# ricklisz/AnatoMask

Hardware: AMD Instinct MI355X
Metric: pretrain volumes/sec @128^3 patch mask=0.6 (higher is better)
Workload: dtype bf16; 1 GPU; STUNet-B AnatoMask step, 128^3 patch, mask_ratio 0.6, bf16 storage/MFMA + fp32 master; per_gpu_batch=16, global_batch=16, parallelism=dp1, step=teacher fwd + sampler + student fwd + loss + bwd + clip + AdamW + EMA

## Files before the change

anatomask_amd/csrc/stream_ops.hip:

```cpp
#include <mutex>
#include <type_traits>
#include "common.h"
#include "../../include/anatomask_hip.h"

namespace {

constexpr int NREP = 8;

struct Geo {
  int B, D, H, W, C;
  int vpw;
  unsigned mW, mH, mD;
  MaskView mask;
  __device__ __forceinline__ bool active(long v) const {
    if (!mask.m) return true;
    const unsigned u = (unsigned)v;
    const unsigned t1 = __umulhi(u, mW); const int w = u - t1 * W;
    const unsigned t2 = __umulhi(t1, mH); const int h = t1 - t2 * H;
    const unsigned b = __umulhi(t2, mD); const int d = t2 - b * D;
    return mask.active((int)b, d, h, w);
  }
  __device__ __forceinline__ void decode(long v, int& b, int& d, int& h, int& w) const {
    const unsigned u = (unsigned)v;
    const unsigned t1 = __umulhi(u, mW); w = u - t1 * W;
// ... 6 lines not shown
template <typename T> struct Walk {
  int cpv, vpp, cl, vl; bool live;
  __device__ __forceinline__ Walk(int C, int nthr = 256) {
    cpv = C / TT<T>::EPC; vpp = nthr / cpv; cl = threadIdx.x % cpv; vl = threadIdx.x / cpv; live = vl < vpp;
  }
};

template <typename T, int NT = 256>
__global__ __launch_bounds__(NT) void chan_stats_kernel(const T* __restrict__ x, Geo g, double* __restrict__ sums) {
  constexpr int EPC = TT<T>::EPC;
  __shared__ float red[NT * 2 * 8];
  Walk<T> wk(g.C, NT);
  float s1[EPC], s2[EPC];
#pragma unroll
  for (int i = 0; i < EPC; ++i) s1[i] = s2[i] = 0.f;
  const long v0 = (long)blockIdx.x * g.vpw, v1 = min(v0 + (long)g.vpw, g.nvox());
  if (wk.live)
    for (long v = v0 + wk.vl; v < v1; v += wk.vpp) {
      if (!g.active(v)) continue;
      float f[EPC];
      chunk_to_f<T>(*(const u32x4*)(x + v * g.C + wk.cl * EPC), f);
#pragma unroll
      for (int i = 0; i < EPC; ++i) { s1[i] += f[i]; s2[i] += f[i] * f[i]; }
    }
#pragma unroll
  for (int i = 0; i < EPC; ++i) { red[(threadIdx.x * 2) * 8 + i] = s1[i]; red[(threadIdx.x * 2 + 1) * 8 + i] = s2[i]; }
  __syncthreads();
  if (threadIdx.x < wk.cpv) {
    double a1[EPC], a2[EPC];
#pragma unroll
    for (int i = 0; i < EPC; ++i) a1[i] = a2[i] = 0.0;
    for (int vl = 0; vl < wk.vpp; ++vl) {
      const int t = vl * wk.cpv + threadIdx.x;
#pragma unroll
      for (int i = 0; i < EPC; ++i) { a1[i] += red[(t * 2) * 8 + i]; a2[i] += red[(t * 2 + 1) * 8 + i]; }
    }
#pragma unroll
    for (int i = 0; i < EPC; ++i) {
      const int c = threadIdx.x * EPC + i;
      double* sr = sums + (size_t)(blockIdx.x % NREP) * g.C * 2;
      atomicAdd(&sr[c * 2], a1[i]); atomicAdd(&sr[c * 2 + 1], a2[i]);
    }
  }
}

__global__ void mask_count_kernel(const uint8_t* mask, int n, int voxels_per_patch, double* out) {
  __shared__ double part[4];
  double c = 0;
  for (int i = threadIdx.x; i < n; i += 256) c += mask[i] ? 1.0 : 0.0;
  c = warp_sum_d(c);
  if ((threadIdx.x & 63) == 0) part[threadIdx.x >> 6] = c;
  __syncthreads();
  if (threadIdx.x == 0) out[0] = (part[0] + part[1] + part[2] + part[3]) * voxels_per_patch;
}

__global__ void norm_finalize_kernel(const double* sums, int nrep, const double* count_ptr, double count_host, int C,
                                     const float* gamma, const float* beta, float eps, float* mean, float* rstd,
                                     float* scale, float* shift, float* run_mean, float* run_var, float momentum) {
  const int c = blockIdx.x * 256 + threadIdx.x;
  if (c >= C) return;
  const double n = count_ptr ? count_ptr[0] : count_host;
  double q1 = 0.0, q2 = 0.0;
  for (int r = 0; r < nrep; ++r) { q1 += sums[((size_t)r * C + c) * 2]; q2 += sums[((size_t)r * C + c) * 2 + 1]; }
  const double m = q1 / n;
  double var = q2 / n - m * m;
  if (var < 0) var = 0;
  const float rs = (float)(1.0 / sqrt(var + (double)eps));
  mean[c] = (float)m; rstd[c] = rs;
  const float sc = gamma[c] * rs;
  scale[c] = sc; shift[c] = beta[c] - (float)m * sc;
  if (run_mean) {
    run_mean[c] = (1.f - momentum) * run_mean[c] + momentum * (float)m;
    run_var[c] = (1.f - momentum) * run_var[c] + momentum * (float)(var * (n / (n - 1.0)));
  }
}

__global__ void norm_fold_running_kernel(int C, const float* gamma, const float* beta, const float* run_mean,
                                         const float* run_var, float eps, float* scale, float* shift) {
  const int c = blockIdx.x * 256 + threadIdx.x;
  if (c >= C) return;
  const float sc = gamma[c] / sqrtf(run_var[c] + eps);
  scale[c] = sc; shift[c] = beta[c] - run_mean[c] * sc;
}

__device__ __forceinline__ float act_fwd(float v, int act) {
  if (act == AM_ACT_LRELU) return v > 0.f ? v : 0.01f * v;
  if (act == AM_ACT_RELU6) return fminf(fmaxf(v, 0.f), 6.f);
  return v;
}
__device__ __forceinline__ float act_grad(float out, int act) {
  if (act == AM_ACT_LRELU) return out > 0.f ? 1.f : 0.01f;
  if (act == AM_ACT_RELU6) return (out > 0.f && out < 6.f) ? 1.f : 0.f;
  return 1.f;
}

__device__ __forceinline__ float act_grad_pre(float pre, int act) {
  if (act == AM_ACT_LRELU) return pre > 0.f ? 1.f : 0.01f;
  if (act == AM_ACT_RELU6) return (pre > 0.f && pre < 6.f) ? 1.f : 0.f;
  return 1.f;
}

template <typename T, int NT = 256, int ACT_ = -1>
__global__ __launch_bounds__(NT) void norm_apply_kernel(const T* __restrict__ x, Geo g, const float* __restrict__ scale,
                                                         const float* __restrict__ shift, int act, const T* __restrict__ res,
                                                         const float* __restrict__ stem_x, const float* __restrict__ stem_w,
                                                         const float* __restrict__ stem_b, const float* __restrict__ fill,
                                                         T* __restrict__ y) {
  constexpr int EPC = TT<T>::EPC;
  Walk<T> wk(g.C, NT);
  if (!wk.live) return;
  float sc[EPC], sh[EPC];
#pragma unroll
  for (int i = 0; i < EPC; ++i) { sc[i] = scale[wk.cl * EPC + i]; sh[i] = shift[wk.cl * EPC + i]; }
  const long v0 = (long)blockIdx.x * g.vpw, v1 = min(v0 + (long)g.vpw, g.nvox());
  for (long v = v0 + wk.vl; v < v1; v += wk.vpp) {
    const size_t off = (size_t)v * g.C + wk.cl * EPC;
    float o[EPC];
    if (g.active(v)) {
      float f[EPC];
      chunk_to_f<T>(*(const u32x4*)(x + off), f);
#pragma unroll
      for (int i = 0; i < EPC; ++i) o[i] = f[i] * sc[i] + sh[i];
      if (res) {
        float r[EPC];
        chunk_to_f<T>(*(const u32x4*)(res + off), r);
#pragma unroll
        for (int i = 0; i < EPC; ++i) o[i] += r[i];
      }
      if (stem_x) {
        const float xv = stem_x[v];
#pragma unroll
        for (int i = 0; i < EPC; ++i) o[i] += stem_w[wk.cl * EPC + i] * xv + stem_b[wk.cl * EPC + i];
      }
#pragma unroll
      for (int i = 0; i < EPC; ++i) o[i] = act_fwd(o[i], ACT_ >= 0 ? ACT_ : act);
    } else if (fill) {
#pragma unroll
      for (int i = 0; i < EPC; ++i) o[i] = fill[wk.cl * EPC + i];
    } else {
      continue;
    }
    *(u32x4*)(y + off) = f_to_chunk<T>(o);
  }
}


struct BwdFin {
  unsigned* ticket;
  const double* count_ptr; double count_host;
  const float* gamma; const float* rstd;
  float *k0, *k1, *k2, *dgamma, *dbeta, *dtoken, *dbeta2;
};

__device__ __forceinline__ bool last_workgroup(unsigned* ticket) {
  __shared__ unsigned tk;
  asm volatile("s_waitcnt vmcnt(0)" ::: "memory");
  __syncthreads();
  if (threadIdx.x == 0) tk = atomicAdd(ticket, 1u);
  __syncthreads();
  return tk == gridDim.x - 1;
}

__device__ __forceinline__ void bwd_reduce_tail(double* bsum, int C, const BwdFin& f) {
  if (!f.ticket) return;
  if (!last_workgroup(f.ticket)) return;
  const double n = f.count_ptr ? f.count_ptr[0] : f.count_host;
  for (int c = threadIdx.x; c < C; c += blockDim.x) {
    double b1 = 0.0, b2 = 0.0, b3 = 0.0;
    for (int r = 0; r < NREP; ++r) {
      double* q = bsum + ((size_t)r * C + c) * 3;
      b1 += __longlong_as_double(atomicExch((unsigned long long*)&q[0], 0ull));
      b2 += __longlong_as_double(atomicExch((unsigned long long*)&q[1], 0ull));
      b3 += __longlong_as_double(atomicExch((unsigned long long*)&q[2], 0ull));
    }
    const float gr = f.gamma[c] * f.rstd[c];
    f.k0[c] = gr; f.k1[c] = gr * (float)(b1 / n); f.k2[c] = gr * (float)(b2 / n);
    if (f.dgamma) f.dgamma[c] += (float)b2;
    if (f.dbeta) f.dbeta[c] += (float)b1;
    if (f.dbeta2) f.dbeta2[c] += (float)b1;
    if (f.dtoken) f.dtoken[c] += (float)b3;
  }
  if (threadIdx.x == 0) atomicExch(f.ticket, 0u);
}

constexpr double AM_DX_FIX = 68719476736.0;
__device__ __forceinline__ void dxsum_tail(double* rep, int nrep, int C, float* accum, unsigned* ticket) {
  if (!ticket) return;
  if (!last_workgroup(ticket)) return;
  for (int c = threadIdx.x; c < C; c += blockDim.x) {
    long long s_ = 0;
    for (int r = 0; r < nrep; ++r) s_ += (long long)atomicExch((unsigned long long*)&rep[(size_t)r * C + c], 0ull);
    accum[c] += (float)((double)s_ / AM_DX_FIX);
  }
  if (threadIdx.x == 0) atomicExch(ticket, 0u);
}

template <typename T, int NT = 256, int ACT_ = -1, int OUT_ = 0>
__global__ __launch_bounds__(NT) void norm_bwd_reduce_kernel(const T* __restrict__ dout, const T* __restrict__ out,
                                                              const T* __restrict__ x, Geo g, const float* __restrict__ mean,
                                                              const float* __restrict__ rstd, int act, int fill,
                                                              double* __restrict__ bsum, const float* __restrict__ psc,
                                                              const float* __restrict__ psh, BwdFin fin) {
  constexpr int EPC = TT<T>::EPC;
  const int actv = ACT_ >= 0 ? ACT_ : act;
  const bool has_out = ACT_ >= 0 ? OUT_ != 0 : out != nullptr;
  __shared__ float red[NT * 3 * 8];
  Walk<T> wk(g.C, NT);
  float s1[EPC], s2[EPC], s3[EPC], mu[EPC], rs[EPC], qs[EPC], qh[EPC];
#pragma unroll
  for (int i = 0; i < EPC; ++i) { s1[i] = s2[i] = s3[i] = 0.f; mu[i] = rs[i] = qs[i] = qh[i] = 0.f; }
  if (wk.live) {
#pragma unroll
    for (int i = 0; i < EPC; ++i) {
      mu[i] = mean[wk.cl * EPC + i]; rs[i] = rstd[wk.cl * EPC + i];
      if (!has_out && actv != AM_ACT_NONE) { qs[i] = psc[wk.cl * EPC + i]; qh[i] = psh[wk.cl * EPC + i]; }
    }
    const long v0 = (long)blockIdx.x * g.vpw, v1 = min(v0 + (long)g.vpw, g.nvox());
    for (long v = v0 + wk.vl; v < v1; v += wk.vpp) {
      const size_t off = (size_t)v * g.C + wk.cl * EPC;
      const bool a = g.active(v);
      if (!a && !fill) continue;
      float d[EPC];
      chunk_to_f<T>(*(const u32x4*)(dout + off), d);
      if (!a) {
#pragma unroll
        for (int i = 0; i < EPC; ++i) s3[i] += d[i];
        continue;
      }
      float f[EPC];
      chunk_to_f<T>(*(const u32x4*)(x + off), f);
      if (actv != AM_ACT_NONE) {
        if (has_out) {
          float o[EPC];
          chunk_to_f<T>(*(const u32x4*)(out + off), o);
#pragma unroll
          for (int i = 0; i < EPC; ++i) d[i] *= act_grad(o[i], actv);
        } else {
#pragma unroll
          for (int i = 0; i < EPC; ++i) d[i] *= act_grad_pre(f[i] * qs[i] + qh[i], actv);
        }
      }
#pragma unroll
      for (int i = 0; i < EPC; ++i) { s1[i] += d[i]; s2[i] += d[i] * (f[i] - mu[i]) * rs[i]; }
    }
  }
#pragma unroll
  for (int i = 0; i < EPC; ++i) {
    red[(threadIdx.x * 3) * 8 + i] = s1[i]; red[(threadIdx.x * 3 + 1) * 8 + i] = s2[i]; red[(threadIdx.x * 3 + 2) * 8 + i] = s3[i];
  }
  __syncthreads();
  if (threadIdx.x < wk.cpv) {
    double a1[EPC], a2[EPC], a3[EPC];
#pragma unroll
    for (int i = 0; i < EPC; ++i) a1[i] = a2[i] = a3[i] = 0.0;
    for (int vl = 0; vl < wk.vpp; ++vl) {
      const int t = vl * wk.cpv + threadIdx.x;
#pragma unroll
      for (int i = 0; i < EPC; ++i) { a1[i] += red[(t * 3) * 8 + i]; a2[i] += red[(t * 3 + 1) * 8 + i]; a3[i] += red[(t * 3 + 2) * 8 + i]; }
    }
#pragma unroll
    for (int i = 0; i < EPC; ++i) {
      const int c = threadIdx.x * EPC + i;
      double* br = bsum + (size_t)(blockIdx.x % NREP) * g.C * 3;
      atomicAdd(&br[c * 3], a1[i]); atomicAdd(&br[c * 3 + 1], a2[i]);
      if (fill) atomicAdd(&br[c * 3 + 2], a3[i]);
    }
  }
  bwd_reduce_tail(bsum, g.C, fin);
}

__global__ void norm_bwd_finalize_kernel(const double* bsum, const double* count_ptr, double count_host, int C,
                                         const float* gamma, const float* rstd, float* k0, float* k1, float* k2,
                                         float* dgamma, float* dbeta, float* dtoken, float* dbeta2) {
  const int c = blockIdx.x * 256 + threadIdx.x;
  if (c >= C) return;
  const double n = count_ptr ? count_ptr[0] : count_host;
  double b1 = 0.0, b2 = 0.0, b3 = 0.0;
  for (int r = 0; r < NREP; ++r) { const double* q = bsum + ((size_t)r * C + c) * 3; b1 += q[0]; b2 += q[1]; b3 += q[2]; }
  const float gr = gamma[c] * rstd[c];
  k0[c] = gr;
  k1[c] = gr * (float)(b1 / n);
  k2[c] = gr * (float)(b2 / n);
  if (dgamma) dgamma[c] += (float)b2;
  if (dbeta) dbeta[c] += (float)b1;
  if (dbeta2) dbeta2[c] += (float)b1;
  if (dtoken) dtoken[c] += (float)b3;
}

template <typename T, int NT = 256, int ACT_ = -1, int OUT_ = 0>
__global__ __launch_bounds__(NT) void norm_bwd_apply_kernel(const T* __restrict__ dout, const T* __restrict__ out,
                                                             const T* __restrict__ x, Geo g, const float* __restrict__ mean,
                                                             const float* __restrict__ rstd, const float* __restrict__ k0,
                                                             const float* __restrict__ k1, const float* __restrict__ k2, int act,
                                                             T* __restrict__ dx, T* __restrict__ dres, double* __restrict__ dxsum,
                                                             int dxrep, const float* __restrict__ psc, const float* __restrict__ psh,
                                                             float* __restrict__ dx_accum, unsigned* dx_ticket) {
  constexpr int EPC = TT<T>::EPC;
  const int actv = ACT_ >= 0 ? ACT_ : act;
  const bool has_out = ACT_ >= 0 ? OUT_ != 0 : out != nullptr;
  __shared__ float red[NT * 8];
  Walk<T> wk(g.C, NT);
  float mu[EPC], rs[EPC], c0[EPC], c1[EPC], c2[EPC], sx[EPC], qs[EPC], qh[EPC];
#pragma unroll
  for (int i = 0; i < EPC; ++i) {
    const int c = wk.cl * EPC + i;
    sx[i] = 0.f; qs[i] = qh[i] = 0.f;
    if (wk.live) {
      mu[i] = mean[c]; rs[i] = rstd[c]; c0[i] = k0[c]; c1[i] = k1[c]; c2[i] = k2[c];
      if (!has_out && actv != AM_ACT_NONE) { qs[i] = psc[c]; qh[i] = psh[c]; }
    }
  }
  const long v0 = (long)blockIdx.x * g.vpw, v1 = min(v0 + (long)g.vpw, g.nvox());
  if (wk.live)
    for (long v = v0 + wk.vl; v < v1; v += wk.vpp) {
      if (!g.active(v)) continue;
      const size_t off = (size_t)v * g.C + wk.cl * EPC;
      float d[EPC], f[EPC];
      chunk_to_f<T>(*(const u32x4*)(dout + off), d);
      chunk_to_f<T>(*(const u32x4*)(x + off), f);
      if (actv != AM_ACT_NONE) {
        if (has_out) {
          float o[EPC];
          chunk_to_f<T>(*(const u32x4*)(out + off), o);
#pragma unroll
          for (int i = 0; i < EPC; ++i) d[i] *= act_grad(o[i], actv);
        } else {
#pragma unroll
          for (int i = 0; i < EPC; ++i) d[i] *= act_grad_pre(f[i] * qs[i] + qh[i], actv);
        }
      }
      if (dres) *(u32x4*)(dres + off) = f_to_chunk<T>(d);
      float r[EPC];
#pragma unroll
      for (int i = 0; i < EPC; ++i) r[i] = c0[i] * d[i] - c1[i] - c2[i] * (f[i] - mu[i]) * rs[i];
      const u32x4 pk = f_to_chunk<T>(r);
      *(u32x4*)(dx + off) = pk;
      if (dxsum) {
        float q[EPC];
        chunk_to_f<T>(pk, q);
#pragma unroll
        for (int i = 0; i < EPC; ++i) sx[i] += q[i];
      }
    }
  if (dxsum) {
#pragma unroll
    for (int i = 0; i < EPC; ++i) red[threadIdx.x * 8 + i] = sx[i];
    __syncthreads();
    if (threadIdx.x < wk.cpv) {
      float a1[EPC];
#pragma unroll
      for (int i = 0; i < EPC; ++i) a1[i] = 0.f;
      for (int vl = 0; vl < wk.vpp; ++vl)
#pragma unroll
        for (int i = 0; i < EPC; ++i) a1[i] += red[(vl * wk.cpv + threadIdx.x) * 8 + i];
#pragma unroll
      for (int i = 0; i < EPC; ++i)
        atomicAdd((unsigned long long*)&dxsum[(size_t)(blockIdx.x % dxrep) * g.C + threadIdx.x * EPC + i], (unsigned long long)__double2ll_rn((double)a1[i] * AM_DX_FIX));
    }
    dxsum_tail(dxsum, dxrep, g.C, dx_accum, dx_ticket);
  }
}


struct RowGeo {
  int B, D, H, W, C, bs;
  int rowchunks;
  int rpp;
  int rpw;
  long total_rows;
  const int* plist;
};
constexpr int UNR = 4;

template <typename T> struct RowWalk {
  int cl, vx, r0, cpv; bool live;
  long row, row_end; int rpp;
  __device__ __forceinline__ RowWalk(const RowGeo& g) {
    cpv = g.C / TT<T>::EPC;
    const int c = threadIdx.x % g.rowchunks;
    r0 = threadIdx.x / g.rowchunks; cl = c % cpv; vx = c / cpv; rpp = g.rpp; live = r0 < g.rpp;
    row = (long)blockIdx.x * g.rpw + r0;
    row_end = min((long)(blockIdx.x + 1) * g.rpw, g.total_rows);
  }
  __device__ __forceinline__ long voxel(const RowGeo& g, long rw) const {
    const int P = 1 << g.bs;
    const int a = (int)(rw >> (2 * g.bs)), r = (int)(rw & (P * P - 1));
    const int pk = g.plist[a];
    const int b = (pk >> 24) & 255, pd = (pk >> 16) & 255, ph = (pk >> 8) & 255, pw = pk & 255;
    return (((long)b * g.D + pd * P + (r >> g.bs)) * g.H + ph * P + (r & (P - 1))) * g.W + pw * P + vx;
  }
};

template <typename T, int ACT, int MODE>
__global__ __launch_bounds__(256) void norm_apply_rows_kernel(const T* __restrict__ x, RowGeo g, const float* __restrict__ scale,
                                                              const float* __restrict__ shift, const T* __restrict__ res,
                                                              const float* __restrict__ stem_x, const float* __restrict__ stem_w,
                                                              const float* __restrict__ stem_b, T* __restrict__ y) {
  constexpr int EPC = TT<T>::EPC;
  RowWalk<T> wk(g);
  float sc[EPC], sh[EPC], sw[EPC];
#pragma unroll
  for (int i = 0; i < EPC; ++i) {
    sc[i] = scale[wk.cl * EPC + i]; sh[i] = shift[wk.cl * EPC + i]; sw[i] = 0.f;
    if (MODE == 2) { sw[i] = stem_w[wk.cl * EPC + i]; sh[i] += stem_b[wk.cl * EPC + i]; }
  }
  const int P = 1 << g.bs, pm = P * P - 1, sh2 = 2 * g.bs;
  const long last = wk.row_end - 1;
  if (wk.row > last) return;
  int pk[UNR];
#pragma unroll
  for (int u = 0; u < UNR; ++u) { const long r = min(wk.row + (long)u * wk.rpp, last); pk[u] = g.plist[r >> sh2]; }
  for (long rw = wk.row; rw <= last; rw += (long)UNR * wk.rpp) {
    size_t off[UNR]; long vox[UNR]; u32x4 xv[UNR], rv[UNR]; float sx[UNR];
#pragma unroll
    for (int u = 0; u < UNR; ++u) {
      const long r = min(rw + (long)u * wk.rpp, last);
      const int q = (int)(r & pm);
      const int b = (pk[u] >> 24) & 255, pd = (pk[u] >> 16) & 255, ph = (pk[u] >> 8) & 255, pw = pk[u] & 255;
      vox[u] = (((long)b * g.D + pd * P + (q >> g.bs)) * g.H + ph * P + (q & (P - 1))) * g.W + pw * P + wk.vx;
      off[u] = (size_t)vox[u] * g.C + wk.cl * EPC;
    }
#pragma unroll
    for (int u = 0; u < UNR; ++u) {
      xv[u] = *(const u32x4*)(x + off[u]);
      if (MODE == 1) rv[u] = *(const u32x4*)(res + off[u]);
      if (MODE == 2) sx[u] = stem_x[vox[u]];
    }
#pragma unroll
    for (int u = 0; u < UNR; ++u) {
      const long r = min(rw + (long)(UNR + u) * wk.rpp, last);
      pk[u] = g.plist[r >> sh2];
    }
#pragma unroll
    for (int u = 0; u < UNR; ++u) {
      float f[EPC], o[EPC];
      chunk_to_f<T>(xv[u], f);
#pragma unroll
      for (int i = 0; i < EPC; ++i) o[i] = f[i] * sc[i] + sh[i];
      if (MODE == 1) {
        float r[EPC];
        chunk_to_f<T>(rv[u], r);
#pragma unroll
        for (int i = 0; i < EPC; ++i) o[i] += r[i];
      }
      if (MODE == 2) {
#pragma unroll
        for (int i = 0; i < EPC; ++i) o[i] += sw[i] * sx[u];
      }
#pragma unroll
      for (int i = 0; i < EPC; ++i) o[i] = act_fwd(o[i], ACT);
      *(u32x4*)(y + off[u]) = f_to_chunk<T>(o);
    }
  }
}

template <typename T>
__global__ __launch_bounds__(256) void chan_stats_rows_kernel(const T* __restrict__ x, RowGeo g, double* __restrict__ sums) {
  constexpr int EPC = TT<T>::EPC;
  __shared__ float red[256 * 2 * 8];
  RowWalk<T> wk(g);
  float s1[EPC], s2[EPC];
#pragma unroll
  for (int i = 0; i < EPC; ++i) s1[i] = s2[i] = 0.f;
  if (wk.live)
    for (long rw = wk.row; rw < wk.row_end; rw += (long)UNR * wk.rpp) {
      long v[UNR]; u32x4 xv[UNR];
#pragma unroll
      for (int u = 0; u < UNR; ++u) { const long r = rw + (long)u * wk.rpp; v[u] = r < wk.row_end ? wk.voxel(g, r) : -1; }
#pragma unroll
      for (int u = 0; u < UNR; ++u) if (v[u] >= 0) xv[u] = *(const u32x4*)(x + (size_t)v[u] * g.C + wk.cl * EPC);
#pragma unroll
      for (int u = 0; u < UNR; ++u) {
        if (v[u] < 0) continue;
        float f[EPC];
        chunk_to_f<T>(xv[u], f);
#pragma unroll
        for (int i = 0; i < EPC; ++i) { s1[i] += f[i]; s2[i] += f[i] * f[i]; }
      }
    }
#pragma unroll
  for (int i = 0; i < EPC; ++i) { red[(threadIdx.x * 2) * 8 + i] = s1[i]; red[(threadIdx.x * 2 + 1) * 8 + i] = s2[i]; }
  __syncthreads();
  const int nlane = blockDim.x / wk.cpv;
  if (threadIdx.x < wk.cpv) {
    double a1[EPC], a2[EPC];
#pragma unroll
    for (int i = 0; i < EPC; ++i) a1[i] = a2[i] = 0.0;
    for (int vl = 0; vl < nlane; ++vl) {
      const int t = vl * wk.cpv + threadIdx.x;
#pragma unroll
      for (int i = 0; i < EPC; ++i) { a1[i] += red[(t * 2) * 8 + i]; a2[i] += red[(t * 2 + 1) * 8 + i]; }
    }
#pragma unroll
    for (int i = 0; i < EPC; ++i) {
      const int c = threadIdx.x * EPC + i;
      double* sr = sums + (size_t)(blockIdx.x % NREP) * g.C * 2;
      atomicAdd(&sr[c * 2], a1[i]); atomicAdd(&sr[c * 2 + 1], a2[i]);
    }
  }
}

template <typename T, int ACT_ = -1, int OUT_ = 0>
__global__ __launch_bounds__(256) void norm_bwd_reduce_rows_kernel(const T* __restrict__ dout, const T* __restrict__ out,
                                                                   const T* __restrict__ x, RowGeo g, const float* __restrict__ mean,
                                                                   const float* __restrict__ rstd, int act, double* __restrict__ bsum,
                                                                   const float* __restrict__ psc, const float* __restrict__ psh, BwdFin fin) {
  constexpr int EPC = TT<T>::EPC;
  const int actv = ACT_ >= 0 ? ACT_ : act;
  const bool has_out = ACT_ >= 0 ? OUT_ != 0 : out != nullptr;
  __shared__ float red[256 * 2 * 8];
  RowWalk<T> wk(g);
  float s1[EPC], s2[EPC], mu[EPC], rs[EPC], qs[EPC], qh[EPC];
#pragma unroll
  for (int i = 0; i < EPC; ++i) { s1[i] = s2[i] = 0.f; mu[i] = rs[i] = qs[i] = qh[i] = 0.f; }
  if (wk.live) {
#pragma unroll
    for (int i = 0; i < EPC; ++i) {
      mu[i] = mean[wk.cl * EPC + i]; rs[i] = rstd[wk.cl * EPC + i];
      if (!has_out && actv != AM_ACT_NONE) { qs[i] = psc[wk.cl * EPC + i]; qh[i] = psh[wk.cl * EPC + i]; }
    }
    for (long rw = wk.row; rw < wk.row_end; rw += (long)UNR * wk.rpp) {
      long v[UNR]; u32x4 dv[UNR], xv[UNR], ov[UNR];
#pragma unroll
      for (int u = 0; u < UNR; ++u) { const long r = rw + (long)u * wk.rpp; v[u] = r < wk.row_end ? wk.voxel(g, r) : -1; }
#pragma unroll
      for (int u = 0; u < UNR; ++u) {
        if (v[u] < 0) continue;
        const size_t off = (size_t)v[u] * g.C + wk.cl * EPC;
        dv[u] = *(const u32x4*)(dout + off); xv[u] = *(const u32x4*)(x + off);
        if (has_out && actv != AM_ACT_NONE) ov[u] = *(const u32x4*)(out + off);
      }
#pragma unroll
      for (int u = 0; u < UNR; ++u) {
        if (v[u] < 0) continue;
        float d[EPC], f[EPC];
        chunk_to_f<T>(dv[u], d); chunk_to_f<T>(xv[u], f);
        if (actv != AM_ACT_NONE) {
          if (has_out) {
            float o[EPC];
            chunk_to_f<T>(ov[u], o);
#pragma unroll
            for (int i = 0; i < EPC; ++i) d[i] *= act_grad(o[i], actv);
          } else {
#pragma unroll
            for (int i = 0; i < EPC; ++i) d[i] *= act_grad_pre(f[i] * qs[i] + qh[i], actv);
          }
        }
#pragma unroll
        for (int i = 0; i < EPC; ++i) { s1[i] += d[i]; s2[i] += d[i] * (f[i] - mu[i]) * rs[i]; }
      }
    }
  }
#pragma unroll
  for (int i = 0; i < EPC; ++i) { red[(threadIdx.x * 2) * 8 + i] = s1[i]; red[(threadIdx.x * 2 + 1) * 8 + i] = s2[i]; }
  __syncthreads();
  const int nlane = blockDim.x / wk.cpv;
  if (threadIdx.x < wk.cpv) {
    double a1[EPC], a2[EPC];
#pragma unroll
    for (int i = 0; i < EPC; ++i) a1[i] = a2[i] = 0.0;
    for (int vl = 0; vl < nlane; ++vl) {
      const int t = vl * wk.cpv + threadIdx.x;
#pragma unroll
      for (int i = 0; i < EPC; ++i) { a1[i] += red[(t * 2) * 8 + i]; a2[i] += red[(t * 2 + 1) * 8 + i]; }
    }
#pragma unroll
    for (int i = 0; i < EPC; ++i) {
      const int c = threadIdx.x * EPC + i;
      double* br = bsum + (size_t)(blockIdx.x % NREP) * g.C * 3;
      atomicAdd(&br[c * 3], a1[i]); atomicAdd(&br[c * 3 + 1], a2[i]);
    }
  }
  bwd_reduce_tail(bsum, g.C, fin);
}

template <typename T, int ACT_ = -1, int OUT_ = 0>
__global__ __launch_bounds__(256) void norm_bwd_apply_rows_kernel(const T* __restrict__ dout, const T* __restrict__ out,
                                                                  const T* __restrict__ x, RowGeo g, const float* __restrict__ mean,
                                                                  const float* __restrict__ rstd, const float* __restrict__ k0,
                                                                  const float* __restrict__ k1, const float* __restrict__ k2, int act,
                                                                  T* __restrict__ dx, T* __restrict__ dres, double* __restrict__ dxsum,
                                                                  int dxrep, const float* __restrict__ psc, const float* __restrict__ psh,
                                                                  float* __restrict__ dx_accum, unsigned* dx_ticket) {
  constexpr int EPC = TT<T>::EPC;
  const int actv = ACT_ >= 0 ? ACT_ : act;
  const bool has_out = ACT_ >= 0 ? OUT_ != 0 : out != nullptr;
  __shared__ float red[256 * 8];
  RowWalk<T> wk(g);
  float mu[EPC], rs[EPC], c0[EPC], c1[EPC], c2[EPC], sx[EPC], qs[EPC], qh[EPC];
#pragma unroll
  for (int i = 0; i < EPC; ++i) {
    const int c = wk.cl * EPC + i;
    sx[i] = 0.f; qs[i] = qh[i] = 0.f;
    if (wk.live) {
      mu[i] = mean[c]; rs[i] = rstd[c]; c0[i] = k0[c]; c1[i] = k1[c]; c2[i] = k2[c];
      if (!has_out && actv != AM_ACT_NONE) { qs[i] = psc[c]; qh[i] = psh[c]; }
    }
  }
  if (wk.live)
    for (long rw = wk.row; rw < wk.row_end; rw += (long)UNR * wk.rpp) {
      long v[UNR]; u32x4 dv[UNR], xv[UNR], ov[UNR];
#pragma unroll
      for (int u = 0; u < UNR; ++u) { const long r = rw + (long)u * wk.rpp; v[u] = r < wk.row_end ? wk.voxel(g, r) : -1; }
#pragma unroll
      for (int u = 0; u < UNR; ++u) {
        if (v[u] < 0) continue;
        const size_t off = (size_t)v[u] * g.C + wk.cl * EPC;
        dv[u] = *(const u32x4*)(dout + off); xv[u] = *(const u32x4*)(x + off);
        if (has_out && actv != AM_ACT_NONE) ov[u] = *(const u32x4*)(out + off);
      }
#pragma unroll
      for (int u = 0; u < UNR; ++u) {
        if (v[u] < 0) continue;
        const size_t off = (size_t)v[u] * g.C + wk.cl * EPC;
        float d[EPC], f[EPC];
        chunk_to_f<T>(dv[u], d); chunk_to_f<T>(xv[u], f);
        if (actv != AM_ACT_NONE) {
          if (has_out) {
            float o[EPC];
            chunk_to_f<T>(ov[u], o);
#pragma unroll
            for (int i = 0; i < EPC; ++i) d[i] *= act_grad(o[i], actv);
          } else {
#pragma unroll
            for (int i = 0; i < EPC; ++i) d[i] *= act_grad_pre(f[i] * qs[i] + qh[i], actv);
          }
        }
        if (dres) *(u32x4*)(dres + off) = f_to_chunk<T>(d);
        float r[EPC];
#pragma unroll
        for (int i = 0; i < EPC; ++i) r[i] = c0[i] * d[i] - c1[i] - c2[i] * (f[i] - mu[i]) * rs[i];
        const u32x4 pk = f_to_chunk<T>(r);
        *(u32x4*)(dx + off) = pk;
        if (dxsum) {
          float q[EPC];
          chunk_to_f<T>(pk, q);
#pragma unroll
          for (int i = 0; i < EPC; ++i) sx[i] += q[i];
        }
      }
    }
  if (dxsum) {
#pragma unroll
    for (int i = 0; i < EPC; ++i) red[threadIdx.x * 8 + i] = sx[i];
    __syncthreads();
    const int nlane = blockDim.x / wk.cpv;
    if (threadIdx.x < wk.cpv) {
      float a1[EPC];
#pragma unroll
      for (int i = 0; i < EPC; ++i) a1[i] = 0.f;
      for (int vl = 0; vl < nlane; ++vl)
#pragma unroll
        for (int i = 0; i < EPC; ++i) a1[i] += red[(vl * wk.cpv + threadIdx.x) * 8 + i];
#pragma unroll
      for (int i = 0; i < EPC; ++i)
        atomicAdd((unsigned long long*)&dxsum[(size_t)(blockIdx.x % dxrep) * g.C + threadIdx.x * EPC + i], (unsigned long long)__double2ll_rn((double)a1[i] * AM_DX_FIX));
    }
    dxsum_tail(dxsum, dxrep, g.C, dx_accum, dx_ticket);
  }
}

__global__ __launch_bounds__(256) void mask_compact_kernel(const uint8_t* __restrict__ mask, int B, int fd, int fh, int fw,
                                                           int* __restrict__ list, int* __restrict__ count) {
  __shared__ int wsum[4];
  __shared__ int base;
  const int n = B * fd * fh * fw;
  if (threadIdx.x == 0) base = 0;
  __syncthreads();
  for (int i0 = 0; i0 < n; i0 += 256) {
    const int i = i0 + threadIdx.x;
    const int a = (i < n && mask[i]) ? 1 : 0;
    const unsigned long long bal = __ballot(a);
    const int lane = threadIdx.x & 63, wv = threadIdx.x >> 6;
    const int pre = __popcll(bal & ((1ull << lane) - 1ull));
    if (lane == 0) wsum[wv] = __popcll(bal);
    __syncthreads();
    int off = base;
    for (int w = 0; w < wv; ++w) off += wsum[w];
    if (a) {
      int q = i;
      const int pw = q % fw; q /= fw;
      const int ph = q % fh; q /= fh;
      const int pd = q % fd; const int b = q / fd;
      list[off + pre] = (b << 24) | (pd << 16) | (ph << 8) | pw;
    }
    __syncthreads();
    if (threadIdx.x == 0) base += wsum[0] + wsum[1] + wsum[2] + wsum[3];
    __syncthreads();
  }
  if (threadIdx.x == 0) count[0] = base;
}

template <typename T, int NT = 256>
__global__ __launch_bounds__(NT) void chan_sum_kernel(const T* __restrict__ x, Geo g, float* __restrict__ out) {
  constexpr int EPC = TT<T>::EPC;
  __shared__ float red[NT * 8];
  Walk<T> wk(g.C, NT);
  float s1[EPC];
#pragma unroll
  for (int i = 0; i < EPC; ++i) s1[i] = 0.f;
  const long v0 = (long)blockIdx.x * g.vpw, v1 = min(v0 + (long)g.vpw, g.nvox());
  if (wk.live)
    for (long v = v0 + wk.vl; v < v1; v += wk.vpp) {
      if (!g.active(v)) continue;
      float f[EPC];
      chunk_to_f<T>(*(const u32x4*)(x + v * g.C + wk.cl * EPC), f);
#pragma unroll
      for (int i = 0; i < EPC; ++i) s1[i] += f[i];
    }
#pragma unroll
  for (int i = 0; i < EPC; ++i) red[threadIdx.x * 8 + i] = s1[i];
  __syncthreads();
  if (threadIdx.x < wk.cpv) {
    float a1[EPC];
#pragma unroll
    for (int i = 0; i < EPC; ++i) a1[i] = 0.f;
    for (int vl = 0; vl < wk.vpp; ++vl)
#pragma unroll
      for (int i = 0; i < EPC; ++i) a1[i] += red[(vl * wk.cpv + threadIdx.x) * 8 + i];
#pragma unroll
    for (int i = 0; i < EPC; ++i) atomicAdd(&out[threadIdx.x * EPC + i], a1[i]);
  }
}

template <typename T>
__global__ void add_kernel(const T* a, const T* b, T* y, size_t nchunk) {
  constexpr int EPC = TT<T>::EPC;
  for (size_t i = (size_t)blockIdx.x * 256 + threadIdx.x; i < nchunk; i += (size_t)gridDim.x * 256) {
    float fa[EPC], fb[EPC];
    chunk_to_f<T>(((const u32x4*)a)[i], fa); chunk_to_f<T>(((const u32x4*)b)[i], fb);
#pragma unroll
    for (int k = 0; k < EPC; ++k) fa[k] += fb[k];
    ((u32x4*)y)[i] = f_to_chunk<T>(fa);
  }
}

constexpr int SBD = 4, SBH = 8, SBW = 16;

template <typename T, int K>
__global__ __launch_bounds__(256) void stem_conv_fwd_kernel(const float* __restrict__ x, Geo g,
                                                            const float* __restrict__ w, const float* __restrict__ bias,
                                                            T* __restrict__ y, float* __restrict__ part) {
  constexpr int EPC = TT<T>::EPC;
  constexpr int NTP = K * K * K, PAD = K / 2;
  constexpr int ED = SBD + 2 * PAD, EH = SBH + 2 * PAD, EW = SBW + 2 * PAD;
  constexpr int MV = SBD * SBH * SBW;
  extern __shared__ float sm[];
  float* wl = sm;
  float* xb = sm + g.C * NTP;
  int bid = blockIdx.x;
  const int nbw = g.W / SBW, nbh = g.H / SBH, nbd = g.D / SBD;
  const int bw_ = bid % nbw; bid /= nbw;
  const int bh_ = bid % nbh; bid /= nbh;
  const int bd_ = bid % nbd; const int b = bid / nbd;
  const int d0 = bd_ * SBD, h0 = bh_ * SBH, w0 = bw_ * SBW;
  float* prow = part ? part + (size_t)blockIdx.x * g.C * 2 : nullptr;
  if (!g.mask.active(b, d0, h0, w0)) {
    if (prow) for (int i = threadIdx.x; i < g.C * 2; i += 256) prow[i] = 0.f;
    return;
  }
  for (int i = threadIdx.x; i < g.C * NTP; i += 256) wl[(i % NTP) * g.C + i / NTP] = w[i];
  for (int e = threadIdx.x; e < ED * EH * EW; e += 256) {
    const int ex = e % EW, ey = (e / EW) % EH, ez = e / (EW * EH);
    const int id = d0 + ez - PAD, ih = h0 + ey - PAD, iw = w0 + ex - PAD;
    float v = 0.f;
    if (id >= 0 && id < g.D && ih >= 0 && ih < g.H && iw >= 0 && iw < g.W && g.mask.active(b, id, ih, iw))
      v = x[((size_t)(b * g.D + id) * g.H + ih) * g.W + iw];
    xb[e] = v;
  }
  __syncthreads();
  Walk<T> wk(g.C);
  float s1[EPC], s2[EPC];
#pragma unroll
  for (int i = 0; i < EPC; ++i) s1[i] = s2[i] = 0.f;
  if (wk.live) {
    float bs[EPC];
#pragma unroll
    for (int i = 0; i < EPC; ++i) bs[i] = bias ? bias[wk.cl * EPC + i] : 0.f;
    constexpr int VPT = 8;
    for (int vb = wk.vl; vb < MV; vb += wk.vpp * VPT) {
      float o[VPT][EPC];
      int xo[VPT];
#pragma unroll
      for (int q = 0; q < VPT; ++q) {
        const int v = vb + q * wk.vpp;
        const int vv = v < MV ? v : 0;
        xo[q] = ((vv / (SBW * SBH)) * EH + (vv / SBW) % SBH) * EW + vv % SBW;
#pragma unroll
        for (int i = 0; i < EPC; ++i) o[q][i] = bs[i];
      }
#pragma unroll 1
      for (int td = 0; td < K; ++td)
#pragma unroll 1
        for (int th = 0; th < K; ++th)
#pragma unroll
          for (int tw = 0; tw < K; ++tw) {
            const int ti = (td * K + th) * K + tw;
            const f32x4 wa = *(const f32x4*)(wl + ti * g.C + wk.cl * EPC);
            f32x4 wb = wa;
            if constexpr (EPC == 8) wb = *(const f32x4*)(wl + ti * g.C + wk.cl * EPC + 4);
#pragma unroll
            for (int q = 0; q < VPT; ++q) {
              const float xv = xb[xo[q] + (td * EH + th) * EW + tw];
#pragma unroll
              for (int i = 0; i < 4; ++i) o[q][i] += wa[i] * xv;
              if constexpr (EPC == 8) {
#pragma unroll
                for (int i = 0; i < 4; ++i) o[q][4 + i] += wb[i] * xv;
              }
            }
          }
#pragma unroll
      for (int q = 0; q < VPT; ++q) {
        const int v = vb + q * wk.vpp;
        if (v >= MV) continue;
        const int lw = v % SBW, lh = (v / SBW) % SBH, ld = v / (SBW * SBH);
        const size_t vox = ((size_t)(b * g.D + d0 + ld) * g.H + h0 + lh) * g.W + w0 + lw;
        const u32x4 pk = f_to_chunk<T>(o[q]);
        *(u32x4*)(y + vox * g.C + wk.cl * EPC) = pk;
        if (prow) {
          float r[EPC];
          chunk_to_f<T>(pk, r);
#pragma unroll
          for (int i = 0; i < EPC; ++i) { s1[i] += r[i]; s2[i] += r[i] * r[i]; }
        }
      }
    }
  }
  if (prow) {
    __syncthreads();
    float* red = sm;
    if (wk.live) {
#pragma unroll
      for (int i = 0; i < EPC; ++i) { red[(threadIdx.x * EPC + i) * 2] = s1[i]; red[(threadIdx.x * EPC + i) * 2 + 1] = s2[i]; }
    }
    __syncthreads();
    for (int c2 = threadIdx.x; c2 < g.C * 2; c2 += 256) {
      const int c = c2 >> 1, cl = c / EPC, i = c % EPC;
      float a = 0.f;
      for (int vl = 0; vl < wk.vpp; ++vl) a += red[((vl * wk.cpv + cl) * EPC + i) * 2 + (c2 & 1)];
      prow[c2] = a;
    }
  }
}


template <int NS>
__global__ __launch_bounds__(256) void stem_conv_mfma_kernel(const float* __restrict__ x, int D, int H, int W, int C, MaskView mask,
                                                             const int* __restrict__ plist, const float* __restrict__ w,
                                                             const float* __restrict__ bias, bf16_t* __restrict__ y,
                                                             float* __restrict__ part) {
  constexpr int E = 18;
  __shared__ float xl[E * E * E + 8];
  __shared__ float red[4 * 16 * NS * 2];
  const int tid = threadIdx.x, lane = tid & 63, wave = tid >> 6, g = lane >> 4, r16 = lane & 15;
  const int pk = plist[blockIdx.x];
  const int b = (pk >> 24) & 255, pd = (pk >> 16) & 255, ph = (pk >> 8) & 255, pw = pk & 255;
  const int d0 = pd * 16, h0 = ph * 16, w0 = pw * 16;
  for (int e = tid; e < E * E * E; e += 256) {
    const int ex = e % E, ey = (e / E) % E, ez = e / (E * E);
    const int id = d0 + ez - 1, ih = h0 + ey - 1, iw = w0 + ex - 1;
    float v = 0.f;
    if ((unsigned)id < (unsigned)D && (unsigned)ih < (unsigned)H && (unsigned)iw < (unsigned)W && mask.active(b, id, ih, iw))
      v = x[((size_t)(b * D + id) * H + ih) * W + iw];
    xl[e] = v;
  }
  typedef __attribute__((ext_vector_type(8))) __bf16 bfx8;
  bfx8 af[NS], afl[NS];
  int toff[8];
#pragma unroll
  for (int j = 0; j < 8; ++j) {
    const int t = 8 * g + j;
    toff[j] = t < 27 ? ((t / 9) * E + (t / 3) % 3) * E + t % 3 : 0;
  }
#pragma unroll
  for (int i = 0; i < NS; ++i) {
    const int ch = crow(i * 16 + r16);
    float wv[8];
#pragma unroll
    for (int j = 0; j < 8; ++j) { const int t = 8 * g + j; wv[j] = t < 27 ? w[ch * 27 + t] : 0.f; }
    u32x4 h, l;
    split8_bf16(wv, h, l);
    af[i] = __builtin_bit_cast(bfx8, h); afl[i] = __builtin_bit_cast(bfx8, l);
  }
  f32x4 bia[NS];
#pragma unroll
  for (int i = 0; i < NS; ++i) bia[i] = bias ? *(const f32x4*)(bias + (i >> 1) * 32 + g * 8 + (i & 1) * 4) : f32x4{0.f, 0.f, 0.f, 0.f};
  float s1[NS][4], s2[NS][4];
#pragma unroll
  for (int i = 0; i < NS; ++i)
#pragma unroll
    for (int q = 0; q < 4; ++q) s1[i][q] = s2[i][q] = 0.f;
  __syncthreads();
  for (int row = wave; row < 256; row += 4) {
    const int dz = row >> 4, dy = row & 15;
    const int base = (dz * E + dy) * E + r16;
    float xv[8];
#pragma unroll
    for (int j = 0; j < 8; ++j) xv[j] = xl[base + toff[j]];
    u32x4 xh, xo;
    split8_bf16(xv, xh, xo);
    const bfx8 bf = __builtin_bit_cast(bfx8, xh), bfl = __builtin_bit_cast(bfx8, xo);
    f32x4 o[NS];
#pragma unroll
    for (int i = 0; i < NS; ++i) {
      o[i] = __builtin_amdgcn_mfma_f32_16x16x32_bf16(afl[i], bf, bia[i], 0, 0, 0);
      o[i] = __builtin_amdgcn_mfma_f32_16x16x32_bf16(af[i], bfl, o[i], 0, 0, 0);
      o[i] = __builtin_amdgcn_mfma_f32_16x16x32_bf16(af[i], bf, o[i], 0, 0, 0);
    }
    const size_t vox = ((size_t)(b * D + d0 + dz) * H + h0 + dy) * W + w0 + r16;
    bf16_t* dst = y + vox * C + g * 8;
#pragma unroll
    for (int h = 0; h < NS / 2; ++h) {
      typedef __attribute__((ext_vector_type(4))) __bf16 bfx4;
      const bfx4 p0 = __builtin_convertvector(o[2 * h], bfx4), p1 = __builtin_convertvector(o[2 * h + 1], bfx4);
      *(bfx8*)(dst + h * 32) = __builtin_shufflevector(p0, p1, 0, 1, 2, 3, 4, 5, 6, 7);
      const f32x4 q0 = __builtin_convertvector(p0, f32x4), q1 = __builtin_convertvector(p1, f32x4);
#pragma unroll
      for (int c = 0; c < 4; ++c) {
        s1[2 * h][c] += q0[c]; s2[2 * h][c] += q0[c] * q0[c];
        s1[2 * h + 1][c] += q1[c]; s2[2 * h + 1][c] += q1[c] * q1[c];
      }
    }
  }
  if (part) {
#pragma unroll
    for (int i = 0; i < NS; ++i)
#pragma unroll
      for (int c = 0; c < 4; ++c) {
        float a1 = s1[i][c], a2 = s2[i][c];
        a1 = row16_sum(a1); a2 = row16_sum(a2);
        if (r16 == 0) {
          const int ch = (i >> 1) * 32 + g * 8 + (i & 1) * 4 + c;
          red[(wave * 16 * NS + ch) * 2] = a1; red[(wave * 16 * NS + ch) * 2 + 1] = a2;
        }
      }
    __syncthreads();
    if (tid < 16 * NS) {
      float a1 = 0.f, a2 = 0.f;
#pragma unroll
      for (int wv = 0; wv < 4; ++wv) { a1 += red[(wv * 16 * NS + tid) * 2]; a2 += red[(wv * 16 * NS + tid) * 2 + 1]; }
      float* pr = part + ((size_t)blockIdx.x * C + tid) * 2;
      pr[0] = a1; pr[1] = a2;
    }
  }
}

__device__ __forceinline__ s16x4 tr_read16(const unsigned char* p) {
  return __builtin_amdgcn_ds_read_tr16_b64_v4i16((__attribute__((address_space(3))) s16x4*)(p));
}

template <int NS, int K>
__global__ __launch_bounds__(256) void stem_wgrad_mfma_kernel(const float* __restrict__ x, const bf16_t* __restrict__ dy, int D, int H, int W,
                                                              MaskView mask, const int* __restrict__ plist, int n_active,
                                                              float* __restrict__ dw, float* __restrict__ db, float* __restrict__ det_ws) {
  constexpr int E = 18, C = 16 * NS, RS = 2 * C + 32;
  constexpr int NTT = K == 3 ? 2 : 1, NTAP = K * K * K;
  constexpr int XB = (E * E * E + 8) * 4;
  constexpr int CPV = C / 8, NLD = CPV;
  extern __shared__ __attribute__((aligned(16))) unsigned char lds[];
  float* xl = (float*)lds;
  unsigned char* yl = lds + XB;
  const int tid = threadIdx.x, lane = tid & 63, wave = tid >> 6, g = lane >> 4, r16 = lane & 15;
  const int q = (lane >> 2) & 3, p = lane & 3;
  typedef __attribute__((ext_vector_type(8))) __bf16 bfx8;
  f32x4 acc[NS][NTT];
#pragma unroll
  for (int i = 0; i < NS; ++i)
#pragma unroll
    for (int n = 0; n < NTT; ++n) acc[i][n] = f32x4{0.f, 0.f, 0.f, 0.f};
  int toff[NTT], kind[NTT];
#pragma unroll
  for (int n = 0; n < NTT; ++n) {
    const int t = 16 * n + r16;
    kind[n] = t < NTAP ? 0 : (t == NTAP ? 1 : 2);
    toff[n] = t < NTAP ? (K == 3 ? ((t / 9) * E + (t / 3) % 3) * E + t % 3 : (E + 1) * E + 1) : 0;
  }
  for (int pi = blockIdx.x; pi < n_active; pi += gridDim.x) {
    const int pk = plist[pi];
    const int b = (pk >> 24) & 255, d0 = ((pk >> 16) & 255) * 16, h0 = ((pk >> 8) & 255) * 16, w0 = (pk & 255) * 16;
    __syncthreads();
    for (int e = tid; e < E * E * E; e += 256) {
      const int ex = e % E, ey = (e / E) % E, ez = e / (E * E);
      const int id = d0 + ez - 1, ih = h0 + ey - 1, iw = w0 + ex - 1;
      float v = 0.f;
      if ((unsigned)id < (unsigned)D && (unsigned)ih < (unsigned)H && (unsigned)iw < (unsigned)W && mask.active(b, id, ih, iw))
        v = x[((size_t)(b * D + id) * H + ih) * W + iw];
      xl[e] = v;
    }
    u32x4 ld[NLD];
    auto load_plane = [&](int dz) {
#pragma unroll
      for (int it = 0; it < NLD; ++it) {
        const int idx = tid + it * 256, vox = idx / CPV, ch = idx % CPV;
        const size_t gv = ((size_t)(b * D + d0 + dz) * H + h0 + (vox >> 4)) * W + w0 + (vox & 15);
        ld[it] = *(const u32x4*)(dy + gv * C + ch * 8);
      }
    };
    load_plane(0);
    for (int dz = 0; dz < 16; ++dz) {
      __syncthreads();
#pragma unroll
      for (int it = 0; it < NLD; ++it) {
        const int idx = tid + it * 256, vox = idx / CPV, ch = idx % CPV;
        *(u32x4*)(yl + vox * RS + ch * 16) = ld[it];
      }
      load_plane(dz < 15 ? dz + 1 : 15);
      __syncthreads();
#pragma unroll
      for (int s2 = 0; s2 < 2; ++s2) {
        const int s = wave + 4 * s2;
        const int v1 = s * 32 + g * 4 + q, v2 = v1 + 16;
        bfx8 af[NS];
#pragma unroll
        for (int i = 0; i < NS; ++i) {
          const s16x4 lo = tr_read16(yl + v1 * RS + (16 * i + 4 * p) * 2), hi = tr_read16(yl + v2 * RS + (16 * i + 4 * p) * 2);
          af[i] = __builtin_bit_cast(bfx8, s16x8{lo[0], lo[1], lo[2], lo[3], hi[0], hi[1], hi[2], hi[3]});
        }
        const int xbase = (dz * E + 2 * s) * E + 4 * g;
#pragma unroll
        for (int n = 0; n < NTT; ++n) {
          float qv[8];
#pragma unroll
          for (int j = 0; j < 4; ++j) { qv[j] = xl[xbase + toff[n] + j]; qv[4 + j] = xl[xbase + toff[n] + E + j]; }
          if (kind[n]) {
#pragma unroll
            for (int j = 0; j < 8; ++j) qv[j] = kind[n] == 1 ? 1.f : 0.f;
          }
          u32x4 xh, xo;
          split8_bf16(qv, xh, xo);
          const bfx8 bf = __builtin_bit_cast(bfx8, xh), bfl = __builtin_bit_cast(bfx8, xo);
#pragma unroll
          for (int i = 0; i < NS; ++i) {
            acc[i][n] = __builtin_amdgcn_mfma_f32_16x16x32_bf16(af[i], bfl, acc[i][n], 0, 0, 0);
            acc[i][n] = __builtin_amdgcn_mfma_f32_16x16x32_bf16(af[i], bf, acc[i][n], 0, 0, 0);
          }
        }
      }
    }
  }
  __syncthreads();
  float* red = (float*)lds;
#pragma unroll
  for (int i = 0; i < NS; ++i)
#pragma unroll
    for (int n = 0; n < NTT; ++n)
#pragma unroll
      for (int r = 0; r < 4; ++r) red[(wave * C + 16 * i + 4 * g + r) * (16 * NTT) + 16 * n + r16] = acc[i][n][r];
  __syncthreads();
  for (int i = tid; i < C * (NTAP + 1); i += 256) {
    const int c = i / (NTAP + 1), t = i % (NTAP + 1);
    float v = 0.f;
#pragma unroll
    for (int wv = 0; wv < 4; ++wv) v += red[(wv * C + c) * (16 * NTT) + t];
    if (det_ws) det_ws[(size_t)blockIdx.x * (C * (NTAP + 1)) + i] = v;
    else if (t < NTAP) atomicAdd(&dw[c * NTAP + t], v);
    else if (db) atomicAdd(&db[c], v);
  }
}

__global__ __launch_bounds__(256) void stem_wgrad_fold_kernel(const float* __restrict__ ws, int nwg, int C, int ntap, float* __restrict__ dw,
                                                              float* __restrict__ db) {
  const int i = blockIdx.x * 256 + threadIdx.x;
  if (i >= C * (ntap + 1)) return;
  float s = 0.f;
  for (int r = 0; r < nwg; ++r) s += ws[(size_t)r * C * (ntap + 1) + i];
  const int c = i / (ntap + 1), t = i % (ntap + 1);
  if (t < ntap) dw[c * ntap + t] += s;
  else if (db) db[c] += s;
}

template <typename T>
__global__ __launch_bounds__(256) void stem_conv_wgrad_kernel(const float* __restrict__ x, const T* __restrict__ dy, Geo g, int k,
                                                              float* __restrict__ dw, float* __restrict__ db) {
  constexpr int EPC = TT<T>::EPC;
  extern __shared__ float sm[];
  const int nt = k * k * k, pad = k / 2;
  const int ED = SBD + 2 * pad, EH = SBH + 2 * pad, EW = SBW + 2 * pad;
  float* acc_l = sm;
  float* xb = sm + g.C * (nt + 1);
  const int nbw = g.W / SBW, nbh = g.H / SBH, nbd = g.D / SBD;
  const int nbrick = g.B * nbd * nbh * nbw;
  for (int i = threadIdx.x; i < g.C * (nt + 1); i += 256) acc_l[i] = 0.f;
  Walk<T> wk(g.C);
  for (int tg = 0; tg < nt; tg += 9) {
    float a[9][EPC], sb[EPC];
#pragma unroll
    for (int q = 0; q < 9; ++q)
#pragma unroll
      for (int i = 0; i < EPC; ++i) a[q][i] = 0.f;
#pragma unroll
    for (int i = 0; i < EPC; ++i) sb[i] = 0.f;
    for (int brick = blockIdx.x; brick < nbrick; brick += gridDim.x) {
      int bid = brick;
      const int bw_ = bid % nbw; bid /= nbw;
      const int bh_ = bid % nbh; bid /= nbh;
      const int bd_ = bid % nbd; const int b = bid / nbd;
      const int d0 = bd_ * SBD, h0 = bh_ * SBH, w0 = bw_ * SBW;
      if (!g.mask.active(b, d0, h0, w0)) continue;
      __syncthreads();
      for (int e = threadIdx.x; e < ED * EH * EW; e += 256) {
        const int ex = e % EW, ey = (e / EW) % EH, ez = e / (EW * EH);
        const int id = d0 + ez - pad, ih = h0 + ey - pad, iw = w0 + ex - pad;
        float v = 0.f;
        if (id >= 0 && id < g.D && ih >= 0 && ih < g.H && iw >= 0 && iw < g.W && g.mask.active(b, id, ih, iw))
          v = x[((size_t)(b * g.D + id) * g.H + ih) * g.W + iw];
        xb[e] = v;
      }
      __syncthreads();
      if (!wk.live) continue;
      for (int v = wk.vl; v < SBD * SBH * SBW; v += wk.vpp) {
        const int lw = v % SBW, lh = (v / SBW) % SBH, ld = v / (SBW * SBH);
        const size_t vox = ((size_t)(b * g.D + d0 + ld) * g.H + h0 + lh) * g.W + w0 + lw;
        float d[EPC];
        chunk_to_f<T>(*(const u32x4*)(dy + vox * g.C + wk.cl * EPC), d);
        if (tg == 0) {
#pragma unroll
          for (int i = 0; i < EPC; ++i) sb[i] += d[i];
        }
#pragma unroll
        for (int q = 0; q < 9; ++q) {
          const int ti = tg + q;
          if (ti < nt) {
            const int td = ti / (k * k), th = (ti / k) % k, tw = ti % k;
            const float xv = xb[((ld + td) * EH + lh + th) * EW + lw + tw];
#pragma unroll
            for (int i = 0; i < EPC; ++i) a[q][i] += d[i] * xv;
          }
        }
      }
    }
    if (wk.live) {
#pragma unroll
      for (int q = 0; q < 9; ++q)
        if (tg + q < nt)
#pragma unroll
          for (int i = 0; i < EPC; ++i) atomicAdd(&acc_l[(wk.cl * EPC + i) * (nt + 1) + tg + q], a[q][i]);
      if (tg == 0)
#pragma unroll
        for (int i = 0; i < EPC; ++i) atomicAdd(&acc_l[(wk.cl * EPC + i) * (nt + 1) + nt], sb[i]);
    }
  }
  __syncthreads();
  for (int i = threadIdx.x; i < g.C * (nt + 1); i += 256) {
    const int c = i / (nt + 1), t = i % (nt + 1);
    const float v = acc_l[i];
    if (v == 0.f) continue;
    if (t < nt) atomicAdd(&dw[c * nt + t], v);
    else if (db) atomicAdd(&db[c], v);
  }
}

template <typename T>
__global__ __launch_bounds__(256) void proj_fwd_kernel(const T* __restrict__ x, long nvox, int C, const float* __restrict__ w,
                                                       const float* __restrict__ b, const float* __restrict__ psc,
                                                       const float* __restrict__ psh, float* __restrict__ rec) {
  constexpr int EPC = TT<T>::EPC;
  const long v = (long)blockIdx.x * 256 + threadIdx.x;
  if (v >= nvox) return;
  float s = b[0];
  if (psc) {
    for (int c = 0; c < C; c += EPC) {
      float f[EPC];
      chunk_to_f<T>(*(const u32x4*)(x + (size_t)v * C + c), f);
#pragma unroll
      for (int i = 0; i < EPC; ++i) s += (f[i] * psc[c + i] + psh[c + i]) * w[c + i];
    }
  } else {
    for (int c = 0; c < C; c += EPC) {
      float f[EPC];
      chunk_to_f<T>(*(const u32x4*)(x + (size_t)v * C + c), f);
#pragma unroll
      for (int i = 0; i < EPC; ++i) s += f[i] * w[c + i];
    }
  }
  rec[v] = s;
}

struct ProjNormFin {
  unsigned* ticket; double n;
  const float *gamma, *beta, *rstd, *scale, *w;
  float *k0w, *k1, *k2, *dgamma, *dbeta, *dw, *db;
};

template <typename T>
__global__ __launch_bounds__(256) void proj_norm_bwd_reduce_kernel(const T* __restrict__ x, const float* __restrict__ drec, long nvox, int C,
                                                                   int vpw, const float* __restrict__ mean, double* __restrict__ acc,
                                                                   ProjNormFin fin) {
  constexpr int EPC = TT<T>::EPC;
  __shared__ float red[256 * 8];
  __shared__ float redb[4];
  __shared__ double s0sh;
  Walk<T> wk(C);
  float s1[EPC], mu[EPC], sb = 0.f;
#pragma unroll
  for (int i = 0; i < EPC; ++i) { s1[i] = 0.f; mu[i] = wk.live ? mean[wk.cl * EPC + i] : 0.f; }
  const long v0 = (long)blockIdx.x * vpw, v1 = min(v0 + (long)vpw, nvox);
  if (wk.live)
    for (long v = v0 + wk.vl; v < v1; v += wk.vpp) {
      const float d = drec[v];
      float f[EPC];
      chunk_to_f<T>(*(const u32x4*)(x + (size_t)v * C + wk.cl * EPC), f);
#pragma unroll
      for (int i = 0; i < EPC; ++i) s1[i] += d * (f[i] - mu[i]);
      if (wk.cl == 0) sb += d;
    }
#pragma unroll
  for (int i = 0; i < EPC; ++i) red[threadIdx.x * 8 + i] = s1[i];
  sb = warp_sum(sb);
  if ((threadIdx.x & 63) == 0) redb[threadIdx.x >> 6] = sb;
// ... 358 lines not shown
  g.vpw = pick_vpw((long)B * D * H * W, C, dtype, reduction);
  g.mW = (unsigned)(0x100000000ull / (unsigned)W) + 1; g.mH = (unsigned)(0x100000000ull / (unsigned)H) + 1;
  g.mD = (unsigned)(0x100000000ull / (unsigned)D) + 1;
  return g;
}
inline bool geo_ok(int B, int D, int H, int W) {
  const unsigned long long n = (unsigned long long)B * D * H * W;
  int m = W > H ? W : H; if (D > m) m = D;
  return n * (unsigned long long)m < 0xffffffffull;
}


inline bool mkrows(RowGeo& r, int dtype, bool reduction, int B, int D, int H, int W, int C, int bs, const int* plist, int n_active) {
  if (!plist || n_active <= 0 || bs < 0 || bs > 6) return false;
  const int epc = dtype == AM_DT_BF16 ? 8 : 4;
  const int P = 1 << bs;
  const long rc = (long)P * C / epc;
  if (rc > 256 || rc < 1 || (D >> bs) > 255 || (H >> bs) > 255 || (W >> bs) > 255 || B > 255) return false;
  if (D % P || H % P || W % P) return false;
  r.B = B; r.D = D; r.H = H; r.W = W; r.C = C; r.bs = bs; r.plist = plist;
  r.rowchunks = (int)rc; r.rpp = 256 / r.rowchunks;
  r.total_rows = (long)n_active * P * P;
  const long target = reduction ? 1024 : 2048;
  long rpw = (r.total_rows + target - 1) / target;
  const long unit = (long)UNR * r.rpp;
  rpw = (rpw + unit - 1) / unit * unit;
  if (rpw < unit) rpw = unit;
  if (rpw > 64 * unit) rpw = 64 * unit;
  r.rpw = (int)rpw;
  return true;
}
inline int rows_blocks(const RowGeo& r) { return (int)((r.total_rows + r.rpw - 1) / r.rpw); }
inline int rows_threads(const RowGeo& r) { return r.rpp * r.rowchunks; }

}

constexpr int F32_MAX_C_512 = 2048, F32_MAX_C_256 = 1024;
template <typename F> inline void by_pack_dtype(int dtype, F&& f) { if (dtype == AM_DT_F32S) f(am_type<f32s_t>{}); else am_by_dtype(dtype, f); }

extern "C" {

int am_chan_stats(int dtype, const void* x, int B, int D, int H, int W, int C, const uint8_t* mask, int bshift, int fd, int fh,
                  int fw, double* sums, const int32_t* active_list, int n_active, void* stream) {
  if (!am_row_ok(dtype, C, F32_MAX_C_512)) return -1;
  Geo g = mkgeo(dtype, true, B, D, H, W, C, mask, bshift, fd, fh, fw);
  const bool geo_bad = mask && !geo_ok(B, D, H, W);
  hipStream_t st = (hipStream_t)stream;
  AM_HIP(hipMemsetAsync(sums, 0, sizeof(double) * 2 * C * NREP, st));
  RowGeo rg;
  if (mask && mkrows(rg, dtype, true, B, D, H, W, C, bshift, active_list, n_active)) {
    am_by_dtype(dtype, [&](auto t) {
      using T = typename decltype(t)::type;
      AM_LAUNCH(chan_stats_rows_kernel<T>, dim3(rows_blocks(rg)), dim3(rows_threads(rg)), 0, st, (const T*)x, rg, sums);
    });
    AM_CHECK_LAUNCH();
    return 0;
  }
  if (geo_bad) return -4;
  const int nb = nblk((long)B * D * H * W, g.vpw);
  am_by_walk(dtype, C, [&](auto t, auto nt) {
    using T = typename decltype(t)::type;
    AM_LAUNCH((chan_stats_kernel<T, nt>), dim3(nb), dim3(nt), 0, st, (const T*)x, g, sums);
  });
  AM_CHECK_LAUNCH();
  return 0;
}

int am_mask_count(const uint8_t* mask, int n, int voxels_per_patch, double* out, void* stream) {
  AM_LAUNCH(mask_count_kernel, dim3(1), dim3(256), 0, (hipStream_t)stream, mask, n, voxels_per_patch, out);
  AM_CHECK_LAUNCH();
  return 0;
}

int am_mask_compact(const uint8_t* mask, int B, int fd, int fh, int fw, int32_t* list, int32_t* count, void* stream) {
  if (B > 255 || fd > 255 || fh > 255 || fw > 255) return -1;
  AM_LAUNCH(mask_compact_kernel, dim3(1), dim3(256), 0, (hipStream_t)stream, mask, B, fd, fh, fw, list, count);
  AM_CHECK_LAUNCH();
  return 0;
}

int am_norm_finalize(const double* sums, int nrep, const double* count_ptr, double count_host, int C, const float* gamma,
                     const float* beta, float eps, float* mean, float* rstd, float* scale, float* shift, float* run_mean,
                     float* run_var, float momentum, void* stream) {
  AM_LAUNCH(norm_finalize_kernel, dim3((C + 255) / 256), dim3(256), 0, (hipStream_t)stream, sums, nrep, count_ptr, count_host,
                     C, gamma, beta, eps, mean, rstd, scale, shift, run_mean, run_var, momentum);
  AM_CHECK_LAUNCH();
  return 0;
}

int am_norm_fold_running(int C, const float* gamma, const float* beta, const float* run_mean, const float* run_var, float eps,
                         float* scale, float* shift, void* stream) {
  AM_LAUNCH(norm_fold_running_kernel, dim3((C + 255) / 256), dim3(256), 0, (hipStream_t)stream, C, gamma, beta, run_mean,
                     run_var, eps, scale, shift);
  AM_CHECK_LAUNCH();
  return 0;
}

int am_norm_apply(int dtype, const void* x, int B, int D, int H, int W, int C, const uint8_t* mask, int bshift, int fd, int fh,
                  int fw, const float* scale, const float* shift, int act, const void* res, const float* stem_x,
                  const float* stem_w, const float* stem_b, const float* fill, void* y, const int32_t* active_list, int n_active,
                  void* stream) {
  if (!am_row_ok(dtype, C, F32_MAX_C_512)) return -1;
  Geo g = mkgeo(dtype, false, B, D, H, W, C, mask, bshift, fd, fh, fw);
  const bool geo_bad = mask && !geo_ok(B, D, H, W);
  hipStream_t st = (hipStream_t)stream;
  RowGeo rg;
  if (mask && !fill && !(res && stem_x) && mkrows(rg, dtype, false, B, D, H, W, C, bshift, active_list, n_active)) {
    const dim3 gr(rows_blocks(rg)), bl(rows_threads(rg));
    const int racts = act == AM_ACT_LRELU || act == AM_ACT_RELU6 ? act : AM_ACT_NONE;
    am_by_dtype_int<AM_ACT_NONE, AM_ACT_LRELU, AM_ACT_RELU6>(dtype, racts, [&](auto t, auto a) {
      using T = typename decltype(t)::type;
      am_by_int<0, 1, 2>(res ? 1 : (stem_x ? 2 : 0), [&](auto m) {
        AM_LAUNCH((norm_apply_rows_kernel<T, a, m>), gr, bl, 0, st, (const T*)x, rg, scale, shift, (const T*)res, stem_x, stem_w, stem_b, (T*)y);
      });
    });
    AM_CHECK_LAUNCH();
    return 0;
  }
  if (geo_bad) return -4;
  const int nb = nblk((long)B * D * H * W, g.vpw);
  am_by_walk_act(dtype, C, act, false, [&](auto t, auto nt, auto a, auto) {
    using T = typename decltype(t)::type;
    AM_LAUNCH((norm_apply_kernel<T, nt, a>), dim3(nb), dim3(nt), 0, st, (const T*)x, g, scale, shift, act, (const T*)res, stem_x, stem_w, stem_b, fill, (T*)y);
  });
  AM_CHECK_LAUNCH();
  return 0;
}

int am_norm_bwd_reduce(int dtype, const void* dout, const void* out, const void* x, int B, int D, int H, int W, int C,
                       const uint8_t* mask, int bshift, int fd, int fh, int fw, const float* mean, const float* rstd, int act,
                       int fill, double* bsum, const float* pre_scale, const float* pre_shift, const int32_t* active_list,
                       int n_active, const double* count_ptr, double count_host, const float* gamma, float* k0, float* k1, float* k2,
                       float* dgamma, float* dbeta, float* dtoken, float* dbeta2, void* stream) {
  if (!am_row_ok(dtype, C, F32_MAX_C_512)) return -1;
  if (!out && act != AM_ACT_NONE && (!pre_scale || !pre_shift)) return -1;
  Geo g = mkgeo(dtype, true, B, D, H, W, C, mask, bshift, fd, fh, fw);
  const bool geo_bad = mask && !geo_ok(B, D, H, W);
  hipStream_t st = (hipStream_t)stream;
  BwdFin fin{};
  if (k0) {
    if (!gamma || !k1 || !k2) return -1;
    fin.ticket = (unsigned*)(bsum + (size_t)3 * C * NREP);
    fin.count_ptr = count_ptr; fin.count_host = count_host; fin.gamma = gamma; fin.rstd = rstd;
    fin.k0 = k0; fin.k1 = k1; fin.k2 = k2; fin.dgamma = dgamma; fin.dbeta = dbeta; fin.dtoken = dtoken; fin.dbeta2 = dbeta2;
  } else {
    AM_HIP(hipMemsetAsync(bsum, 0, sizeof(double) * 3 * C * NREP, st));
  }
  RowGeo rg;
  if (mask && !fill && mkrows(rg, dtype, true, B, D, H, W, C, bshift, active_list, n_active)) {
    am_by_dtype(dtype, [&](auto t) {
      using T = typename decltype(t)::type;
      am_by_act(act, out != nullptr, [&](auto a, auto o) {
        AM_LAUNCH((norm_bwd_reduce_rows_kernel<T, a, o>), dim3(rows_blocks(rg)), dim3(rows_threads(rg)), 0, st, (const T*)dout, (const T*)out, (const T*)x, rg,
                  mean, rstd, act, bsum, pre_scale, pre_shift, fin);
      });
    });
    AM_CHECK_LAUNCH();
    return 0;
  }
  if (geo_bad) return -4;
  const int nb = nblk((long)B * D * H * W, g.vpw);
  am_by_walk_act(dtype, C, act, out != nullptr, [&](auto t, auto nt, auto a, auto o) {
    using T = typename decltype(t)::type;
    AM_LAUNCH((norm_bwd_reduce_kernel<T, nt, a, o>), dim3(nb), dim3(nt), 0, st, (const T*)dout, (const T*)out, (const T*)x, g, mean, rstd, act, fill, bsum,
              pre_scale, pre_shift, fin);
  });
  AM_CHECK_LAUNCH();
  return 0;
}

int am_norm_bwd_finalize(const double* bsum, const double* count_ptr, double count_host, int C, const float* gamma,
                         const float* rstd, float* k0, float* k1, float* k2, float* dgamma, float* dbeta, float* dtoken,
                         float* dbeta2, void* stream) {
  AM_LAUNCH(norm_bwd_finalize_kernel, dim3((C + 255) / 256), dim3(256), 0, (hipStream_t)stream, bsum, count_ptr,
                     count_host, C, gamma, rstd, k0, k1, k2, dgamma, dbeta, dtoken, dbeta2);
  AM_CHECK_LAUNCH();
  return 0;
}

int am_norm_bwd_apply(int dtype, const void* dout, const void* out, const void* x, int B, int D, int H, int W, int C,
                      const uint8_t* mask, int bshift, int fd, int fh, int fw, const float* mean, const float* rstd,
                      const float* k0, const float* k1, const float* k2, int act, void* dx, void* dres, float* dxsum_accum,
                      double* dxsum_scratch, const float* pre_scale, const float* pre_shift, const int32_t* active_list, int n_active,
                      int scratch_is_zero_workspace, void* stream) {
  if (!am_row_ok(dtype, C, F32_MAX_C_512)) return -1;
  if (!out && act != AM_ACT_NONE && (!pre_scale || !pre_shift)) return -1;
  Geo g = mkgeo(dtype, false, B, D, H, W, C, mask, bshift, fd, fh, fw);
  const bool geo_bad = mask && !geo_ok(B, D, H, W);
  hipStream_t st = (hipStream_t)stream;
  RowGeo rg;
  const bool rows = mask && mkrows(rg, dtype, false, B, D, H, W, C, bshift, active_list, n_active);
  if (!rows && geo_bad) return -4;
  const int nb = rows ? rows_blocks(rg) : nblk((long)B * D * H * W, g.vpw);
  if (dxsum_accum && !dxsum_scratch) return -1;
  const bool rep = dxsum_accum != nullptr;
  double* dxs = rep ? dxsum_scratch : nullptr;
  const int nrep = AM_DXREP;
  const bool fused = rep && scratch_is_zero_workspace;
  float* dx_accum = fused ? dxsum_accum : nullptr;
  unsigned* dx_ticket = fused ? (unsigned*)(dxsum_scratch + (size_t)AM_DXREP * C) : nullptr;
  if (rep && !fused) AM_HIP(hipMemsetAsync(dxsum_scratch, 0, sizeof(double) * AM_DXREP * C, st));
  if (rows) {
    am_by_dtype(dtype, [&](auto t) {
      using T = typename decltype(t)::type;
      am_by_act(act, out != nullptr, [&](auto a, auto o) {
        AM_LAUNCH((norm_bwd_apply_rows_kernel<T, a, o>), dim3(nb), dim3(rows_threads(rg)), 0, st, (const T*)dout, (const T*)out, (const T*)x, rg, mean, rstd,
                  k0, k1, k2, act, (T*)dx, (T*)dres, dxs, nrep, pre_scale, pre_shift, dx_accum, dx_ticket);
      });
    });
  } else {
    am_by_walk_act(dtype, C, act, out != nullptr, [&](auto t, auto nt, auto a, auto o) {
      using T = typename decltype(t)::type;
      AM_LAUNCH((norm_bwd_apply_kernel<T, nt, a, o>), dim3(nb), dim3(nt), 0, st, (const T*)dout, (const T*)out, (const T*)x, g, mean, rstd,
                k0, k1, k2, act, (T*)dx, (T*)dres, dxs, nrep, pre_scale, pre_shift, dx_accum, dx_ticket);
    });
  }
  AM_CHECK_LAUNCH();
  if (rep && !fused) { AM_LAUNCH(rep_reduce_kernel, dim3((C + 255) / 256), dim3(256), 0, st, dxsum_scratch, AM_DXREP, C, dxsum_accum); AM_CHECK_LAUNCH(); }
  return 0;
}

int am_chan_sum(int dtype, const void* x, int B, int D, int H, int W, int C, const uint8_t* mask, int bshift, int fd, int fh,
                int fw, float* out_accum, void* stream) {
  if (!am_row_ok(dtype, C, F32_MAX_C_512)) return -1;
  Geo g = mkgeo(dtype, true, B, D, H, W, C, mask, bshift, fd, fh, fw);
  if (mask && !geo_ok(B, D, H, W)) return -4;
  hipStream_t st = (hipStream_t)stream;
  if ((long)B * D * H * W * C <= (4L << 20)) { g.vpw = (int)((long)B * D * H * W); const int vpp = walk_threads(C, dtype) / (C / (dtype == AM_DT_BF16 ? 8 : 4)) > 0 ? walk_threads(C, dtype) / (C / (dtype == AM_DT_BF16 ? 8 : 4)) : 1; g.vpw = (g.vpw + vpp - 1) / vpp * vpp; }
  const int nb = nblk((long)B * D * H * W, g.vpw);
  am_by_walk(dtype, C, [&](auto t, auto nt) {
    using T = typename decltype(t)::type;
    AM_LAUNCH((chan_sum_kernel<T, nt>), dim3(nb), dim3(nt), 0, st, (const T*)x, g, out_accum);
  });
  AM_CHECK_LAUNCH();
  return 0;
}

int am_add(int dtype, const void* a, const void* b, void* y, long n_elems, void* stream) {
  hipStream_t st = (hipStream_t)stream;
  const size_t nchunk = (size_t)n_elems / (dtype == AM_DT_BF16 ? 8 : 4);
  int nb = (int)((nchunk + 255) / 256); if (nb > 4096) nb = 4096; if (nb < 1) nb = 1;
  am_by_dtype(dtype, [&](auto t) {
    using T = typename decltype(t)::type;
    AM_LAUNCH(add_kernel<T>, dim3(nb), dim3(256), 0, st, (const T*)a, (const T*)b, (T*)y, nchunk);
  });
  AM_CHECK_LAUNCH();
  return 0;
}

int am_stem_conv_fwd(int dtype, const float* x, int B, int D, int H, int W, int C, int ksize, const uint8_t* mask, int bshift,
                     int fd, int fh, int fw, const float* w, const float* bias, void* y, float* partials,
                     const int32_t* active_list, int n_active, int* partial_rows_written, void* stream) {
  if (!am_row_ok(dtype, C, F32_MAX_C_256)) return -1;
  if (ksize != 1 && ksize != 3) return -2;
  Geo g = mkgeo(dtype, false, B, D, H, W, C, mask, bshift, fd, fh, fw);
  hipStream_t st = (hipStream_t)stream;
  if (!mask || bshift != 4 || D % 16 || H % 16 || W % 16) return -2;
  if ((long)B * (D / SBD) * (H / SBH) * (W / SBW) > 0x7fffffffL) return -4;
  if (partial_rows_written) *partial_rows_written = B * (D / SBD) * (H / SBH) * (W / SBW);
  if (dtype == AM_DT_BF16 && ksize == 3 && active_list && n_active > 0 && (C == 32 || C == 64 || C == 96) && B <= 255 && fd <= 255 && fh <= 255 && fw <= 255) {
    const MaskView mv{mask, fd, fh, fw, bshift};
    am_by_int<2, 4, 6>(C / 16, [&](auto ns) {
      AM_LAUNCH(stem_conv_mfma_kernel<ns>, dim3(n_active), dim3(256), 0, st, x, D, H, W, C, mv, active_list, w, bias, (bf16_t*)y, partials);
    });
    AM_CHECK_LAUNCH();
    if (partial_rows_written) *partial_rows_written = n_active;
    return 0;
  }
  const int nb = B * (D / SBD) * (H / SBH) * (W / SBW);
  const int pad_ = ksize / 2;
  size_t fl = (size_t)C * ksize * ksize * ksize;
  if (partials && fl < (size_t)256 * 8 * 2) fl = (size_t)256 * 8 * 2;
  const size_t sm = sizeof(float) * (fl + (size_t)(SBD + 2 * pad_) * (SBH + 2 * pad_) * (SBW + 2 * pad_));
  am_by_dtype_int<1, 3>(dtype, ksize, [&](auto t, auto k) {
    using T = typename decltype(t)::type;
    AM_LAUNCH((stem_conv_fwd_kernel<T, k>), dim3(nb), dim3(256), sm, st, x, g, w, bias, (T*)y, partials);
  });
  AM_CHECK_LAUNCH();
  return 0;
}

int am_stem_conv_wgrad(int dtype, const float* x, const void* dy, int B, int D, int H, int W, int C, int ksize,
                       const uint8_t* mask, int bshift, int fd, int fh, int fw, float* dw_accum, float* db_accum,
                       const int32_t* active_list, int n_active, float* det_workspace, long det_workspace_floats, void* stream) {
  if (!am_row_ok(dtype, C, F32_MAX_C_256)) return -1;
  if (ksize != 1 && ksize != 3) return -2;
  Geo g = mkgeo(dtype, true, B, D, H, W, C, mask, bshift, fd, fh, fw);
  hipStream_t st = (hipStream_t)stream;
  if (!mask || bshift != 4 || D % 16 || H % 16 || W % 16) return -2;
  if (dtype == AM_DT_BF16 && active_list && n_active > 0 && (C == 32 || C == 64 || C == 96) && B <= 255 && fd <= 255 && fh <= 255 && fw <= 255) {
    const MaskView mv{mask, fd, fh, fw, bshift};
    int nwg = n_active < 1024 ? n_active : 1024;
    const long det_row = (long)C * (ksize * ksize * ksize + 1);
    if (det_workspace) {
        if (det_workspace_floats < det_row) return -6;
        if (nwg > det_workspace_floats / det_row) nwg = (int)(det_workspace_floats / det_row);
    }
    const size_t sm = (size_t)(18 * 18 * 18 + 8) * 4 + (size_t)256 * (2 * C + 32);
    hipError_t optin = hipSuccess;
    am_by_int<2, 4, 6>(C / 16, [&](auto ns) {
      am_by_int<1, 3>(ksize, [&](auto k) {
        constexpr auto kern = stem_wgrad_mfma_kernel<ns, k>;
        if ((optin = am_lds_optin<kern>()) != hipSuccess) return;
        AM_LAUNCH(kern, dim3(nwg), dim3(256), sm, st, x, (const bf16_t*)dy, D, H, W, mv, active_list, n_active, dw_accum, db_accum, det_workspace);
      });
    });
    AM_HIP(optin);
    AM_CHECK_LAUNCH();
    if (det_workspace) {
      AM_LAUNCH(stem_wgrad_fold_kernel, dim3((unsigned)((det_row + 255) / 256)), dim3(256), 0, st, det_workspace, nwg, C, ksize * ksize * ksize, dw_accum, db_accum);
      AM_CHECK_LAUNCH();
    }
    return 0;
  }
  if ((long)B * (D / SBD) * (H / SBH) * (W / SBW) > 0x7fffffffL) return -4;
  int nb = B * (D / SBD) * (H / SBH) * (W / SBW);
  if (nb > 1024) nb = 1024;
  const int pad_ = ksize / 2;
  const size_t sm = sizeof(float) * ((size_t)C * (ksize * ksize * ksize + 1) + (size_t)(SBD + 2 * pad_) * (SBH + 2 * pad_) * (SBW + 2 * pad_));
  am_by_dtype(dtype, [&](auto t) {
    using T = typename decltype(t)::type;
    AM_LAUNCH(stem_conv_wgrad_kernel<T>, dim3(nb), dim3(256), sm, st, x, (const T*)dy, g, ksize, dw_accum, db_accum);
  });
  AM_CHECK_LAUNCH();
  return 0;
}

int am_proj_fwd(int dtype, const void* x, long nvox, int C, const float* w, const float* b, const float* pre_scale, const float* pre_shift,
                float* rec, void* stream) {
  if (!am_row_ok(dtype, C, F32_MAX_C_256)) return -1;
  if ((pre_scale == nullptr) != (pre_shift == nullptr)) return -1;
  hipStream_t st = (hipStream_t)stream;
  const int nb = (int)((nvox + 255) / 256);
  am_by_dtype(dtype, [&](auto t) {
    using T = typename decltype(t)::type;
    AM_LAUNCH(proj_fwd_kernel<T>, dim3(nb), dim3(256), 0, st, (const T*)x, nvox, C, w, b, pre_scale, pre_shift, rec);
  });
  AM_CHECK_LAUNCH();
  return 0;
}

int am_proj_norm_bwd(int dtype, const void* x, const float* drec, long nvox, int C, const float* w, const float* gamma, const float* beta,
                     const float* mean, const float* rstd, const float* scale, double* workspace, float* coef, void* dx,
                     float* dgamma_accum, float* dbeta_accum, float* dw_accum, float* db_accum, void* stream) {
  if (!am_row_ok(dtype, C, F32_MAX_C_256)) return -1;
  if (!x || !drec || !w || !gamma || !beta || !mean || !rstd || !scale || !workspace || !coef || !dx || !dgamma_accum || !dbeta_accum ||
      !dw_accum || !db_accum || nvox <= 0) return -1;
  hipStream_t st = (hipStream_t)stream;
  ProjNormFin fin{(unsigned*)(workspace + (size_t)NREP * (C + 1)), (double)nvox, gamma, beta, rstd, scale, w,
                  coef, coef + C, coef + 2 * C, dgamma_accum, dbeta_accum, dw_accum, db_accum};
  const int vr = pick_vpw(nvox, C, dtype, true), va = pick_vpw(nvox, C, dtype, false);
  am_by_dtype(dtype, [&](auto t) {
    using T = typename decltype(t)::type;
    AM_LAUNCH(proj_norm_bwd_reduce_kernel<T>, dim3(nblk(nvox, vr)), dim3(256), 0, st, (const T*)x, drec, nvox, C, vr, mean, workspace, fin);
  });
  AM_CHECK_LAUNCH();
  am_by_dtype(dtype, [&](auto t) {
    using T = typename decltype(t)::type;
    AM_LAUNCH(proj_norm_bwd_apply_kernel<T>, dim3(nblk(nvox, va)), dim3(256), 0, st, (const T*)x, drec, nvox, C, va, mean, rstd, coef, coef + C, coef + 2 * C, (T*)dx);
  });
  AM_CHECK_LAUNCH();
  return 0;
}

int am_proj_bwd(int dtype, const void* x, const float* drec, long nvox, int C, const float* w, void* dx, float* dw_accum,
                float* db_accum, float* det_workspace, long det_workspace_floats, void* stream) {
  if (!am_row_ok(dtype, C, F32_MAX_C_256)) return -1;
  hipStream_t st = (hipStream_t)stream;
  const int vpw = pick_vpw(nvox, C, dtype, true);
  const int nb = nblk(nvox, vpw);
  if (det_workspace && det_workspace_floats < (long)nb * (C + 1)) return -6;
  am_by_dtype(dtype, [&](auto t) {
    using T = typename decltype(t)::type;
    AM_LAUNCH(proj_bwd_kernel<T>, dim3(nb), dim3(256), 0, st, (const T*)x, drec, nvox, C, vpw, w, (T*)dx, dw_accum, db_accum, det_workspace);
  });
  AM_CHECK_LAUNCH();
  if (det_workspace) {
    AM_LAUNCH(rows_fold_kernel, dim3((C + 1 + 255) / 256), dim3(256), 0, st, det_workspace, nb, C + 1, C, dw_accum, db_accum);
    AM_CHECK_LAUNCH();
  }
  return 0;
}

int am_partials_reduce(const float* partials, int rows, int C, double* sums, float* sum_accum, void* stream) {
  hipStream_t st = (hipStream_t)stream;
  if ((256 % C == 0 || C % 256 == 0) && rows >= 64) {
    const int rstep = C <= 256 ? 256 / C : 1;
    int nb = rows / (rstep * 16); nb = nb < 1 ? 1 : (nb > 256 ? 256 : nb);
    const int rpb = ((rows + nb - 1) / nb + rstep - 1) / rstep * rstep;
    nb = (rows + rpb - 1) / rpb;
    if (sums) AM_HIP(hipMemsetAsync(sums, 0, sizeof(double) * 2 * C, st));
    AM_LAUNCH(partials_reduce2_kernel, dim3(nb), dim3(256), 0, st, partials, rows, C, rpb, sums, sum_accum);
    AM_CHECK_LAUNCH();
    return 0;
  }
  AM_LAUNCH(partials_reduce_kernel, dim3(C), dim3(256), 0, st, partials, rows, C, sums, sum_accum);
  AM_CHECK_LAUNCH();
  return 0;
}


int am_partials_finalize(const float* partials, int rows, int C, double* workspace, const double* count_ptr, double count_host,
                         const float* gamma, const float* beta, float eps, float* mean, float* rstd, float* scale, float* shift,
                         float* run_mean, float* run_var, float momentum, long* num_batches_tracked, float* sum_accum, void* stream) {
  if (C <= 0 || C > 4096 || rows <= 0 || !workspace) return -1;
  if (gamma && (!beta || !mean || !rstd || !scale || !shift)) return -1;
  if (C % 2) return -1;
  const int cp = C / 2, rstep = cp <= 256 ? 256 / cp : 1;
  int nb = rows / (rstep * 8); nb = nb < 1 ? 1 : (nb > 2048 ? 2048 : nb);
  const int rpb = ((rows + nb - 1) / nb + rstep - 1) / rstep * rstep;
  nb = (rows + rpb - 1) / rpb;
  AM_LAUNCH(partials_finalize_kernel, dim3(nb), dim3(256), 0, (hipStream_t)stream, partials, rows, C, rpb, workspace, count_ptr, count_host,
            gamma, beta, eps, mean, rstd, scale, shift, run_mean, run_var, momentum, num_batches_tracked, sum_accum,
            (const float*)nullptr, (const float*)nullptr, (float*)nullptr, (float*)nullptr, (float*)nullptr, (float*)nullptr, (float*)nullptr, (float*)nullptr);
  AM_CHECK_LAUNCH();
  return 0;
}

int am_norm_bwd_from_partials(const float* partials, int rows, int C, double* workspace, const double* count_ptr, double count_host,
                              const float* gamma, const float* mean, const float* rstd, float* k0, float* k1, float* k2,
                              float* dgamma, float* dbeta, float* dbeta2, void* stream) {
  if (C <= 0 || C > 4096 || C % 2 || rows <= 0 || !workspace || !gamma || !mean || !rstd || !k0 || !k1 || !k2) return -1;
  const int cp = C / 2, rstep = cp <= 256 ? 256 / cp : 1;
  int nb = rows / (rstep * 8); nb = nb < 1 ? 1 : (nb > 2048 ? 2048 : nb);
  const int rpb = ((rows + nb - 1) / nb + rstep - 1) / rstep * rstep;
  nb = (rows + rpb - 1) / rpb;
  AM_LAUNCH(partials_finalize_kernel, dim3(nb), dim3(256), 0, (hipStream_t)stream, partials, rows, C, rpb, workspace, count_ptr, count_host,
            gamma, (const float*)nullptr, 0.f, (float*)nullptr, (float*)nullptr, (float*)nullptr, (float*)nullptr, (float*)nullptr, (float*)nullptr,
            0.f, (long*)nullptr, (float*)nullptr, mean, rstd, k0, k1, k2, dgamma, dbeta, dbeta2);
  AM_CHECK_LAUNCH();
  return 0;
}

int am_pack_weight(int dtype, const float* src, void* dst, int R, int K, int taps, long stride_r, long stride_k, int Rp, int Kp,
                   void* stream) {
  hipStream_t st = (hipStream_t)stream;
  if (Rp < R || Kp < K) return -1;
  dim3 grid(Rp, (Kp + 63) / 64);
  const size_t sm = sizeof(float) * 64 * taps;
  if (dtype == AM_DT_F32S && Kp % 16) return -1;
  by_pack_dtype(dtype, [&](auto t) {
    using T = typename decltype(t)::type;
    AM_LAUNCH(pack_weight_kernel<T>, grid, dim3(256), sm, st, src, (T*)dst, R, K, taps, stride_r, stride_k, Rp, Kp);
  });
  AM_CHECK_LAUNCH();
  return 0;
}

int am_pack_weights_batched(int dtype, const am_pack_desc* descs, int ndesc, int total_blocks, void* stream) {
  hipStream_t st = (hipStream_t)stream;
  if (ndesc <= 0 || total_blocks <= 0) return 0;
  by_pack_dtype(dtype, [&](auto t) { AM_LAUNCH(pack_weights_batched_kernel<typename decltype(t)::type>, dim3(total_blocks), dim3(256), 0, st, descs, ndesc); });
  AM_CHECK_LAUNCH();
  return 0;
}

int am_split_bf16(const float* x, void* hi, void* lo, long n, void* stream) {
  if (n % 4) return -1;
  long nb = (n / 4 + 255) / 256; if (nb > 16384) nb = 16384;
  AM_LAUNCH(split_bf16_kernel, dim3((unsigned)nb), dim3(256), 0, (hipStream_t)stream, x, (bf16_t*)hi, (bf16_t*)lo, n / 4);
  AM_CHECK_LAUNCH();
  return 0;
}

int am_unpack_grad(const float* src_packed, float* dst, int R, int K, int taps, long stride_r, long stride_k, int accumulate,
                   void* stream) {
  const long n = (long)taps * R * K;
  int nb = (int)((n + 255) / 256); if (nb > 8192) nb = 8192;
  AM_LAUNCH(unpack_grad_kernel, dim3(nb), dim3(256), 0, (hipStream_t)stream, src_packed, dst, R, K, taps, stride_r, stride_k, accumulate);
  AM_CHECK_LAUNCH();
  return 0;
}

}
```

anatomask_amd/engine.py:

```python
from __future__ import annotations

from dataclasses import dataclass, field
from typing import Dict, List, Optional, Sequence, Tuple

import torch

from . import ops
from .ops import ACT_LRELU, ACT_NONE, ACT_RELU6, CONV_DGRAD, CONV_FWD, CONVT_DGRAD, CONVT_FWD, MaskInfo, NormStats

ENC = "sparse_encoder.sp_cnn.conv_blocks_context"
DEC = "dense_decoder.dec"


@dataclass
class Spec:
    dims: Sequence[int]
    depth: Sequence[int]
    width: int
    input_size: Tuple[int, int, int]
    in_ch: int = 1
    out_ch: int = 1
    downsample: int = 16
    n_stage: int = 5
    sync_bn: bool = False
# ... 201 lines not shown
    else:
        a1 = ops.norm_apply(y1, st1, ACT_LRELU, mask, bs)
        y2, pt2 = ops.conv3d(CONV_FWD, a1, w2, W[f"{p}.conv2.bias"], sp, 3, 1,
                             in_mask=mask, in_bshift=bs, out_mask=mask, out_bshift=bs, want_partials=True)
    st2 = _sparse_norm(y2, mask, bs, counts, W[f"{p}.norm2.weight"], W[f"{p}.norm2.bias"], 1e-5, pt2)
    if s == 0 and first and prefix is None:
        out = ops.norm_apply(y2, st2, ACT_LRELU, mask, bs, stem=(inp, W[f"{p}.conv3.weight"].view(-1), W[f"{p}.conv3.bias"]))
    elif first:
        sc = ops.conv3d(CONV_FWD, x, pk.get(W, f"{p}.conv3.weight", False, False), W[f"{p}.conv3.bias"], sp, 1, stride,
                        in_mask=mask, in_bshift=bs + (1 if stride == 2 else 0), out_mask=mask, out_bshift=bs)
        out = ops.norm_apply(y2, st2, ACT_LRELU, mask, bs, res=sc)
    else:
        out = ops.norm_apply(y2, st2, ACT_LRELU, mask, bs, res=x)
    rec_.update(y1=y1, st1=st1, a1=a1, y2=y2, st2=st2, out=out)
    return out, rec_


def _dec_block(W, pk, i: int, x, nxt, train: bool, update_running: bool = True, fuse_eval: bool = False, out_skip=None, sync: bool = False,
               head: bool = False, inorm: bool = False, stencil_tail: bool = False):
    q = f"{DEC}.{i}"
    so = tuple(2 * v for v in x.shape[1:4])
    u = ops.conv3d(CONVT_FWD, x, pk.get(W, f"{q}.up_sample.weight", True, False), W[f"{q}.up_sample.bias"], so, 4, 2)
    if inorm:
        assert not head
        c1 = ops.conv3d(CONV_FWD, u, pk.get(W, f"{q}.conv.0.weight", False, False), None, so, 3, 1)
        r, st1 = _instance_norm(c1, ACT_RELU6)
        c2 = ops.conv3d(CONV_FWD, r, pk.get(W, f"{q}.conv.3.weight", False, False), None, so, 3, 1)
        o, st2 = _instance_norm(c2, ACT_NONE, res=nxt)
        return o, {"q": q, "xin": x, "u": u, "c1": c1, "st1": st1, "r": r, "c2": c2, "st2": st2, "inorm": True}
    if not train and fuse_eval:
        C1, C2 = W[f"{q}.conv.0.weight"].shape[0], W[f"{q}.conv.3.weight"].shape[0]
        st1, st2 = NormStats(C1, x.device), NormStats(C2, x.device)
        ops.norm_fold_running(st1, W[f"{q}.conv.1.weight"], W[f"{q}.conv.1.bias"], W[f"{q}.conv.1.running_mean"], W[f"{q}.conv.1.running_var"], 1e-5)
        ops.norm_fold_running(st2, W[f"{q}.conv.4.weight"], W[f"{q}.conv.4.bias"], W[f"{q}.conv.4.running_mean"], W[f"{q}.conv.4.running_var"], 1e-5)
        r = ops.conv3d(CONV_FWD, u, pk.get(W, f"{q}.conv.0.weight", False, False), None, so, 3, 1,
                       ep_scale=st1.scale, ep_shift=st1.shift, ep_act=ACT_RELU6)
        if stencil_tail and nxt is None and ops.head_stencil_supported(r):
            return r, {"stencil": True, "st2": st2}
        o = ops.conv3d(CONV_FWD, r, pk.get(W, f"{q}.conv.3.weight", False, False), None, so, 3, 1,
                       ep_scale=st2.scale, ep_shift=st2.shift, ep_res=nxt, out_mask=out_skip, out_bshift=4 if out_skip is not None else 0)
        return o, None
    c1, pt1 = ops.conv3d(CONV_FWD, u, pk.get(W, f"{q}.conv.0.weight", False, False), None, so, 3, 1, want_partials=train), None
    if train:
        c1, pt1 = c1
    st1 = _batch_norm(c1, W, f"{q}.conv.1", train, pt1, update_running, sync)
    r = ops.norm_apply(c1, st1, ACT_RELU6)
    c2, pt2 = ops.conv3d(CONV_FWD, r, pk.get(W, f"{q}.conv.3.weight", False, False), None, so, 3, 1, want_partials=train), None
    if train:
        c2, pt2 = c2
    st2 = _batch_norm(c2, W, f"{q}.conv.4", train, pt2, update_running, sync)
    if head:
        assert train and nxt is None and st2.sync_world <= 1
        return c2, {"q": q, "xin": x, "u": u, "c1": c1, "st1": st1, "r": r, "c2": c2, "st2": st2, "head": True}
    o = ops.norm_apply(c2, st2, ACT_NONE, res=nxt)
    return o, {"q": q, "xin": x, "u": u, "c1": c1, "st1": st1, "r": r, "c2": c2, "st2": st2}


def encoder_forward(spec: Spec, W, pk: PackCache, inp: torch.Tensor, mask: MaskInfo, counts, tape: Optional[Tape] = None,
                    recompute: bool = False) -> List[torch.Tensor]:
    feats = []
    x = None
    for s in range(spec.n_stage):
        sp = spec.stage_spatial(s)
        if tape is not None and recompute:
            tape.enc_in.append(x)
        for b in range(spec.depth[s]):
            x, rec_ = _enc_block(W, pk, inp, mask, counts, sp, s, b, x, keep=tape is not None)
            if tape is not None and not recompute:
                tape.enc.append(rec_)
        feats.append(x)
    return feats


def densify_forward(spec: Spec, W, pk: PackCache, feats, mask: MaskInfo, counts, tape: Optional[Tape] = None) -> List[torch.Tensor]:
    n_dec = len(spec.dec_chs) - 1
    to_dec = []
    for i in range(n_dec):
        f = feats[4 - i]
        st = _sparse_norm(f, mask, i, counts, W[f"densify_norms.{i}.weight"], W[f"densify_norms.{i}.bias"], 1e-6)
        d = ops.norm_apply(f, st, ACT_NONE, mask, i, fill=W[f"mask_tokens.{i}"].view(-1))
        pw = f"densify_projs.{i}.weight"
        if pw in W:
            k = W[pw].shape[-1]
            pr = ops.conv3d(CONV_FWD, d, pk.get(W, pw, False, False), W[f"densify_projs.{i}.bias"], tuple(d.shape[1:4]), k, 1)
        else:
            pr = d
        to_dec.append(pr)
        if tape is not None:
            tape.dens.append({"i": i, "f": f, "st": st, "d": d, "k": W[pw].shape[-1] if pw in W else 0})
    return to_dec


HEAD_STENCIL = True


def decoder_forward(spec: Spec, W, pk: PackCache, to_dec, train: bool, tape: Optional[Tape] = None, recompute: bool = False,
                    needed_patches: Optional[MaskInfo] = None, fuse_eval: Optional[bool] = None, l2_of: Optional[tuple] = None) -> torch.Tensor:
    n_dec = len(spec.dec_chs) - 1
    if fuse_eval is None:
        fuse_eval = tape is None
    x = to_dec[0]
    head = bool(train and FUSED_HEAD and _sync_world(spec.sync_bn) <= 1 and not spec.dec_inorm)
    st_head = None
    for i in range(n_dec):
        nxt = to_dec[i + 1] if i + 1 < n_dec else None
        last = i == n_dec - 1
        o, rec_ = _dec_block(W, pk, i, x, nxt, train, fuse_eval=fuse_eval,
                             out_skip=needed_patches if (last and tape is None and not train) else None, sync=spec.sync_bn,
                             head=head and last, inorm=spec.dec_inorm,
                             stencil_tail=bool(HEAD_STENCIL and last and tape is None and not train and fuse_eval and not spec.dec_inorm))
        if rec_ is not None and rec_.get("stencil"):
            q = f"{DEC}.{i}"
            weff, beff = ops.head_fold(W[f"{q}.conv.3.weight"], rec_["st2"].scale, rec_["st2"].shift, W["dense_decoder.proj.weight"].view(-1),
                                       W["dense_decoder.proj.bias"])
            B_, D_, H_, W_ = o.shape[:4]
            patches = needed_patches
            if patches is None:
                patches = MaskInfo(torch.ones(B_, D_ // 16, H_ // 16, W_ // 16, device=o.device, dtype=torch.uint8), n_active=B_ * (D_ // 16) * (H_ // 16) * (W_ // 16))
            if l2_of is not None:
                ops.head_stencil(o, weff, beff, patches, inp=l2_of[0], l2=l2_of[1])
                return None
            rec = torch.empty(B_, D_, H_, W_, device=o.device, dtype=torch.float32)
            ops.head_stencil(o, weff, beff, patches, rec=rec)
            return rec
        if head and last:
            st_head = rec_["st2"]
        if tape is not None:
            tape.dec.append({"q": rec_["q"], "xin": x, "nxt": nxt, "head": head and last} if recompute else rec_)
        x = o
    rec = ops.proj_fwd(x, W["dense_decoder.proj.weight"].view(-1), W["dense_decoder.proj.bias"], pre=st_head)
    if tape is not None:
        tape.last = x
    return rec


def forward(spec: Spec, W: Dict[str, torch.Tensor], pk: PackCache, inp: torch.Tensor, mask: MaskInfo, train: bool,
            tape: Optional[Tape] = None, want_feats: bool = False, encoder_only: bool = False, recompute: bool = False,
            want_to_dec0: bool = False, needed_patches: Optional[MaskInfo] = None, l2_out: Optional[torch.Tensor] = None):
    counts = _counts(mask, range(5))
    if tape is not None:
        tape.counts = counts
        tape.recompute = recompute
    feats = encoder_forward(spec, W, pk, inp, mask, counts, tape, recompute)
    if encoder_only:
        return feats
    to_dec = densify_forward(spec, W, pk, feats, mask, counts, tape)
    rec = decoder_forward(spec, W, pk, to_dec, train, tape, recompute, needed_patches, l2_of=(inp, l2_out) if l2_out is not None else None)
    if want_to_dec0:
        return rec, to_dec[0]
    return (rec, feats) if want_feats else rec


FUSED_HEAD = True
_SIDE: Dict[int, "torch.cuda.Stream"] = {}
_SIDE_KEEP: Dict[int, List[torch.Tensor]] = {}
_USE_SIDE = True


def _dev_index(dev) -> int:
    return dev.index if dev.index is not None else torch.cuda.current_device()


def _side_stream(dev) -> "torch.cuda.Stream":
    i = _dev_index(dev)
    if i not in _SIDE:
        _SIDE[i] = torch.cuda.Stream(device=dev)
    return _SIDE[i]


def _on_side(dev, tensors, fn):
    if not _USE_SIDE:
        return fn()
    s2 = _side_stream(dev)
    ev = torch.cuda.Event()
    ev.record()
    s2.wait_event(ev)
    _SIDE_KEEP.setdefault(_dev_index(dev), []).extend(tensors)
    with torch.cuda.stream(s2):
        fn()


def _join_side(dev):
    i = _dev_index(dev)
    if _USE_SIDE and i in _SIDE:
        ev = torch.cuda.Event()
        ev.record(_SIDE[i])
        torch.cuda.current_stream(dev).wait_event(ev)
    _SIDE_KEEP.pop(i, None)


def _wgrad_into(pk: PackCache, G, name, mode, x, dy, k, stride, transposed=False, **masks):
    def run():
        dwp = ops.conv3d_wgrad(mode, x, dy, k, stride, f32_split=pk.f32_split, deterministic=pk.deterministic, **masks)
        ops.unpack_grad(dwp, G[name], transposed, accumulate=True)
    _on_side(x.device, (x, dy), run)


def _dec_block_backward(W, G, pk: PackCache, t: dict, g: Optional[torch.Tensor], drec: Optional[torch.Tensor], bias_sum_into: Optional[torch.Tensor]):
    q = t["q"]
    if t.get("inorm"):
        so = tuple(t["r"].shape[1:4])
        dc2 = _instance_norm_backward(g, t["c2"], t["st2"], ACT_NONE)
        dr = ops.conv3d(CONV_DGRAD, dc2, pk.get(W, f"{q}.conv.3.weight", False, True), None, so, 3, 1)
        _wgrad_into(pk, G, f"{q}.conv.3.weight", CONV_FWD, t["r"], dc2, 3, 1)
        dc1 = _instance_norm_backward(dr, t["c1"], t["st1"], ACT_RELU6)
    elif t.get("head"):
        dc2 = ops.proj_norm_bwd(t["c2"], t["st2"], drec, W["dense_decoder.proj.weight"].view(-1), W[f"{q}.conv.4.weight"],
                                W[f"{q}.conv.4.bias"], G[f"{q}.conv.4.weight"], G[f"{q}.conv.4.bias"],
                                G["dense_decoder.proj.weight"].view(-1), G["dense_decoder.proj.bias"])
    else:
        dc2 = ops.norm_backward(g, None, t["c2"], t["st2"], W[f"{q}.conv.4.weight"], ACT_NONE, None, 0,
                                G[f"{q}.conv.4.weight"], G[f"{q}.conv.4.bias"])
    if not t.get("inorm"):
        so = tuple(t["r"].shape[1:4])
        fuse = ops.FUSED_NORM_BWD_REDUCE and dc2.dtype == torch.bfloat16 and t["st1"].sync_world <= 1 and dc2.shape[-1] >= 128
        dr = ops.conv3d(CONV_DGRAD, dc2, pk.get(W, f"{q}.conv.3.weight", False, True), None, so, 3, 1,
                        norm_bwd=(t["c1"], t["st1"], ACT_RELU6) if fuse else None)
        dr, red1 = dr if fuse else (dr, None)
        _wgrad_into(pk, G, f"{q}.conv.3.weight", CONV_FWD, t["r"], dc2, 3, 1)
        dc1 = ops.norm_backward(dr, None, t["c1"], t["st1"], W[f"{q}.conv.1.weight"], ACT_RELU6, None, 0,
                                G[f"{q}.conv.1.weight"], G[f"{q}.conv.1.bias"], reduced=red1)
    du, ptu = ops.conv3d(CONV_DGRAD, dc1, pk.get(W, f"{q}.conv.0.weight", False, True), None, so, 3, 1, want_partials=True, partials_sum_only=True)
    ptu.finalize(None, sum_accum=G[f"{q}.up_sample.bias"])
    _wgrad_into(pk, G, f"{q}.conv.0.weight", CONV_FWD, t["u"], dc1, 3, 1)
    si = tuple(t["xin"].shape[1:4])
    gin = ops.conv3d(CONVT_DGRAD, du, pk.get(W, f"{q}.up_sample.weight", True, True), None, si, 4, 2, want_partials=bias_sum_into is not None)
    if bias_sum_into is not None:
        gin, ptg = gin
        ptg.finalize(None, sum_accum=bias_sum_into)
    _wgrad_into(pk, G, f"{q}.up_sample.weight", CONVT_FWD, t["xin"], du, 4, 2, transposed=True)
    return gin


def decoder_backward(spec: Spec, W, G, pk: PackCache, tape: Tape, drec: torch.Tensor, after_group=None) -> List[Optional[torch.Tensor]]:
    n_dec = len(spec.dec_chs) - 1
    fused_head = bool(tape.dec[n_dec - 1].get("head"))
    g = None
    if not fused_head:
        g = ops.proj_bwd(tape.last, drec, W["dense_decoder.proj.weight"].view(-1), G["dense_decoder.proj.weight"].view(-1),
                         G["dense_decoder.proj.bias"], deterministic=pk.deterministic)
        if after_group:
            after_group("proj")
    dproj: List[Optional[torch.Tensor]] = [None] * n_dec
    for i in reversed(range(n_dec)):
        t = tape.dec[i]
        if tape.recompute:
            _, t = _dec_block(W, pk, i, t["xin"], t["nxt"], True, update_running=False, sync=spec.sync_bn, head=bool(t.get("head")),
                              inorm=spec.dec_inorm)
            tape.dec[i] = None
        if i + 1 < n_dec:
            dproj[i + 1] = g
        need_sum = i > 0 and f"densify_projs.{i}.bias" in G
        g = _dec_block_backward(W, G, pk, t, g, drec, G[f"densify_projs.{i}.bias"] if need_sum else None)
        if t.get("head") and after_group:
            after_group("proj")
        if after_group:
            after_group(f"dec{i}")
    dproj[0] = g
    return dproj


def densify_backward(spec: Spec, W, G, pk: PackCache, mask: MaskInfo, tape: Tape, dproj) -> List[Optional[torch.Tensor]]:
    n_dec = len(spec.dec_chs) - 1
    dfeat: List[Optional[torch.Tensor]] = [None] * spec.n_stage
    for i in range(n_dec):
        t = tape.dens[i]
        dp = dproj[i]
        if t["k"]:
            pw = f"densify_projs.{i}.weight"
            dd = ops.conv3d(CONV_DGRAD, dp, pk.get(W, pw, False, True), None, tuple(dp.shape[1:4]), t["k"], 1)
            _wgrad_into(pk, G, pw, CONV_FWD, t["d"], dp, t["k"], 1)
            if i == 0:
                ops.chan_sum(dp, None, 0, G[f"densify_projs.{i}.bias"])
        else:
            dd = dp
        dfeat[4 - i] = ops.norm_backward(dd, None, t["f"], t["st"], W[f"densify_norms.{i}.weight"], ACT_NONE, mask, i,
                                         G[f"densify_norms.{i}.weight"], G[f"densify_norms.{i}.bias"],
                                         dtoken=G[f"mask_tokens.{i}"].view(-1), fill=True)
    return dfeat


def _enc_block_backward(W, G, pk: PackCache, inp: torch.Tensor, mask: MaskInfo, t: dict, gout: torch.Tensor, base: Optional[torch.Tensor],
                        free_saved: bool = False) -> Optional[torch.Tensor]:
    p, s = t["p"], t["s"]
    bs = 4 - s
    y2, a1, y1, out, x = t["y2"], t["a1"], t["y1"], t["out"], t["x"]
    dpre = torch.empty_like(y2)
    dy2 = ops.norm_backward(gout, out, y2, t["st2"], W[f"{p}.norm2.weight"], ACT_LRELU, mask, bs,
                            G[f"{p}.norm2.weight"], G[f"{p}.norm2.bias"], dres=dpre,
                            dbeta2=G.get(f"{p}.conv3.bias"), dxsum=G[f"{p}.conv2.bias"])
    sp = tuple(y2.shape[1:4])
    da1 = ops.conv3d(CONV_DGRAD, dy2, pk.get(W, f"{p}.conv2.weight", False, True), None, sp, 3, 1,
                     in_mask=mask, in_bshift=bs, out_mask=mask, out_bshift=bs)
    red1 = None
    _wgrad_into(pk, G, f"{p}.conv2.weight", CONV_FWD, a1, dy2, 3, 1, x_mask=mask, x_bshift=bs, y_mask=mask, y_bshift=bs)
    dy1 = ops.norm_backward(da1, None, y1, t["st1"], W[f"{p}.norm1.weight"], ACT_LRELU, mask, bs,
                            G[f"{p}.norm1.weight"], G[f"{p}.norm1.bias"], dxsum=G[f"{p}.conv1.bias"], reduced=red1)
    stride = t["stride"]
    if s == 0 and t["first"]:
        ops.stem_conv_wgrad(inp, dy1, 3, mask, bs, G[f"{p}.conv1.weight"].view(-1, 27), None, deterministic=pk.deterministic)
        ops.stem_conv_wgrad(inp, dpre, 1, mask, bs, G[f"{p}.conv3.weight"].view(-1, 1), None, deterministic=pk.deterministic)
        return None
    bsx = bs + (1 if stride == 2 else 0)
    spx = tuple(x.shape[1:4])
    _wgrad_into(pk, G, f"{p}.conv1.weight", CONV_FWD, x, dy1, 3, stride, x_mask=mask, x_bshift=bsx, y_mask=mask, y_bshift=bs)
    if free_saved:
        t["y1"] = t["a1"] = t["y2"] = t["out"] = None
    if t["first"]:
        gx = ops.conv3d(CONV_DGRAD, dy1, pk.get(W, f"{p}.conv1.weight", False, True), None, spx, 3, stride,
                        in_mask=mask, in_bshift=bs, out_mask=mask, out_bshift=bsx, out=base, accumulate=base is not None)
        _wgrad_into(pk, G, f"{p}.conv3.weight", CONV_FWD, x, dpre, 1, stride, x_mask=mask, x_bshift=bsx, y_mask=mask, y_bshift=bs)
        ops.conv3d(CONV_DGRAD, dpre, pk.get(W, f"{p}.conv3.weight", False, True), None, spx, 1, stride,
                   in_mask=mask, in_bshift=bs, out_mask=mask, out_bshift=bsx, out=gx, accumulate=True)
        return gx
    gx = ops.conv3d(CONV_DGRAD, dy1, pk.get(W, f"{p}.conv1.weight", False, True), None, spx, 3, 1,
                    in_mask=mask, in_bshift=bs, out_mask=mask, out_bshift=bs)
    return ops.add(gx, dpre, out=gx)


def encoder_backward(spec: Spec, W, G, pk: PackCache, inp: torch.Tensor, mask: MaskInfo, tape: Tape, dfeat, after_group=None):
    counts = tape.counts
    gstage: List[Optional[torch.Tensor]] = list(dfeat)
    by_stage: Dict[int, List[dict]] = {}
    for t in tape.enc:
        by_stage.setdefault(t["s"], []).append(t)
    for s in reversed(range(spec.n_stage)):
        if tape.recompute:
            xs, recs = tape.enc_in[s], []
            for b in range(spec.depth[s]):
                xs, r_ = _enc_block(W, pk, inp, mask, counts, spec.stage_spatial(s), s, b, xs)
                recs.append(r_)
            by_stage[s] = recs
        gout = gstage[s]
        if gout is None:
            gout = torch.zeros_like(by_stage[s][-1]["out"])
        for t in reversed(by_stage[s]):
            gx = _enc_block_backward(W, G, pk, inp, mask, t, gout, gstage[s - 1] if (t["first"] and s > 0) else None, tape.recompute)
            if t["first"] and s > 0:
                gstage[s - 1] = gx
            elif gx is not None:
                gout = gx
            if after_group:
                after_group(f"stage{s}.{t['b']}")
            if gx is None:
                break
    _join_side(inp.device)


def backward(spec: Spec, W: Dict[str, torch.Tensor], G: Dict[str, torch.Tensor], pk: PackCache, inp: torch.Tensor, mask: MaskInfo,
             tape: Tape, drec: torch.Tensor, after_group=None, join_before_hook: bool = True):
    if after_group is not None and join_before_hook:
        user_hook = after_group

        def after_group(tag, _h=user_hook, _dev=inp.device):
            _join_side(_dev)
            _h(tag)
    try:
        dproj = decoder_backward(spec, W, G, pk, tape, drec, after_group)
        dfeat = densify_backward(spec, W, G, pk, mask, tape, dproj)
        if after_group:
            after_group("densify")
        encoder_backward(spec, W, G, pk, inp, mask, tape, dfeat, after_group)
    finally:
        _join_side(inp.device)


NET = ENC.rsplit(".", 1)[0]


def _dense_mask(size: Tuple[int, int, int], device) -> MaskInfo:
    f = tuple(v // 16 for v in size)
    return MaskInfo(torch.ones(1, *f, dtype=torch.uint8, device=device), n_active=f[0] * f[1] * f[2])


def seg_encoder_forward(W, pk: PackCache, inp: torch.Tensor, depth: Sequence[int], mask: Optional[MaskInfo] = None, counts=None) -> List[torch.Tensor]:
    size = tuple(inp.shape[1:])
    if mask is None:
        mask = _dense_mask(size, inp.device)
        counts = _counts(mask, range(5))
    feats, x = [], None
    for s in range(6):
        sp = tuple(v >> min(s, 4) for v in size)
        for b in range(depth[s]):
            x, _ = _enc_block(W, pk, inp, mask, counts, sp, s, b, x, keep=False, stride=1 if s == 5 else None)
        feats.append(x)
    return feats


def seg_forward(W, pk: PackCache, inp: torch.Tensor, depth: Sequence[int], all_levels: bool = False) -> List[torch.Tensor]:
    B = inp.shape[0]
    outs: List[Optional[torch.Tensor]] = [None] * 5
    mask = _dense_mask(tuple(inp.shape[1:]), inp.device)
    counts = _counts(mask, range(5))
    for bi in range(B):
        feats = seg_encoder_forward(W, pk, inp[bi:bi + 1], depth, mask, counts)
        x = feats[5]
        for u in range(5):
            s = 4 - u
            skip = feats[s]
            sp = tuple(skip.shape[1:4])
            wn = f"{NET}.upsample_layers.{u}.conv.weight"
            xu = ops.conv3d(CONV_FWD, x, pk.get(W, wn, False, False), W[f"{NET}.upsample_layers.{u}.conv.bias"], tuple(x.shape[1:4]), 1, 1)
            x = ops.seg_upcat(xu, skip)
            for b in range(depth[s]):
                x, _ = _enc_block(W, pk, None, mask, counts, sp, s, b, x, keep=False, stride=1, prefix=f"{NET}.conv_blocks_localization.{u}")
            if (all_levels or u == 4) and B == 1:
                outs[u] = x
            elif all_levels or u == 4:
                if outs[u] is None:
                    outs[u] = torch.empty(B, *x.shape[1:], device=x.device, dtype=x.dtype)
                outs[u][bi:bi + 1].copy_(x)
    return outs if all_levels else [outs[4]]
```

anatomask_amd/hip.py:

```python
import ctypes as C
import os
import re

_HERE = os.path.dirname(os.path.abspath(__file__))
LIB_PATH = os.path.join(_HERE, "libanatomask_hip.so")
HEADER = os.path.join(os.path.dirname(_HERE), "include", "anatomask_hip.h")

DT_F32, DT_BF16, DT_F32S = 0, 1, 2
CONV_FWD, CONV_DGRAD, CONVT_FWD, CONVT_DGRAD = 0, 1, 2, 3
ACT_NONE, ACT_LRELU, ACT_RELU6 = 0, 1, 2

_CT = {"int": C.c_int, "long": C.c_long, "float": C.c_float, "double": C.c_double}


def declared_functions(header: str = HEADER):
    txt = open(header).read()
    txt = re.sub(r"/\*.*?\*/", " ", txt, flags=re.S)
    out = {}
    for m in re.finditer(r"\bint\s+(am_\w+)\s*\(([^;]*?)\)\s*;", txt, flags=re.S):
        name, args = m.group(1), m.group(2).strip()
        types = []
        if args and args != "void":
            for a in args.split(","):
                a = " ".join(a.split())
                if "*" in a:
                    types.append(C.c_void_p)
                else:
                    types.append(_CT[a.replace("const ", "").split(" ")[0]])
        out[name] = types
    return out


class HipLib:
    ANSWERS = ("am_head_stencil_supported", "am_conv3d_wgrad_uses_k3", "am_conv3d_uses_k3", "am_conv3d_prenorm_supported", "am_version")

    def __init__(self, path: str = LIB_PATH):
        import torch
        if not os.path.exists(path):
            raise RuntimeError(f"{path} not built: run `python -m anatomask_amd.build` (no fallback path exists)")
        if os.path.abspath(path) == LIB_PATH:
            from . import build as _b
            sp = _b.stamp_path(path)
            have = open(sp).read().strip() if os.path.exists(sp) else None
            if have != _b.source_digest():
                raise RuntimeError(f"{path} was not built from the csrc/ + include/ sources next to it (stamp {str(have)[:12]}.. != sources "
                                   f"{_b.source_digest()[:12]}..): run `python -m anatomask_amd.build`")
        self._lib = C.CDLL(path)
        self.functions = declared_functions()
        for name, argtypes in self.functions.items():
            fn = getattr(self._lib, name)
            fn.argtypes = argtypes
            fn.restype = C.c_int
            if name not in self.ANSWERS:
                setattr(self, name[3:], self._wrap(name, fn))

    @staticmethod
    def _wrap(name, fn):
        def call(*args):
            rc = fn(*args)
            if rc != 0:
                raise RuntimeError(f"{name} failed with code {rc}")
        call.__name__ = name
        return call


_LIB = None


def lib() -> HipLib:
    global _LIB
    if _LIB is None:
        _LIB = HipLib()
    return _LIB


def use_library(path: str) -> HipLib:
    global _LIB
    if _LIB is not None:
        raise RuntimeError("use_library() after the library was loaded")
    _LIB = HipLib(path)
    return _LIB
```

anatomask_amd/ops.py:

```python
from __future__ import annotations

from typing import Optional, Tuple

import torch

from . import hip
from .hip import ACT_LRELU, ACT_NONE, ACT_RELU6, CONV_DGRAD, CONV_FWD, CONVT_DGRAD, CONVT_FWD


def _dt(t: torch.Tensor) -> int:
    if t.dtype == torch.float32:
        return hip.DT_F32
    if t.dtype == torch.bfloat16:
        return hip.DT_BF16
    raise TypeError(f"unsupported dtype {t.dtype}")


DEFAULT_F32_SPLIT = False


def _dtc(t: torch.Tensor, f32_split: bool) -> int:
    return hip.DT_F32S if (t.dtype == torch.float32 and f32_split) else _dt(t)


# ... 297 lines not shown
    return hi, lo


def stem_conv_fwd(x_b1: torch.Tensor, w: torch.Tensor, bias: Optional[torch.Tensor], mask: Optional[MaskInfo], bshift: int,
                  dtype: torch.dtype, want_partials: bool = False, out: Optional[torch.Tensor] = None):
    B, D, H, W = x_b1.shape
    Cc, k = w.shape[0], w.shape[2]
    y = torch.empty(B, D, H, W, Cc, device=x_b1.device, dtype=dtype) if out is None else out
    mp, fd, fh, fw = _mk(mask)
    part = None
    if want_partials:
        part = ConvPartials.__new__(ConvPartials)
        part.rows, part.C = B * (D // 4) * (H // 8) * (W // 16), Cc
        part.t = torch.empty(part.rows, Cc, 2, device=x_b1.device, dtype=torch.float32)
    hip.lib().stem_conv_fwd(_dt(y), x_b1.data_ptr(), B, D, H, W, Cc, k, mp, bshift, fd, fh, fw, w.data_ptr(), _p(bias),
                            y.data_ptr(), part.t.data_ptr() if part else None, *_al(mask), _ROWS_ADDR if part else None, _stream())
    if part is not None:
        part.rows = _ROWS_OUT.value
    return (y, part) if want_partials else y


def stem_conv_wgrad(x_b1: torch.Tensor, dy: torch.Tensor, ksize: int, mask: Optional[MaskInfo], bshift: int,
                    dw_accum: torch.Tensor, db_accum: Optional[torch.Tensor], deterministic: Optional[bool] = None):
    B, D, H, W, Cc = dy.shape
    mp, fd, fh, fw = _mk(mask)
    ws = _det_workspace(dy.device, 1024 * Cc * (ksize ** 3 + 1) // 8) if (_det(deterministic) and dy.dtype == torch.bfloat16) else None
    hip.lib().stem_conv_wgrad(_dt(dy), x_b1.data_ptr(), dy.data_ptr(), B, D, H, W, Cc, ksize, mp, bshift, fd, fh, fw,
                              dw_accum.data_ptr(), _p(db_accum), *_al(mask), _p(ws), ws.numel() if ws is not None else 0, _stream())


NREP = 8
DXREP = 64


class NormStats:

    def __init__(self, C: int, device):
        self.sums = torch.empty(NREP, C, 2, device=device, dtype=torch.float64)
        self.nrep = NREP
        self.buf = torch.empty(4, C, device=device, dtype=torch.float32)
        self.mean, self.rstd, self.scale, self.shift = self.buf[0], self.buf[1], self.buf[2], self.buf[3]
        self.count_ptr: Optional[torch.Tensor] = None
        self.count_host: float = 0.0
        self.sync_world: int = 1


def chan_stats(x: torch.Tensor, mask: Optional[MaskInfo], bshift: int, st: NormStats):
    B, D, H, W, Cc = x.shape
    mp, fd, fh, fw = _mk(mask)
    hip.lib().chan_stats(_dt(x), x.data_ptr(), B, D, H, W, Cc, mp, bshift, fd, fh, fw, st.sums.data_ptr(), *_al(mask), _stream())
    st.nrep = NREP


def mask_count(mask: MaskInfo, voxels_per_patch: int, out: torch.Tensor):
    hip.lib().mask_count(mask.t.data_ptr(), mask.t.numel(), voxels_per_patch, out.data_ptr(), _stream())


def norm_finalize(st: NormStats, gamma: torch.Tensor, beta: torch.Tensor, eps: float,
                  run_mean: Optional[torch.Tensor] = None, run_var: Optional[torch.Tensor] = None, momentum: float = 0.1):
    Cc = gamma.numel()
    hip.lib().norm_finalize(st.sums.data_ptr(), st.nrep, _p(st.count_ptr), float(st.count_host), Cc, gamma.data_ptr(), beta.data_ptr(),
                            eps, st.mean.data_ptr(), st.rstd.data_ptr(), st.scale.data_ptr(), st.shift.data_ptr(),
                            _p(run_mean), _p(run_var), momentum, _stream())


def norm_fold_running(st: NormStats, gamma, beta, run_mean, run_var, eps: float):
    hip.lib().norm_fold_running(gamma.numel(), gamma.data_ptr(), beta.data_ptr(), run_mean.data_ptr(), run_var.data_ptr(), eps,
                                st.scale.data_ptr(), st.shift.data_ptr(), _stream())


def norm_apply(x: torch.Tensor, st: NormStats, act: int, mask: Optional[MaskInfo] = None, bshift: int = 0,
               res: Optional[torch.Tensor] = None, stem: Optional[Tuple[torch.Tensor, torch.Tensor, torch.Tensor]] = None,
               fill: Optional[torch.Tensor] = None, out: Optional[torch.Tensor] = None) -> torch.Tensor:
    B, D, H, W, Cc = x.shape
    if out is None:
        out = torch.empty_like(x)
    mp, fd, fh, fw = _mk(mask)
    sx, sw, sb = stem if stem is not None else (None, None, None)
    hip.lib().norm_apply(_dt(x), x.data_ptr(), B, D, H, W, Cc, mp, bshift, fd, fh, fw, st.scale.data_ptr(), st.shift.data_ptr(),
                         act, _p(res), _p(sx), _p(sw), _p(sb), _p(fill), out.data_ptr(), *_al(mask), _stream())
    return out


class NormBwdScratch:
    def __init__(self, C: int, device):
        self.k = torch.empty(3, C, device=device, dtype=torch.float32)


def norm_backward(dout: torch.Tensor, out: Optional[torch.Tensor], x: torch.Tensor, st: NormStats, gamma: torch.Tensor, act: int,
                  mask: Optional[MaskInfo], bshift: int, dgamma: Optional[torch.Tensor], dbeta: Optional[torch.Tensor],
                  dtoken: Optional[torch.Tensor] = None, fill: bool = False, dx: Optional[torch.Tensor] = None,
                  dres: Optional[torch.Tensor] = None, scratch: Optional[NormBwdScratch] = None,
                  dbeta2: Optional[torch.Tensor] = None, dxsum: Optional[torch.Tensor] = None,
                  reduced: Optional[ConvPartials] = None) -> torch.Tensor:
    B, D, H, W, Cc = x.shape
    sc = scratch or NormBwdScratch(Cc, x.device)
    mp, fd, fh, fw = _mk(mask)
    L = hip.lib()
    s = _stream()
    ws_b, ws_x = _bwd_workspaces(x.device, Cc)
    if reduced is not None:
        assert st.sync_world <= 1 and out is None and dtoken is None and not fill
        reduced.finalize_bwd(st, gamma, sc, dgamma, dbeta, dbeta2)
        if dx is None:
            dx = torch.empty_like(x)
        L.norm_bwd_apply(_dt(x), dout.data_ptr(), None, x.data_ptr(), B, D, H, W, Cc, mp, bshift, fd, fh, fw,
                         st.mean.data_ptr(), st.rstd.data_ptr(), sc.k[0].data_ptr(), sc.k[1].data_ptr(), sc.k[2].data_ptr(), act,
                         dx.data_ptr(), _p(dres), _p(dxsum), ws_x.data_ptr(), st.scale.data_ptr(), st.shift.data_ptr(), *_al(mask), 1, s)
        return dx
    if st.sync_world > 1:
        import torch.distributed as dist
        L.norm_bwd_reduce(_dt(x), dout.data_ptr(), _p(out), x.data_ptr(), B, D, H, W, Cc, mp, bshift, fd, fh, fw,
                          st.mean.data_ptr(), st.rstd.data_ptr(), act, int(fill), ws_b.data_ptr(), st.scale.data_ptr(), st.shift.data_ptr(),
                          *_al(mask), None, 0.0, None, None, None, None, None, None, None, None, s)
        L.norm_bwd_finalize(ws_b.data_ptr(), None, float(st.count_host), Cc, gamma.data_ptr(), st.rstd.data_ptr(),
                            sc.k[0].data_ptr(), sc.k[1].data_ptr(), sc.k[2].data_ptr(), _p(dgamma), _p(dbeta), _p(dtoken), _p(dbeta2), s)
        dist.all_reduce(ws_b[:NREP * Cc * 3])
        L.norm_bwd_finalize(ws_b.data_ptr(), None, float(st.count_host), Cc, gamma.data_ptr(), st.rstd.data_ptr(),
                            sc.k[0].data_ptr(), sc.k[1].data_ptr(), sc.k[2].data_ptr(), None, None, None, None, s)
        ws_b[:NREP * Cc * 3].zero_()
        if dx is None:
            dx = torch.empty_like(x)
        L.norm_bwd_apply(_dt(x), dout.data_ptr(), _p(out), x.data_ptr(), B, D, H, W, Cc, mp, bshift, fd, fh, fw,
                         st.mean.data_ptr(), st.rstd.data_ptr(), sc.k[0].data_ptr(), sc.k[1].data_ptr(), sc.k[2].data_ptr(), act,
                         dx.data_ptr(), _p(dres), _p(dxsum), ws_x.data_ptr(), st.scale.data_ptr(), st.shift.data_ptr(), *_al(mask), 1, s)
        return dx
    if not FUSED_BWD_TAILS:
        L.norm_bwd_reduce(_dt(x), dout.data_ptr(), _p(out), x.data_ptr(), B, D, H, W, Cc, mp, bshift, fd, fh, fw,
                          st.mean.data_ptr(), st.rstd.data_ptr(), act, int(fill), ws_b.data_ptr(), st.scale.data_ptr(), st.shift.data_ptr(),
                          *_al(mask), None, 0.0, None, None, None, None, None, None, None, None, s)
        L.norm_bwd_finalize(ws_b.data_ptr(), _p(st.count_ptr), float(st.count_host), Cc, gamma.data_ptr(), st.rstd.data_ptr(),
                            sc.k[0].data_ptr(), sc.k[1].data_ptr(), sc.k[2].data_ptr(), _p(dgamma), _p(dbeta), _p(dtoken), _p(dbeta2), s)
        ws_b[:NREP * Cc * 3].zero_()
        if dx is None:
            dx = torch.empty_like(x)
        L.norm_bwd_apply(_dt(x), dout.data_ptr(), _p(out), x.data_ptr(), B, D, H, W, Cc, mp, bshift, fd, fh, fw,
                         st.mean.data_ptr(), st.rstd.data_ptr(), sc.k[0].data_ptr(), sc.k[1].data_ptr(), sc.k[2].data_ptr(), act,
                         dx.data_ptr(), _p(dres), _p(dxsum), ws_x.data_ptr(), st.scale.data_ptr(), st.shift.data_ptr(), *_al(mask), 0, s)
        if dxsum is not None:
            ws_x[:DXREP * Cc].zero_()
        return dx
    L.norm_bwd_reduce(_dt(x), dout.data_ptr(), _p(out), x.data_ptr(), B, D, H, W, Cc, mp, bshift, fd, fh, fw,
                      st.mean.data_ptr(), st.rstd.data_ptr(), act, int(fill), ws_b.data_ptr(), st.scale.data_ptr(), st.shift.data_ptr(),
                      *_al(mask), _p(st.count_ptr), float(st.count_host), gamma.data_ptr(), sc.k[0].data_ptr(), sc.k[1].data_ptr(),
                      sc.k[2].data_ptr(), _p(dgamma), _p(dbeta), _p(dtoken), _p(dbeta2), s)
    if dx is None:
        dx = torch.empty_like(x)
    L.norm_bwd_apply(_dt(x), dout.data_ptr(), _p(out), x.data_ptr(), B, D, H, W, Cc, mp, bshift, fd, fh, fw,
                     st.mean.data_ptr(), st.rstd.data_ptr(), sc.k[0].data_ptr(), sc.k[1].data_ptr(), sc.k[2].data_ptr(), act,
                     dx.data_ptr(), _p(dres), _p(dxsum), ws_x.data_ptr(), st.scale.data_ptr(), st.shift.data_ptr(), *_al(mask), 1, s)
    return dx


_BWS = {}
FUSED_BWD_TAILS = True
FUSED_NORM_BWD_REDUCE = False


def _bwd_workspaces(device, C: int):
    key = (device, torch.cuda.current_stream(device).cuda_stream)
    ws = _BWS.get(key)
    if ws is None or ws[2] < C:
        cap = max(C, 2048)
        ws = _BWS[key] = (torch.zeros(NREP * cap * 3 + 2, device=device, dtype=torch.float64),
                          torch.zeros(DXREP * cap + 2, device=device, dtype=torch.float64), cap)
    return ws[0], ws[1]


def chan_sum(x: torch.Tensor, mask: Optional[MaskInfo], bshift: int, out_accum: torch.Tensor):
    B, D, H, W, Cc = x.shape
    mp, fd, fh, fw = _mk(mask)
    hip.lib().chan_sum(_dt(x), x.data_ptr(), B, D, H, W, Cc, mp, bshift, fd, fh, fw, out_accum.data_ptr(), _stream())


def add(a: torch.Tensor, b: torch.Tensor, out: Optional[torch.Tensor] = None) -> torch.Tensor:
    if out is None:
        out = torch.empty_like(a)
    hip.lib().add(_dt(a), a.data_ptr(), b.data_ptr(), out.data_ptr(), a.numel(), _stream())
    return out


def proj_fwd(x: torch.Tensor, w: torch.Tensor, b: torch.Tensor, pre: Optional["NormStats"] = None) -> torch.Tensor:
    B, D, H, W, Cc = x.shape
    rec = torch.empty(B, D, H, W, device=x.device, dtype=torch.float32)
    hip.lib().proj_fwd(_dt(x), x.data_ptr(), B * D * H * W, Cc, w.data_ptr(), b.data_ptr(), _p(pre.scale) if pre else None,
                       _p(pre.shift) if pre else None, rec.data_ptr(), _stream())
    return rec


def proj_norm_bwd(x: torch.Tensor, st: "NormStats", drec: torch.Tensor, w: torch.Tensor, gamma: torch.Tensor, beta: torch.Tensor,
                  dgamma: torch.Tensor, dbeta: torch.Tensor, dw_accum: torch.Tensor, db_accum: torch.Tensor) -> torch.Tensor:
    B, D, H, W, Cc = x.shape
    assert st.sync_world <= 1
    dx = torch.empty_like(x)
    ws_b, _ = _bwd_workspaces(x.device, Cc)
    coef = torch.empty(3, Cc, device=x.device, dtype=torch.float32)
    hip.lib().proj_norm_bwd(_dt(x), x.data_ptr(), drec.data_ptr(), B * D * H * W, Cc, w.data_ptr(), gamma.data_ptr(), beta.data_ptr(),
                            st.mean.data_ptr(), st.rstd.data_ptr(), st.scale.data_ptr(), ws_b.data_ptr(), coef.data_ptr(), dx.data_ptr(),
                            dgamma.data_ptr(), dbeta.data_ptr(), dw_accum.data_ptr(), db_accum.data_ptr(), _stream())
    return dx


def proj_bwd(x: torch.Tensor, drec: torch.Tensor, w: torch.Tensor, dw_accum: torch.Tensor, db_accum: torch.Tensor,
             deterministic: Optional[bool] = None) -> torch.Tensor:
    B, D, H, W, Cc = x.shape
    dx = torch.empty_like(x)
    ws = _det_workspace(x.device, 4096 * (Cc + 1) // 8) if _det(deterministic) else None
    hip.lib().proj_bwd(_dt(x), x.data_ptr(), drec.data_ptr(), B * D * H * W, Cc, w.data_ptr(), dx.data_ptr(), dw_accum.data_ptr(),
                       db_accum.data_ptr(), _p(ws), ws.numel() if ws is not None else 0, _stream())
    return dx


def head_stencil_supported(x: torch.Tensor) -> bool:
    B, D, H, W, C = x.shape
    ok = hip.lib()._lib.am_head_stencil_supported(_dt(x), C) == 1
    return bool(ok and D % 16 == 0 and H % 16 == 0 and W % 16 == 0 and max(B, D // 16, H // 16, W // 16) <= 255)


def head_fold(w2: torch.Tensor, scale: torch.Tensor, shift: torch.Tensor, wproj: torch.Tensor, bproj: torch.Tensor):
    cmid, cin = w2.shape[0], w2.shape[1]
    assert tuple(w2.shape[2:]) == (3, 3, 3) and w2.is_contiguous() and wproj.numel() == cmid
    weff = torch.empty(27, cin, device=w2.device, dtype=torch.float32)
    beff = torch.empty(1, device=w2.device, dtype=torch.float32)
    hip.lib().head_fold(w2.data_ptr(), cmid, cin, scale.data_ptr(), shift.data_ptr(), wproj.data_ptr(), bproj.data_ptr(), weff.data_ptr(),
                        beff.data_ptr(), _stream())
    return weff, beff


def head_stencil(r: torch.Tensor, weff: torch.Tensor, beff: torch.Tensor, patches: MaskInfo, rec: Optional[torch.Tensor] = None,
                 inp: Optional[torch.Tensor] = None, l2: Optional[torch.Tensor] = None):
    B, D, H, W, C = r.shape
    lst, n = patches.active_list()
    assert lst is not None and (patches.fd, patches.fh, patches.fw) == (D // 16, H // 16, W // 16) and r.is_contiguous()
    assert rec is None or (rec.dtype == torch.float32 and tuple(rec.shape) == (B, D, H, W) and rec.is_contiguous())
    assert l2 is None or (inp is not None and l2.dtype == torch.float32 and l2.numel() == B * patches.fd * patches.fh * patches.fw)
    hip.lib().head_stencil(_dt(r), r.data_ptr(), B, D, H, W, C, weff.data_ptr(), beff.data_ptr(), lst.data_ptr(), n, _p(rec), _p(inp), _p(l2), _stream())


def patch_loss_fwd(inp: torch.Tensor, rec: torch.Tensor, mask: MaskInfo, normalized: bool, want_loss: bool = True):
    B, D, H, W = inp.shape
    L = mask.fd * mask.fh * mask.fw
    l2m = torch.empty(B, L, device=inp.device, dtype=torch.float32)
    pm = torch.empty(B, L, device=inp.device, dtype=torch.float32) if want_loss else None
    pr = torch.empty(B, L, device=inp.device, dtype=torch.float32) if want_loss else None
    info = torch.empty(2, device=inp.device, dtype=torch.float32) if want_loss else None
    hip.lib().patch_loss_fwd(inp.data_ptr(), rec.data_ptr(), mask.t.data_ptr(), B, D, H, W, int(normalized), l2m.data_ptr(),
                             _p(pm), _p(pr), _p(info), _stream())
    return l2m, pm, pr, info


def patch_loss_bwd(inp, rec, mask: MaskInfo, pm, pr, info, gout: Optional[torch.Tensor]) -> torch.Tensor:
    B, D, H, W = inp.shape
    drec = torch.empty_like(rec)
    hip.lib().patch_loss_bwd(inp.data_ptr(), rec.data_ptr(), mask.t.data_ptr(), B, D, H, W, pm.data_ptr(), pr.data_ptr(),
                             info.data_ptr(), _p(gout), drec.data_ptr(), _stream())
    return drec


def mask_sampler(loss: torch.Tensor, keys: torch.Tensor, len_keep: int, len_loss: int) -> torch.Tensor:
    B, L = loss.shape
    out = torch.empty(B, L, device=loss.device, dtype=torch.uint8)
    hip.lib().mask_sampler(loss.data_ptr(), keys.data_ptr(), B, L, len_keep, len_loss, out.data_ptr(), _stream())
    return out


def sumsq(g: torch.Tensor, out: torch.Tensor):
    hip.lib().sumsq(g.data_ptr(), g.numel(), out.data_ptr(), _stream())


def adamw_ema(p, g, m, v, ema, n, lr, betas, eps, wd, step, sumsq_t, max_norm, ema_decay, gnorm_out, grad_scale: float = 1.0, dyn=None,
              guard: Optional[torch.Tensor] = None):
    assert guard is None or (guard.dtype == torch.int32 and guard.numel() >= 4)
    hip.lib().adamw_ema(p.data_ptr(), g.data_ptr(), m.data_ptr(), v.data_ptr(), _p(ema), n, lr, betas[0], betas[1], eps, wd, step,
                        _p(sumsq_t), max_norm, ema_decay, grad_scale, _p(gnorm_out), _p(dyn), _p(guard), _stream())


def adam_dyn_scalars(lr: float, betas, step: int, ema_decay: float):
    import math
    return [float(lr), 1.0 - betas[0] ** step, math.sqrt(1.0 - betas[1] ** step), float(ema_decay)]


def ema(ema_t: torch.Tensor, p: torch.Tensor, decay: float, guard: Optional[torch.Tensor] = None):
    hip.lib().ema(ema_t.data_ptr(), p.data_ptr(), p.numel(), decay, _p(guard), _stream())


def ema_i64(ema_t: torch.Tensor, p: torch.Tensor, decay: float, guard: Optional[torch.Tensor] = None):
    assert ema_t.dtype == p.dtype == torch.int64 and ema_t.numel() == p.numel() and ema_t.is_contiguous() and p.is_contiguous()
    hip.lib().ema_i64(ema_t.data_ptr(), p.data_ptr(), p.numel(), decay, _p(guard), _stream())


def guard_restore(dst: torch.Tensor, snapshot: torch.Tensor, guard: torch.Tensor):
    assert dst.dtype == snapshot.dtype and dst.numel() == snapshot.numel() and dst.is_contiguous() and snapshot.is_contiguous()
    hip.lib().guard_restore(dst.data_ptr(), snapshot.data_ptr(), dst.numel() * dst.element_size(), guard.data_ptr(), _stream())


def spline_prefilter(vol: torch.Tensor):
    assert vol.dtype == torch.float32 and vol.dim() == 3 and vol.is_contiguous()
    hip.lib().spline_prefilter(vol.data_ptr(), *vol.shape, _stream())
    return vol


def resample_affine(src: torch.Tensor, dst: torch.Tensor, affine_3x4, order: int, cval: float = 0.0):
    assert src.dtype == dst.dtype == torch.float32 and src.is_contiguous() and dst.is_contiguous()
    arr = (_ct.c_float * 12)(*[float(v) for v in affine_3x4])
    hip.lib().resample_affine(src.data_ptr(), *src.shape, dst.data_ptr(), *dst.shape, _ct.addressof(arr), int(order), float(cval), _stream())
    return dst
# ... 99 lines not shown
```

include/anatomask_hip.h:

```cpp
#ifndef ANATOMASK_HIP_H
#define ANATOMASK_HIP_H
#include <stdint.h>
#ifdef __cplusplus
extern "C" {
#endif

#define AM_DT_F32 0
#define AM_DT_BF16 1
#define AM_DT_F32S 2

#define AM_CONV_PARTIALS_SUM_ONLY 2
#define AM_CONV_FWD 0
#define AM_CONV_DGRAD 1
#define AM_CONVT_FWD 2
#define AM_CONVT_DGRAD 3

#define AM_DXREP 64
#define AM_NREP 8

#define AM_ACT_NONE 0
#define AM_ACT_LRELU 1
#define AM_ACT_RELU6 2

int am_version(void);

int am_conv3d(int mode, int dtype, int ksize, int stride, const void* x, const void* w_packed, const float* bias, void* y,
              int B, int Di, int Hi, int Wi, int Cin, int Do, int Ho, int Wo, int Cout,
              const uint8_t* in_mask, int in_bshift, const uint8_t* out_mask, int out_bshift, int fd, int fh, int fw,
              int accumulate, float* partials ,
              const float* ep_scale, const float* ep_shift ,
              const void* ep_res ,
              int ep_act ,
              const int32_t* active_list, int n_active ,
              int* partial_rows_written ,
              void* stream);
int am_conv3d_prenorm_supported(int mode, int dtype, int ksize, int stride, int B, int Do, int Ho, int Wo, int Cin, int Cout, int sparse,
                                int in_bshift, int out_bshift, int n_active);
int am_conv3d_prenorm(int mode, int dtype, int ksize, int stride, const void* x, const void* w_packed, const float* bias, void* y, int B, int Di,
                      int Hi, int Wi, int Cin, int Do, int Ho, int Wo, int Cout, const uint8_t* mask, int in_bshift, int out_bshift, int fd,
                      int fh, int fw, float* partials , const float* in_scale, const float* in_shift, int in_act,
                      const int32_t* active_list, int n_active, int* partial_rows_written , void* stream);

int am_conv3d_nbred(int mode, int dtype, int ksize, int stride, const void* x, const void* w_packed, void* y, int B, int Di,
                    int Hi, int Wi, int Cin, int Do, int Ho, int Wo, int Cout, const uint8_t* in_mask, int in_bshift,
                    const uint8_t* out_mask, int out_bshift, int fd, int fh, int fw, int accumulate, float* partials,
                    const void* nb_x, const float* nb_scale, const float* nb_shift, int nb_act,
                    int* partial_rows_written, void* stream);
int am_packed_dims(int dtype, int rows, int k, int* rows_padded, int* k_padded);
int am_conv3d_partials_rows(int mode, int dtype, int ksize, int stride, int B, int Do, int Ho, int Wo, int Cin, int Cout,
                            int out_sparse, int out_bshift ,
                            int n_active, int* rows );
int am_conv3d_uses_k3(int mode, int dtype, int ksize, int stride, int B, int Di, int Hi, int Wi, int Cin, int Do, int Ho, int Wo, int Cout,
                      int has_masks, int accumulate, int fused_epilogue, int want_partials);
int am_partials_reduce(const float* partials, int rows, int C, double* sums, float* sum_accum, void* stream);

int am_conv3d_wgrad(int mode, int dtype, int ksize, int stride, const void* x, const void* dy, float* dw_packed,
                    int B, int Dx, int Hx, int Wx, int Cx, int Dy, int Hy, int Wy, int Cy,
                    const uint8_t* x_mask, int x_bshift, const uint8_t* y_mask, int y_bshift, int fd, int fh, int fw,
                    float* det_workspace, long det_workspace_floats,
                    const int32_t* active_list, int n_active ,
                    void* gather_workspace, long gather_workspace_bytes ,
                    void* stream);
int am_conv3d_wgrad_uses_k3(int mode, int dtype, int ksize, int stride, int B, int D, int H, int W, int Cx, int Cy, int has_masks,
                            int deterministic);
int am_conv3d_wgrad_gather_bytes(int mode, int dtype, int ksize, int stride, int B, int Cx, int Cy, int y_bshift, int has_y_mask, int n_active,
                                 int fd, int fh, int fw, long* bytes );

int am_split_bf16(const float* x, void* hi, void* lo, long n, void* stream);

int am_pack_weight(int dtype, const float* src, void* dst, int R, int K, int taps, long stride_r, long stride_k, int Rp, int Kp,
                   void* stream);
typedef struct am_pack_desc {
  const float* src; void* dst; long stride_r, stride_k; int R, K, taps, Rp, Kp, first_block;
} am_pack_desc;
int am_pack_weights_batched(int dtype, const am_pack_desc* descs, int ndesc, int total_blocks, void* stream);
int am_unpack_grad(const float* src_packed, float* dst, int R, int K, int taps, long stride_r, long stride_k, int accumulate,
                   void* stream);

int am_stem_conv_fwd(int dtype, const float* x, int B, int D, int H, int W, int C, int ksize, const uint8_t* mask, int bshift,
                     int fd, int fh, int fw, const float* w, const float* bias, void* y,
                     float* partials ,
                     const int32_t* active_list, int n_active ,
                     int* partial_rows_written , void* stream);
int am_stem_conv_wgrad(int dtype, const float* x, const void* dy, int B, int D, int H, int W, int C, int ksize,
                       const uint8_t* mask, int bshift, int fd, int fh, int fw, float* dw_accum, float* db_accum,
                       const int32_t* active_list, int n_active ,
                       float* det_workspace, long det_workspace_floats ,
                       void* stream);

int am_chan_stats(int dtype, const void* x, int B, int D, int H, int W, int C, const uint8_t* mask, int bshift, int fd, int fh,
                  int fw, double* sums ,
                  const int32_t* active_list, int n_active ,
                  void* stream);
int am_mask_count(const uint8_t* mask, int n, int voxels_per_patch, double* out, void* stream);
int am_mask_compact(const uint8_t* mask, int B, int fd, int fh, int fw, int32_t* list, int32_t* count, void* stream);
int am_norm_finalize(const double* sums, int nrep , const double* count_ptr, double count_host, int C, const float* gamma,
                     const float* beta, float eps, float* mean, float* rstd, float* scale, float* shift,
                     float* run_mean , float* run_var, float momentum, void* stream);
#define AM_FIN_REP 16
int am_partials_finalize(const float* partials, int rows, int C, double* workspace, const double* count_ptr, double count_host,
                         const float* gamma, const float* beta, float eps, float* mean, float* rstd, float* scale, float* shift,
                         float* run_mean, float* run_var, float momentum, long* num_batches_tracked, float* sum_accum, void* stream);
int am_norm_bwd_from_partials(const float* partials, int rows, int C, double* workspace, const double* count_ptr, double count_host,
                              const float* gamma, const float* mean, const float* rstd, float* k0, float* k1, float* k2,
                              float* dgamma, float* dbeta, float* dbeta2, void* stream);
int am_norm_fold_running(int C, const float* gamma, const float* beta, const float* run_mean, const float* run_var, float eps,
                         float* scale, float* shift, void* stream);
int am_norm_apply(int dtype, const void* x, int B, int D, int H, int W, int C, const uint8_t* mask, int bshift, int fd, int fh,
                  int fw, const float* scale, const float* shift, int act, const void* res, const float* stem_x,
                  const float* stem_w, const float* stem_b, const float* fill, void* y,
                  const int32_t* active_list, int n_active, void* stream);
int am_norm_bwd_reduce(int dtype, const void* dout, const void* out, const void* x, int B, int D, int H, int W, int C,
                       const uint8_t* mask, int bshift, int fd, int fh, int fw, const float* mean, const float* rstd, int act,
                       int fill, double* bsum ,
                       const float* pre_scale, const float* pre_shift ,
                       const int32_t* active_list, int n_active,
                       const double* count_ptr, double count_host, const float* gamma, float* k0, float* k1, float* k2,
                       float* dgamma_accum, float* dbeta_accum, float* dtoken_accum, float* dbeta2_accum
                       ,
                       void* stream);
int am_norm_bwd_finalize(const double* bsum, const double* count_ptr, double count_host, int C, const float* gamma,
                         const float* rstd, float* k0, float* k1, float* k2, float* dgamma_accum, float* dbeta_accum,
                         float* dtoken_accum, float* dbeta2_accum , void* stream);
int am_norm_bwd_apply(int dtype, const void* dout, const void* out, const void* x, int B, int D, int H, int W, int C,
                      const uint8_t* mask, int bshift, int fd, int fh, int fw, const float* mean, const float* rstd,
                      const float* k0, const float* k1, const float* k2, int act, void* dx, void* dres,
                      float* dxsum_accum ,
                      double* dxsum_scratch ,
                      const float* pre_scale, const float* pre_shift ,
                      const int32_t* active_list, int n_active,
                      int scratch_is_zero_workspace , void* stream);
int am_chan_sum(int dtype, const void* x, int B, int D, int H, int W, int C, const uint8_t* mask, int bshift, int fd, int fh,
                int fw, float* out_accum, void* stream);
int am_add(int dtype, const void* a, const void* b, void* y, long n_elems, void* stream);

int am_head_fold(const float* w2, int cmid, int cin, const float* scale, const float* shift, const float* wproj, const float* bproj,
                 float* weff, float* beff, void* stream);
int am_head_stencil(int dtype, const void* r, int B, int D, int H, int W, int C, const float* weff, const float* beff,
                    const int32_t* patch_list, int n_patches, float* rec , const float* inp ,
                    float* l2 , void* stream);
int am_head_stencil_supported(int dtype, int C);

int am_proj_fwd(int dtype, const void* x, long nvox, int C, const float* w, const float* b,
                const float* pre_scale, const float* pre_shift , float* rec, void* stream);
int am_proj_norm_bwd(int dtype, const void* x, const float* drec, long nvox, int C, const float* w, const float* gamma, const float* beta,
                     const float* mean, const float* rstd, const float* scale, double* workspace, float* coef, void* dx,
                     float* dgamma_accum, float* dbeta_accum, float* dw_accum, float* db_accum, void* stream);
int am_proj_bwd(int dtype, const void* x, const float* drec, long nvox, int C, const float* w, void* dx, float* dw_accum,
                float* db_accum, float* det_workspace, long det_workspace_floats , void* stream);

int am_patch_loss_fwd(const float* inp, const float* rec, const uint8_t* active, int B, int D, int H, int W, int normalized,
                      float* l2m, float* pmean, float* prstd, float* lossinfo, void* stream);
int am_patch_loss_bwd(const float* inp, const float* rec, const uint8_t* active, int B, int D, int H, int W, const float* pmean,
                      const float* prstd, const float* lossinfo, const float* gout, float* drec, void* stream);

int am_mask_sampler(const float* loss, const float* keys, int B, int L, int len_keep, int len_loss, uint8_t* mask, void* stream);

int am_sumsq(const float* g, long n, double* out, void* stream);
int am_adamw_ema(float* p, const float* g, float* m, float* v, float* ema , long n, double lr, double beta1,
                 double beta2, double eps, double weight_decay, int step, const double* sumsq ,
                 double max_norm, double ema_decay, double grad_scale ,
                 float* gnorm_out,
                 const float* dyn_scalars ,
                 int* guard ,
                 void* stream);
int am_ema(float* ema, const float* p, long n, double decay, const int* guard , void* stream);
int am_ema_i64(long* ema, const long* p, int n, double decay, const int* guard, void* stream);
int am_guard_restore(void* dst, const void* snapshot, long nbytes, const int* guard, void* stream);

int am_spline_prefilter(float* vol, int D, int H, int W, void* stream);
int am_resample_affine(const float* src, int Ds, int Hs, int Ws, float* dst, int D, int H, int W, const float* affine_host12, int order,
                       float cval, void* stream);


#define AM_LAYER_REP 64
int am_voxel_norm_fwd(int dtype, int kind, const void* x, void* y, int B, int D, int H, int W, int C, int groups, const float* gamma,
                      const float* beta, float eps, const uint8_t* mask, int bshift, const int32_t* active_list, int n_active, void* stream);
int am_voxel_norm_bwd(int dtype, int kind, const void* x, const void* dy, void* dx, int B, int D, int H, int W, int C, int groups,
                      const float* gamma, float eps, float* dgamma_accum, float* dbeta_accum, const uint8_t* mask, int bshift,
                      const int32_t* active_list, int n_active, void* stream);

int am_pool3d_fwd(int dtype, int op, const void* x, void* y, int32_t* argmax, int B, int Di, int Hi, int Wi, int C, int ksize, int stride,
                  int pad, int dilation, int count_include_pad, int Do, int Ho, int Wo, const uint8_t* mask, int in_bshift, int out_bshift,
                  int fd, int fh, int fw, const int32_t* active_list, int n_active, void* stream);
int am_pool3d_bwd(int dtype, int op, const void* dy, const int32_t* argmax, void* dx, int B, int Di, int Hi, int Wi, int C, int ksize,
                  int stride, int pad, int dilation, int count_include_pad, int Do, int Ho, int Wo, const uint8_t* mask, int in_bshift,
                  int out_bshift, int fd, int fh, int fw, const int32_t* active_list, int n_active, void* stream);

int am_dwconv3d(int dtype, int data_grad, const void* x, const float* w, const float* bias, void* y, int B, int D, int H, int W, int C,
                int ksize, const uint8_t* mask, int bshift, int fd, int fh, int fw, void* stream);
int am_dwconv3d_wgrad(int dtype, const void* x, const void* dy, float* dw_accum, float* db_accum, int B, int D, int H, int W, int C, int ksize,
                      const uint8_t* mask, int bshift, int fd, int fh, int fw, void* stream);

int am_dwconv3d_s2(int dtype, int data_grad, const void* src, const float* w, const float* bias, void* dst, int B, int Df, int Hf, int Wf,
                   int C, int ksize, const uint8_t* mask, int fine_bshift, int fd, int fh, int fw, const int32_t* active_list, int n_active,
                   void* stream);
int am_dwconv3d_s2_wgrad(int dtype, const void* x, const void* dy, float* dw_accum, float* db_accum, int B, int Df, int Hf, int Wf, int C,
                         int ksize, const uint8_t* mask, int fine_bshift, int fd, int fh, int fw, const int32_t* active_list, int n_active,
                         void* stream);

int am_gelu(int dtype, const void* x, const void* dy, void* out, int B, int D, int H, int W, int C, const uint8_t* mask, int bshift,
            const int32_t* active_list, int n_active, void* stream);
int am_scale_residual(int dtype, int backward, const void* x, const void* other, const float* gamma, void* out, float* dgamma_accum, int B, int D,
                      int H, int W, int C, const uint8_t* mask, int bshift, const int32_t* active_list, int n_active, void* stream);

int am_masked_mean_fwd(int dtype, const void* x, float* mean, int B, int D, int H, int W, int C, const uint8_t* mask, int bshift, int fd, int fh,
                       int fw, void* stream);
int am_masked_mean_bwd(int dtype, const float* dmean, const float* count, void* dx, int B, int D, int H, int W, int C, const uint8_t* mask,
                       int bshift, const int32_t* active_list, int n_active, void* stream);

int am_seg_gather(const float* vol, int X, int Y, int Z, int o0, int o1, int o2, int T0, int T1, int T2, int axes, float* out, void* stream);
int am_seg_upcat(int dtype, const void* u, const void* skip, void* y, int B, int D, int H, int W, int C, int factor, void* stream);
#define AM_SEG_LDS_C 240
int am_seg_head(int dtype, const void* f, int B, int D, int H, int W, int C, const float* w, const float* bias, int K, float* logits,
                void* stream);
int am_seg_head_accumulate(int dtype, const void* f, int axes, int T0, int T1, int T2, int C, const float* w, const float* bias, int K,
                           const float* gauss, float* acc, float* wsum, int X, int Y, int Z, int s0, int s1, int s2, void* stream);
int am_seg_finalize(const float* acc, const float* wsum, int K, int Xp, int Yp, int Zp, int c0, int c1, int c2, int X, int Y, int Z,
                    float* logits, void* labels, int label_bytes, void* stream);
#define AM_SEG_SOFTMAX 0
#define AM_SEG_SIGMOID 1
int am_seg_export(const float* acc, const float* wsum, int K, int Xp, int Yp, int Zp, int c0, int c1, int c2, int X, int Y, int Z, int nonlin,
                  const int32_t* region_order, float* probs, void* labels, int label_bytes, void* stream);

#ifdef __cplusplus
}
#endif
#endif
```

Before: 136.9 volumes/s.

## Fuse stem block backward: recompute residual 1x1 conv and fold norm bwd into wgrad

Adds a fused backward path for the first stem block. The norm2 backward recomputes the residual 1x1 stem conv output on the fly from the input and weights instead of reading a stored tensor, and it accumulates that conv's weight gradient in the same pass. The norm1 backward apply is folded into the conv1 MFMA weight-gradient kernel, which converts dy to dx in registers before staging it into LDS and reduces the dx channel sums with a last-workgroup ticket. This removes separate elementwise kernels and the round trips of intermediate dres/dx tensors through memory. In exchange it adds kernel template variants, extra per-voxel loads of the stem input, and more register pressure in the wgrad kernel.

```diff
diff --git a/anatomask_amd/csrc/stream_ops.hip b/anatomask_amd/csrc/stream_ops.hip
--- a/anatomask_amd/csrc/stream_ops.hip
+++ b/anatomask_amd/csrc/stream_ops.hip
@@ -182,13 +182,16 @@
   float *k0, *k1, *k2, *dgamma, *dbeta, *dtoken, *dbeta2;
 };
 
+__device__ __forceinline__ bool last_workgroup(unsigned* ticket, unsigned* tk) {
+  asm volatile("s_waitcnt vmcnt(0)" ::: "memory");
+  __syncthreads();
+  if (threadIdx.x == 0) *tk = atomicAdd(ticket, 1u);
+  __syncthreads();
+  return *tk == gridDim.x - 1;
+}
 __device__ __forceinline__ bool last_workgroup(unsigned* ticket) {
   __shared__ unsigned tk;
-  asm volatile("s_waitcnt vmcnt(0)" ::: "memory");
-  __syncthreads();
-  if (threadIdx.x == 0) tk = atomicAdd(ticket, 1u);
-  __syncthreads();
-  return tk == gridDim.x - 1;
+  return last_workgroup(ticket, &tk);
 }
 
 __device__ __forceinline__ void bwd_reduce_tail(double* bsum, int C, const BwdFin& f) {
@@ -214,16 +217,48 @@
 }
 
 constexpr double AM_DX_FIX = 68719476736.0;
-__device__ __forceinline__ void dxsum_tail(double* rep, int nrep, int C, float* accum, unsigned* ticket) {
-  if (!ticket) return;
-  if (!last_workgroup(ticket)) return;
+__device__ __forceinline__ void dxsum_add(double* rep, int c, float v) {
+  atomicAdd((unsigned long long*)&rep[c], (unsigned long long)__double2ll_rn((double)v * AM_DX_FIX));
+}
+__device__ __forceinline__ void dxsum_fold(double* rep, int nrep, int C, float* accum) {
   for (int c = threadIdx.x; c < C; c += blockDim.x) {
     long long s_ = 0;
     for (int r = 0; r < nrep; ++r) s_ += (long long)atomicExch((unsigned long long*)&rep[(size_t)r * C + c], 0ull);
     accum[c] += (float)((double)s_ / AM_DX_FIX);
   }
+}
+__device__ __forceinline__ void dxsum_tail(double* rep, int nrep, int C, float* accum, unsigned* ticket) {
+  if (!ticket) return;
+  if (!last_workgroup(ticket)) return;
+  dxsum_fold(rep, nrep, C, accum);
   if (threadIdx.x == 0) atomicExch(ticket, 0u);
 }
+
+template <int EPC> struct BwdCoef {
+  float mu[EPC], rs[EPC], c0[EPC], c1[EPC], c2[EPC], qs[EPC], qh[EPC];
+};
+template <int EPC> __device__ __forceinline__ void gate_pre_chunk(float (&d)[EPC], const float (&f)[EPC], const BwdCoef<EPC>& k, int actv) {
+#pragma unroll
+  for (int i = 0; i < EPC; ++i) d[i] *= act_grad_pre(f[i] * k.qs[i] + k.qh[i], actv);
+}
+template <int EPC> __device__ __forceinline__ void gate_stem_chunk(float (&d)[EPC], const float (&f)[EPC], const BwdCoef<EPC>& k,
+                                                                   const float (&sw)[EPC], float xv, int actv) {
+#pragma unroll
+  for (int i = 0; i < EPC; ++i) {
+    float o = f[i] * k.qs[i] + k.qh[i];
+    o += sw[i] * xv;
+    d[i] *= act_grad_pre(o, actv);
+  }
+}
+template <int EPC> __device__ __forceinline__ void dx_chunk(const float (&d)[EPC], const float (&f)[EPC], const BwdCoef<EPC>& k, float (&r)[EPC]) {
+#pragma unroll
+  for (int i = 0; i < EPC; ++i) r[i] = k.c0[i] * d[i] - k.c1[i] - k.c2[i] * (f[i] - k.mu[i]) * k.rs[i];
+}
+
+struct StemGate {
+  const float *x, *w, *b;
+  double* wsum; float* dw_accum;
+};
 
 template <typename T, int NT = 256, int ACT_ = -1, int OUT_ = 0>
 __global__ __launch_bounds__(NT) void norm_bwd_reduce_kernel(const T* __restrict__ dout, const T* __restrict__ out,
@@ -530,27 +565,30 @@
   }
 }
 
-template <typename T, int ACT_ = -1, int OUT_ = 0>
+template <typename T, int ACT_ = -1, int OUT_ = 0, int STEM = 0>
 __global__ __launch_bounds__(256) void norm_bwd_reduce_rows_kernel(const T* __restrict__ dout, const T* __restrict__ out,
                                                                    const T* __restrict__ x, RowGeo g, const float* __restrict__ mean,
                                                                    const float* __restrict__ rstd, int act, double* __restrict__ bsum,
-                                                                   const float* __restrict__ psc, const float* __restrict__ psh, BwdFin fin) {
+                                                                   const float* __restrict__ psc, const float* __restrict__ psh, BwdFin fin,
+                                                                   StemGate sg) {
   constexpr int EPC = TT<T>::EPC;
   const int actv = ACT_ >= 0 ? ACT_ : act;
   const bool has_out = ACT_ >= 0 ? OUT_ != 0 : out != nullptr;
   __shared__ float red[256 * 2 * 8];
   RowWalk<T> wk(g);
-  float s1[EPC], s2[EPC], mu[EPC], rs[EPC], qs[EPC], qh[EPC];
-#pragma unroll
-  for (int i = 0; i < EPC; ++i) { s1[i] = s2[i] = 0.f; mu[i] = rs[i] = qs[i] = qh[i] = 0.f; }
+  float s1[EPC], s2[EPC], mu[EPC], rs[EPC], sw[EPC];
+  BwdCoef<EPC> kc;
+#pragma unroll
+  for (int i = 0; i < EPC; ++i) { s1[i] = s2[i] = 0.f; mu[i] = rs[i] = kc.qs[i] = kc.qh[i] = sw[i] = 0.f; }
   if (wk.live) {
 #pragma unroll
     for (int i = 0; i < EPC; ++i) {
       mu[i] = mean[wk.cl * EPC + i]; rs[i] = rstd[wk.cl * EPC + i];
-      if (!has_out && actv != AM_ACT_NONE) { qs[i] = psc[wk.cl * EPC + i]; qh[i] = psh[wk.cl * EPC + i]; }
+      if (!has_out && actv != AM_ACT_NONE) { kc.qs[i] = psc[wk.cl * EPC + i]; kc.qh[i] = psh[wk.cl * EPC + i]; }
+      if (STEM) { sw[i] = sg.w[wk.cl * EPC + i]; kc.qh[i] += sg.b[wk.cl * EPC + i]; }
     }
     for (long rw = wk.row; rw < wk.row_end; rw += (long)UNR * wk.rpp) {
-      long v[UNR]; u32x4 dv[UNR], xv[UNR], ov[UNR];
+      long v[UNR]; u32x4 dv[UNR], xv[UNR], ov[UNR]; float sx[UNR];
 #pragma unroll
       for (int u = 0; u < UNR; ++u) { const long r = rw + (long)u * wk.rpp; v[u] = r < wk.row_end ? wk.voxel(g, r) : -1; }
 #pragma unroll
@@ -559,6 +597,7 @@
         const size_t off = (size_t)v[u] * g.C + wk.cl * EPC;
         dv[u] = *(const u32x4*)(dout + off); xv[u] = *(const u32x4*)(x + off);
         if (has_out && actv != AM_ACT_NONE) ov[u] = *(const u32x4*)(out + off);
+        if (STEM) sx[u] = sg.x[v[u]];
       }
 #pragma unroll
       for (int u = 0; u < UNR; ++u) {
@@ -571,9 +610,10 @@
             chunk_to_f<T>(ov[u], o);
 #pragma unroll
             for (int i = 0; i < EPC; ++i) d[i] *= act_grad(o[i], actv);
+          } else if (STEM) {
+            gate_stem_chunk<EPC>(d, f, kc, sw, sx[u], actv);
           } else {
-#pragma unroll
-            for (int i = 0; i < EPC; ++i) d[i] *= act_grad_pre(f[i] * qs[i] + qh[i], actv);
+            gate_pre_chunk<EPC>(d, f, kc, actv);
           }
         }
 #pragma unroll
@@ -604,32 +644,34 @@
   bwd_reduce_tail(bsum, g.C, fin);
 }
 
-template <typename T, int ACT_ = -1, int OUT_ = 0>
+template <typename T, int ACT_ = -1, int OUT_ = 0, int STEM = 0>
 __global__ __launch_bounds__(256) void norm_bwd_apply_rows_kernel(const T* __restrict__ dout, const T* __restrict__ out,
                                                                   const T* __restrict__ x, RowGeo g, const float* __restrict__ mean,
                                                                   const float* __restrict__ rstd, const float* __restrict__ k0,
                                                                   const float* __restrict__ k1, const float* __restrict__ k2, int act,
                                                                   T* __restrict__ dx, T* __restrict__ dres, double* __restrict__ dxsum,
                                                                   int dxrep, const float* __restrict__ psc, const float* __restrict__ psh,
-                                                                  float* __restrict__ dx_accum, unsigned* dx_ticket) {
+                                                                  float* __restrict__ dx_accum, unsigned* dx_ticket, StemGate sg) {
   constexpr int EPC = TT<T>::EPC;
   const int actv = ACT_ >= 0 ? ACT_ : act;
   const bool has_out = ACT_ >= 0 ? OUT_ != 0 : out != nullptr;
   __shared__ float red[256 * 8];
   RowWalk<T> wk(g);
-  float mu[EPC], rs[EPC], c0[EPC], c1[EPC], c2[EPC], sx[EPC], qs[EPC], qh[EPC];
+  BwdCoef<EPC> kc;
+  float sx[EPC], sw[EPC], sdw[EPC];
 #pragma unroll
   for (int i = 0; i < EPC; ++i) {
     const int c = wk.cl * EPC + i;
-    sx[i] = 0.f; qs[i] = qh[i] = 0.f;
+    sx[i] = 0.f; kc.qs[i] = kc.qh[i] = 0.f; sw[i] = sdw[i] = 0.f;
     if (wk.live) {
-      mu[i] = mean[c]; rs[i] = rstd[c]; c0[i] = k0[c]; c1[i] = k1[c]; c2[i] = k2[c];
-      if (!has_out && actv != AM_ACT_NONE) { qs[i] = psc[c]; qh[i] = psh[c]; }
+      kc.mu[i] = mean[c]; kc.rs[i] = rstd[c]; kc.c0[i] = k0[c]; kc.c1[i] = k1[c]; kc.c2[i] = k2[c];
+      if (!has_out && actv != AM_ACT_NONE) { kc.qs[i] = psc[c]; kc.qh[i] = psh[c]; }
+      if (STEM) { sw[i] = sg.w[c]; kc.qh[i] += sg.b[c]; }
     }
   }
   if (wk.live)
     for (long rw = wk.row; rw < wk.row_end; rw += (long)UNR * wk.rpp) {
-      long v[UNR]; u32x4 dv[UNR], xv[UNR], ov[UNR];
+      long v[UNR]; u32x4 dv[UNR], xv[UNR], ov[UNR]; float xs[UNR];
 #pragma unroll
       for (int u = 0; u < UNR; ++u) { const long r = rw + (long)u * wk.rpp; v[u] = r < wk.row_end ? wk.voxel(g, r) : -1; }
 #pragma unroll
@@ -638,6 +680,7 @@
         const size_t off = (size_t)v[u] * g.C + wk.cl * EPC;
         dv[u] = *(const u32x4*)(dout + off); xv[u] = *(const u32x4*)(x + off);
         if (has_out && actv != AM_ACT_NONE) ov[u] = *(const u32x4*)(out + off);
+        if (STEM) xs[u] = sg.x[v[u]];
       }
 #pragma unroll
       for (int u = 0; u < UNR; ++u) {
@@ -651,15 +694,21 @@
             chunk_to_f<T>(ov[u], o);
 #pragma unroll
             for (int i = 0; i < EPC; ++i) d[i] *= act_grad(o[i], actv);
+          } else if (STEM) {
+            gate_stem_chunk<EPC>(d, f, kc, sw, xs[u], actv);
           } else {
-#pragma unroll
-            for (int i = 0; i < EPC; ++i) d[i] *= act_grad_pre(f[i] * qs[i] + qh[i], actv);
+            gate_pre_chunk<EPC>(d, f, kc, actv);
           }
         }
         if (dres) *(u32x4*)(dres + off) = f_to_chunk<T>(d);
+        if (STEM) {
+          float q[EPC];
+          chunk_to_f<T>(f_to_chunk<T>(d), q);
+#pragma unroll
+          for (int i = 0; i < EPC; ++i) sdw[i] += xs[u] * q[i];
+        }
         float r[EPC];
-#pragma unroll
-        for (int i = 0; i < EPC; ++i) r[i] = c0[i] * d[i] - c1[i] - c2[i] * (f[i] - mu[i]) * rs[i];
+        dx_chunk<EPC>(d, f, kc, r);
         const u32x4 pk = f_to_chunk<T>(r);
         *(u32x4*)(dx + off) = pk;
         if (dxsum) {
@@ -671,22 +720,31 @@
       }
     }
   if (dxsum) {
-#pragma unroll
-    for (int i = 0; i < EPC; ++i) red[threadIdx.x * 8 + i] = sx[i];
-    __syncthreads();
     const int nlane = blockDim.x / wk.cpv;
-    if (threadIdx.x < wk.cpv) {
-      float a1[EPC];
-#pragma unroll
-      for (int i = 0; i < EPC; ++i) a1[i] = 0.f;
-      for (int vl = 0; vl < nlane; ++vl)
-#pragma unroll
-        for (int i = 0; i < EPC; ++i) a1[i] += red[(vl * wk.cpv + threadIdx.x) * 8 + i];
-#pragma unroll
-      for (int i = 0; i < EPC; ++i)
-        atomicAdd((unsigned long long*)&dxsum[(size_t)(blockIdx.x % dxrep) * g.C + threadIdx.x * EPC + i], (unsigned long long)__double2ll_rn((double)a1[i] * AM_DX_FIX));
-    }
-    dxsum_tail(dxsum, dxrep, g.C, dx_accum, dx_ticket);
+#pragma unroll
+    for (int pass = 0; pass < (STEM ? 2 : 1); ++pass) {
+      if (pass) __syncthreads();
+#pragma unroll
+      for (int i = 0; i < EPC; ++i) red[threadIdx.x * 8 + i] = pass ? sdw[i] : sx[i];
+      __syncthreads();
+      if (threadIdx.x < wk.cpv) {
+        float a1[EPC];
+#pragma unroll
+        for (int i = 0; i < EPC; ++i) a1[i] = 0.f;
+        for (int vl = 0; vl < nlane; ++vl)
+#pragma unroll
+          for (int i = 0; i < EPC; ++i) a1[i] += red[(vl * wk.cpv + threadIdx.x) * 8 + i];
+#pragma unroll
+        for (int i = 0; i < EPC; ++i) dxsum_add(pass ? sg.wsum : dxsum, (blockIdx.x % dxrep) * g.C + threadIdx.x * EPC + i, a1[i]);
+      }
+    }
+    if (!STEM) {
+      dxsum_tail(dxsum, dxrep, g.C, dx_accum, dx_ticket);
+    } else if (last_workgroup(dx_ticket)) {
+      dxsum_fold(dxsum, dxrep, g.C, dx_accum);
+      dxsum_fold(sg.wsum, dxrep, g.C, sg.dw_accum);
+      if (threadIdx.x == 0) atomicExch(dx_ticket, 0u);
+    }
   }
 }
 
@@ -980,20 +1038,38 @@
   return __builtin_amdgcn_ds_read_tr16_b64_v4i16((__attribute__((address_space(3))) s16x4*)(p));
 }
 
-template <int NS, int K>
+struct WgradPre {
+  const bf16_t* y;
+  const float *mean, *rstd, *k0, *k1, *k2, *scale, *shift;
+  double* dxsum; float* dx_accum; unsigned* ticket;
+};
+
+template <int NS, int K, int PRE = 0>
 __global__ __launch_bounds__(256) void stem_wgrad_mfma_kernel(const float* __restrict__ x, const bf16_t* __restrict__ dy, int D, int H, int W,
                                                               MaskView mask, const int* __restrict__ plist, int n_active,
-                                                              float* __restrict__ dw, float* __restrict__ db, float* __restrict__ det_ws) {
+                                                              float* __restrict__ dw, float* __restrict__ db, float* __restrict__ det_ws,
+                                                              WgradPre pre) {
   constexpr int E = 18, C = 16 * NS, RS = 2 * C + 32;
   constexpr int NTT = K == 3 ? 2 : 1, NTAP = K * K * K;
   constexpr int XB = (E * E * E + 8) * 4;
   constexpr int CPV = C / 8, NLD = CPV;
+  static_assert(!PRE || 256 % CPV == 0, "PRE: one channel chunk per thread");
   extern __shared__ __attribute__((aligned(16))) unsigned char lds[];
   float* xl = (float*)lds;
   unsigned char* yl = lds + XB;
   const int tid = threadIdx.x, lane = tid & 63, wave = tid >> 6, g = lane >> 4, r16 = lane & 15;
   const int q = (lane >> 2) & 3, p = lane & 3;
   typedef __attribute__((ext_vector_type(8))) __bf16 bfx8;
+  BwdCoef<8> kc;
+  float sx[8];
+  if (PRE) {
+#pragma unroll
+    for (int i = 0; i < 8; ++i) {
+      const int c = (tid % CPV) * 8 + i;
+      kc.mu[i] = pre.mean[c]; kc.rs[i] = pre.rstd[c]; kc.c0[i] = pre.k0[c]; kc.c1[i] = pre.k1[c]; kc.c2[i] = pre.k2[c];
+      kc.qs[i] = pre.scale[c]; kc.qh[i] = pre.shift[c]; sx[i] = 0.f;
+    }
+  }
   f32x4 acc[NS][NTT];
 #pragma unroll
   for (int i = 0; i < NS; ++i)
@@ -1018,13 +1094,14 @@
         v = x[((size_t)(b * D + id) * H + ih) * W + iw];
       xl[e] = v;
     }
-    u32x4 ld[NLD];
+    u32x4 ld[NLD], ly[PRE ? NLD : 1];
     auto load_plane = [&](int dz) {
 #pragma unroll
       for (int it = 0; it < NLD; ++it) {
         const int idx = tid + it * 256, vox = idx / CPV, ch = idx % CPV;
         const size_t gv = ((size_t)(b * D + d0 + dz) * H + h0 + (vox >> 4)) * W + w0 + (vox & 15);
         ld[it] = *(const u32x4*)(dy + gv * C + ch * 8);
+        if (PRE) ly[it] = *(const u32x4*)(pre.y + gv * C + ch * 8);
       }
     };
     load_plane(0);
@@ -1033,6 +1110,16 @@
 #pragma unroll
       for (int it = 0; it < NLD; ++it) {
         const int idx = tid + it * 256, vox = idx / CPV, ch = idx % CPV;
+        if (PRE) {
+          float d[8], f[8], r[8], rq[8];
+          chunk_to_f<bf16_t>(ld[it], d); chunk_to_f<bf16_t>(ly[it], f);
+          gate_pre_chunk<8>(d, f, kc, AM_ACT_LRELU);
+          dx_chunk<8>(d, f, kc, r);
+          ld[it] = f_to_chunk<bf16_t>(r);
+          chunk_to_f<bf16_t>(ld[it], rq);
+#pragma unroll
+          for (int i = 0; i < 8; ++i) sx[i] += rq[i];
+        }
         *(u32x4*)(yl + vox * RS + ch * 16) = ld[it];
       }
       load_plane(dz < 15 ? dz + 1 : 15);
@@ -1086,6 +1173,26 @@
     if (det_ws) det_ws[(size_t)blockIdx.x * (C * (NTAP + 1)) + i] = v;
     else if (t < NTAP) atomicAdd(&dw[c * NTAP + t], v);
     else if (db) atomicAdd(&db[c], v);
+  }
+  if (PRE) {
+    __syncthreads();
+#pragma unroll
+    for (int i = 0; i < 8; ++i) red[tid * 8 + i] = sx[i];
+    __syncthreads();
+    if (tid < CPV) {
+      float a1[8];
+#pragma unroll
+      for (int i = 0; i < 8; ++i) a1[i] = 0.f;
+      for (int vl = 0; vl < 256 / CPV; ++vl)
+#pragma unroll
+        for (int i = 0; i < 8; ++i) a1[i] += red[(vl * CPV + tid) * 8 + i];
+#pragma unroll
+      for (int i = 0; i < 8; ++i) dxsum_add(pre.dxsum, (blockIdx.x % AM_DXREP) * C + tid * 8 + i, a1[i]);
+    }
+    if (last_workgroup(pre.ticket, (unsigned*)(lds + 256 * 8 * 4))) {
+      dxsum_fold(pre.dxsum, AM_DXREP, C, pre.dx_accum);
+      if (tid == 0) atomicExch(pre.ticket, 0u);
+    }
   }
 }
 
@@ -1750,7 +1857,7 @@
       using T = typename decltype(t)::type;
       am_by_act(act, out != nullptr, [&](auto a, auto o) {
         AM_LAUNCH((norm_bwd_reduce_rows_kernel<T, a, o>), dim3(rows_blocks(rg)), dim3(rows_threads(rg)), 0, st, (const T*)dout, (const T*)out, (const T*)x, rg,
-                  mean, rstd, act, bsum, pre_scale, pre_shift, fin);
+                  mean, rstd, act, bsum, pre_scale, pre_shift, fin, StemGate{});
       });
     });
     AM_CHECK_LAUNCH();
@@ -1803,7 +1910,7 @@
       using T = typename decltype(t)::type;
       am_by_act(act, out != nullptr, [&](auto a, auto o) {
         AM_LAUNCH((norm_bwd_apply_rows_kernel<T, a, o>), dim3(nb), dim3(rows_threads(rg)), 0, st, (const T*)dout, (const T*)out, (const T*)x, rg, mean, rstd,
-                  k0, k1, k2, act, (T*)dx, (T*)dres, dxs, nrep, pre_scale, pre_shift, dx_accum, dx_ticket);
+                  k0, k1, k2, act, (T*)dx, (T*)dres, dxs, nrep, pre_scale, pre_shift, dx_accum, dx_ticket, StemGate{});
       });
     });
   } else {
@@ -1900,7 +2007,7 @@
       am_by_int<1, 3>(ksize, [&](auto k) {
         constexpr auto kern = stem_wgrad_mfma_kernel<ns, k>;
         if ((optin = am_lds_optin<kern>()) != hipSuccess) return;
-        AM_LAUNCH(kern, dim3(nwg), dim3(256), sm, st, x, (const bf16_t*)dy, D, H, W, mv, active_list, n_active, dw_accum, db_accum, det_workspace);
+        AM_LAUNCH(kern, dim3(nwg), dim3(256), sm, st, x, (const bf16_t*)dy, D, H, W, mv, active_list, n_active, dw_accum, db_accum, det_workspace, WgradPre{});
       });
     });
     AM_HIP(optin);
@@ -1920,6 +2027,74 @@
     using T = typename decltype(t)::type;
     AM_LAUNCH(stem_conv_wgrad_kernel<T>, dim3(nb), dim3(256), sm, st, x, (const T*)dy, g, ksize, dw_accum, db_accum);
   });
+  AM_CHECK_LAUNCH();
+  return 0;
+}
+
+static bool stem_bwd_geo(RowGeo& rg, bool reduction, int B, int D, int H, int W, int C, int bshift, const int32_t* active_list, int n_active) {
+  if (bshift != 4 || (C != 32 && C != 64) || !active_list || n_active <= 0) return false;
+  return mkrows(rg, AM_DT_BF16, reduction, B, D, H, W, C, bshift, active_list, n_active);
+}
+
+int am_stem_bwd_supported(int dtype, int B, int D, int H, int W, int C, int bshift, int n_active) {
+  RowGeo rg;
+  static const int32_t some_list = 0;
+  return dtype == AM_DT_BF16 && stem_bwd_geo(rg, false, B, D, H, W, C, bshift, &some_list, n_active) ? 1 : 0;
+}
+
+int am_stem_norm_bwd_reduce(const void* dout, const void* x, int B, int D, int H, int W, int C, int bshift, const int32_t* active_list,
+                            int n_active, const float* stem_x, const float* stem_w, const float* stem_b, const float* mean,
+                            const float* rstd, const float* scale, const float* shift, double* workspace, const double* count_ptr,
+                            double count_host, const float* gamma, float* k0, float* k1, float* k2, float* dgamma, float* dbeta,
+                            float* dbeta2, void* stream) {
+  RowGeo rg;
+  if (!stem_bwd_geo(rg, true, B, D, H, W, C, bshift, active_list, n_active)) return -2;
+  if (!stem_x || !stem_w || !stem_b || !scale || !shift || !gamma || !k0 || !k1 || !k2) return -1;
+  BwdFin fin{};
+  fin.ticket = (unsigned*)(workspace + (size_t)3 * C * NREP);
+  fin.count_ptr = count_ptr; fin.count_host = count_host; fin.gamma = gamma; fin.rstd = rstd;
+  fin.k0 = k0; fin.k1 = k1; fin.k2 = k2; fin.dgamma = dgamma; fin.dbeta = dbeta; fin.dbeta2 = dbeta2;
+  const StemGate sg{stem_x, stem_w, stem_b, nullptr, nullptr};
+  AM_LAUNCH((norm_bwd_reduce_rows_kernel<bf16_t, AM_ACT_LRELU, 0, 1>), dim3(rows_blocks(rg)), dim3(rows_threads(rg)), 0, (hipStream_t)stream,
+            (const bf16_t*)dout, (const bf16_t*)nullptr, (const bf16_t*)x, rg, mean, rstd, AM_ACT_LRELU, workspace, scale, shift, fin, sg);
+  AM_CHECK_LAUNCH();
+  return 0;
+}
+
+int am_stem_norm_bwd_apply(const void* dout, const void* x, int B, int D, int H, int W, int C, int bshift, const int32_t* active_list,
+                           int n_active, const float* stem_x, const float* stem_w, const float* stem_b, const float* mean,
+                           const float* rstd, const float* k0, const float* k1, const float* k2, const float* scale, const float* shift,
+                           void* dx, float* dxsum_accum, float* stem_dw_accum, double* workspace, void* stream) {
+  RowGeo rg;
+  if (!stem_bwd_geo(rg, false, B, D, H, W, C, bshift, active_list, n_active)) return -2;
+  if (!stem_x || !stem_w || !stem_b || !scale || !shift || !dx || !dxsum_accum || !stem_dw_accum || !workspace) return -1;
+  const StemGate sg{stem_x, stem_w, stem_b, workspace + (size_t)AM_DXREP * C, stem_dw_accum};
+  AM_LAUNCH((norm_bwd_apply_rows_kernel<bf16_t, AM_ACT_LRELU, 0, 1>), dim3(rows_blocks(rg)), dim3(rows_threads(rg)), 0, (hipStream_t)stream,
+            (const bf16_t*)dout, (const bf16_t*)nullptr, (const bf16_t*)x, rg, mean, rstd, k0, k1, k2, AM_ACT_LRELU, (bf16_t*)dx,
+            (bf16_t*)nullptr, workspace, AM_DXREP, scale, shift, dxsum_accum, (unsigned*)(workspace + (size_t)2 * AM_DXREP * C), sg);
+  AM_CHECK_LAUNCH();
+  return 0;
+}
+
+int am_stem_conv_wgrad_norm(const float* x, const void* dout, const void* y, int B, int D, int H, int W, int C, const uint8_t* mask,
+                            int bshift, int fd, int fh, int fw, const int32_t* active_list, int n_active, const float* mean,
+                            const float* rstd, const float* k0, const float* k1, const float* k2, const float* scale, const float* shift,
+                            float* dw_accum, float* dxsum_accum, double* workspace, void* stream) {
+  RowGeo rg;
+  if (!mask || D % 16 || H % 16 || W % 16 || !stem_bwd_geo(rg, false, B, D, H, W, C, bshift, active_list, n_active)) return -2;
+  if (!dw_accum || !dxsum_accum || !workspace || !mean || !rstd || !k0 || !k1 || !k2 || !scale || !shift) return -1;
+  const MaskView mv{mask, fd, fh, fw, bshift};
+  const int nwg = n_active < 512 ? n_active : 512;
+  const size_t sm = (size_t)(18 * 18 * 18 + 8) * 4 + (size_t)256 * (2 * C + 32);
+  const WgradPre pre{(const bf16_t*)y, mean, rstd, k0, k1, k2, scale, shift, workspace, dxsum_accum, (unsigned*)(workspace + (size_t)AM_DXREP * C)};
+  hipError_t optin = hipSuccess;
+  am_by_int<2, 4>(C / 16, [&](auto ns) {
+    constexpr auto kern = stem_wgrad_mfma_kernel<ns, 3, 1>;
+    if ((optin = am_lds_optin<kern>()) != hipSuccess) return;
+    AM_LAUNCH(kern, dim3(nwg), dim3(256), sm, (hipStream_t)stream, x, (const bf16_t*)dout, D, H, W, mv, active_list, n_active, dw_accum,
+              (float*)nullptr, (float*)nullptr, pre);
+  });
+  AM_HIP(optin);
   AM_CHECK_LAUNCH();
   return 0;
 }
diff --git a/anatomask_amd/engine.py b/anatomask_amd/engine.py
--- a/anatomask_amd/engine.py
+++ b/anatomask_amd/engine.py
@@ -377,6 +377,7 @@
 
 
 FUSED_HEAD = True
+FUSED_STEM_BWD = True
 _SIDE: Dict[int, "torch.cuda.Stream"] = {}
 _SIDE_KEEP: Dict[int, List[torch.Tensor]] = {}
 _USE_SIDE = True
@@ -510,6 +511,17 @@
     p, s = t["p"], t["s"]
     bs = 4 - s
     y2, a1, y1, out, x = t["y2"], t["a1"], t["y1"], t["out"], t["x"]
+    if FUSED_STEM_BWD and s == 0 and t["first"] and not pk.deterministic and ops.stem_bwd_supported(y2, mask, bs, t["st1"], t["st2"]):
+        dy2 = ops.stem_norm2_backward(gout, y2, t["st2"], W[f"{p}.norm2.weight"], (inp, W[f"{p}.conv3.weight"].view(-1), W[f"{p}.conv3.bias"]),
+                                      mask, bs, G[f"{p}.norm2.weight"], G[f"{p}.norm2.bias"], G[f"{p}.conv3.bias"], G[f"{p}.conv2.bias"],
+                                      G[f"{p}.conv3.weight"].view(-1))
+        sp = tuple(y2.shape[1:4])
+        da1 = ops.conv3d(CONV_DGRAD, dy2, pk.get(W, f"{p}.conv2.weight", False, True), None, sp, 3, 1,
+                         in_mask=mask, in_bshift=bs, out_mask=mask, out_bshift=bs)
+        _wgrad_into(pk, G, f"{p}.conv2.weight", CONV_FWD, a1, dy2, 3, 1, x_mask=mask, x_bshift=bs, y_mask=mask, y_bshift=bs)
+        ops.stem_conv_wgrad_norm(inp, da1, y1, t["st1"], W[f"{p}.norm1.weight"], mask, bs, G[f"{p}.norm1.weight"], G[f"{p}.norm1.bias"],
+                                 G[f"{p}.conv1.bias"], G[f"{p}.conv1.weight"].view(-1, 27))
+        return None
     dpre = torch.empty_like(y2)
     dy2 = ops.norm_backward(gout, out, y2, t["st2"], W[f"{p}.norm2.weight"], ACT_LRELU, mask, bs,
                             G[f"{p}.norm2.weight"], G[f"{p}.norm2.bias"], dres=dpre,
diff --git a/anatomask_amd/hip.py b/anatomask_amd/hip.py
--- a/anatomask_amd/hip.py
+++ b/anatomask_amd/hip.py
@@ -32,7 +32,7 @@
 
 
 class HipLib:
-    ANSWERS = ("am_head_stencil_supported", "am_conv3d_wgrad_uses_k3", "am_conv3d_uses_k3", "am_conv3d_prenorm_supported", "am_version")
+    ANSWERS = ("am_head_stencil_supported", "am_conv3d_wgrad_uses_k3", "am_conv3d_uses_k3", "am_conv3d_prenorm_supported", "am_stem_bwd_supported", "am_version")
 
     def __init__(self, path: str = LIB_PATH):
         import torch
diff --git a/anatomask_amd/ops.py b/anatomask_amd/ops.py
--- a/anatomask_amd/ops.py
+++ b/anatomask_amd/ops.py
@@ -473,6 +473,55 @@
     return dx
 
 
+def stem_bwd_supported(y: torch.Tensor, mask: Optional[MaskInfo], bshift: int, st1: NormStats, st2: NormStats) -> bool:
+    if mask is None or y.dtype != torch.bfloat16 or not FUSED_BWD_TAILS or st1.sync_world > 1 or st2.sync_world > 1:
+        return False
+    lst, n = mask.active_list()
+    if lst is None or n <= 0:
+        return False
+    B, D, H, W, Cc = y.shape
+    return hip.lib()._lib.am_stem_bwd_supported(_dt(y), B, D, H, W, Cc, bshift, n) == 1
+
+
+def stem_norm2_backward(dout: torch.Tensor, y2: torch.Tensor, st: NormStats, gamma: torch.Tensor,
+                        stem: Tuple[torch.Tensor, torch.Tensor, torch.Tensor], mask: MaskInfo, bshift: int, dgamma: torch.Tensor,
+                        dbeta: torch.Tensor, dbeta2: Optional[torch.Tensor], dxsum: torch.Tensor, stem_dw: torch.Tensor) -> torch.Tensor:
+    B, D, H, W, Cc = y2.shape
+    sc = NormBwdScratch(Cc, y2.device)
+    L = hip.lib()
+    s = _stream()
+    ws_b, ws_x = _bwd_workspaces(y2.device, Cc)
+    al = _al(mask)
+    sx, sw, sb = stem
+    L.stem_norm_bwd_reduce(dout.data_ptr(), y2.data_ptr(), B, D, H, W, Cc, bshift, *al, sx.data_ptr(), sw.data_ptr(), sb.data_ptr(),
+                           st.mean.data_ptr(), st.rstd.data_ptr(), st.scale.data_ptr(), st.shift.data_ptr(), ws_b.data_ptr(),
+                           _p(st.count_ptr), float(st.count_host), gamma.data_ptr(), sc.k[0].data_ptr(), sc.k[1].data_ptr(),
+                           sc.k[2].data_ptr(), dgamma.data_ptr(), dbeta.data_ptr(), _p(dbeta2), s)
+    dx = torch.empty_like(y2)
+    L.stem_norm_bwd_apply(dout.data_ptr(), y2.data_ptr(), B, D, H, W, Cc, bshift, *al, sx.data_ptr(), sw.data_ptr(), sb.data_ptr(),
+                          st.mean.data_ptr(), st.rstd.data_ptr(), sc.k[0].data_ptr(), sc.k[1].data_ptr(), sc.k[2].data_ptr(),
+                          st.scale.data_ptr(), st.shift.data_ptr(), dx.data_ptr(), dxsum.data_ptr(), stem_dw.data_ptr(), ws_x.data_ptr(), s)
+    return dx
+
+
+def stem_conv_wgrad_norm(x_b1: torch.Tensor, dout: torch.Tensor, y1: torch.Tensor, st: NormStats, gamma: torch.Tensor, mask: MaskInfo,
+                         bshift: int, dgamma: torch.Tensor, dbeta: torch.Tensor, dxsum: torch.Tensor, dw_accum: torch.Tensor):
+    B, D, H, W, Cc = y1.shape
+    sc = NormBwdScratch(Cc, y1.device)
+    mp, fd, fh, fw = _mk(mask)
+    L = hip.lib()
+    s = _stream()
+    ws_b, ws_x = _bwd_workspaces(y1.device, Cc)
+    al = _al(mask)
+    L.norm_bwd_reduce(_dt(y1), dout.data_ptr(), None, y1.data_ptr(), B, D, H, W, Cc, mp, bshift, fd, fh, fw,
+                      st.mean.data_ptr(), st.rstd.data_ptr(), ACT_LRELU, 0, ws_b.data_ptr(), st.scale.data_ptr(), st.shift.data_ptr(),
+                      *al, _p(st.count_ptr), float(st.count_host), gamma.data_ptr(), sc.k[0].data_ptr(), sc.k[1].data_ptr(),
+                      sc.k[2].data_ptr(), dgamma.data_ptr(), dbeta.data_ptr(), None, None, s)
+    L.stem_conv_wgrad_norm(x_b1.data_ptr(), dout.data_ptr(), y1.data_ptr(), B, D, H, W, Cc, mp, bshift, fd, fh, fw, *al,
+                           st.mean.data_ptr(), st.rstd.data_ptr(), sc.k[0].data_ptr(), sc.k[1].data_ptr(), sc.k[2].data_ptr(),
+                           st.scale.data_ptr(), st.shift.data_ptr(), dw_accum.data_ptr(), dxsum.data_ptr(), ws_x.data_ptr(), s)
+
+
 _BWS = {}
 FUSED_BWD_TAILS = True
 FUSED_NORM_BWD_REDUCE = False
diff --git a/include/anatomask_hip.h b/include/anatomask_hip.h
--- a/include/anatomask_hip.h
+++ b/include/anatomask_hip.h
@@ -130,6 +130,20 @@
                       const float* pre_scale, const float* pre_shift ,
                       const int32_t* active_list, int n_active,
                       int scratch_is_zero_workspace , void* stream);
+int am_stem_bwd_supported(int dtype, int B, int D, int H, int W, int C, int bshift, int n_active);
+int am_stem_norm_bwd_reduce(const void* dout, const void* x, int B, int D, int H, int W, int C, int bshift, const int32_t* active_list,
+                            int n_active, const float* stem_x, const float* stem_w, const float* stem_b, const float* mean,
+                            const float* rstd, const float* scale, const float* shift, double* workspace, const double* count_ptr,
+                            double count_host, const float* gamma, float* k0, float* k1, float* k2, float* dgamma_accum,
+                            float* dbeta_accum, float* dbeta2_accum, void* stream);
+int am_stem_norm_bwd_apply(const void* dout, const void* x, int B, int D, int H, int W, int C, int bshift, const int32_t* active_list,
+                           int n_active, const float* stem_x, const float* stem_w, const float* stem_b, const float* mean,
+                           const float* rstd, const float* k0, const float* k1, const float* k2, const float* scale, const float* shift,
+                           void* dx, float* dxsum_accum, float* stem_dw_accum, double* workspace, void* stream);
+int am_stem_conv_wgrad_norm(const float* x, const void* dout, const void* y, int B, int D, int H, int W, int C, const uint8_t* mask,
+                            int bshift, int fd, int fh, int fw, const int32_t* active_list, int n_active, const float* mean,
+                            const float* rstd, const float* k0, const float* k1, const float* k2, const float* scale, const float* shift,
+                            float* dw_accum, float* dxsum_accum, double* workspace, void* stream);
 int am_chan_sum(int dtype, const void* x, int B, int D, int H, int W, int C, const uint8_t* mask, int bshift, int fd, int fh,
                 int fw, float* out_accum, void* stream);
 int am_add(int dtype, const void* a, const void* b, void* y, long n_elems, void* stream);
```

Measured after the change: 137.8 volumes/s, median of 6. About the same (+0.7%).
